# Xharlie/pointnerf

Hardware: AMD Instinct MI355X
Metric: rays/sec (render+bwd) NeRF-synth lego 800^2, K=8, 128 samp/ray (higher is better)
Workload: dtype f32 in / out / accumulate; forward GEMM operands as 2 x f16 planes (22-bit) on the f16 MFMA, 3 products per multiply-add; input-gradient GEMMs: f16 leading product + e4m3 cross terms (csrc/mixq.h), 2 product equivalents; weight-gradient GEMM operands as one f16 plane each

## Files before the change

pointnerf_amd/csrc/aggregate.hip:

```cpp
#include "mixq.h"
#include <stdlib.h>

extern "C" int pnerf_mlp_layout(int feat_dim, int64_t *offsets) {
    if (feat_dim != PN_F || !offsets) return PNERF_E_UNSUP;
    const int64_t o[PNERF_MLP_NTENSORS + 1] = {PO_W1, PO_B1, PO_W2, PO_B2, PO_W3, PO_B3, PO_W4, PO_B4, PO_W5, PO_B5,
                                               PO_WC1, PO_BC1, PO_WC2, PO_BC2, PO_WC3, PO_BC3, PO_WC4, PO_BC4, PO_TOTAL};
    for (int i = 0; i <= PNERF_MLP_NTENSORS; ++i) offsets[i] = o[i];
    return 0;
}
extern "C" size_t pnerf_mlp_packed_bytes(void) { return (size_t)PKC_END; }

namespace {
struct PackHDesc { int src, ld, trans, Mreal, Kreal, NCH, MB, dst, cm1, ck1; };
__device__ __forceinline__ float pn_pack_scale(const char *packed, int cm1, int ck1, int m, int k) {
    float f = 1.f;
    if (cm1 && m < (cm1 - 1 < PN_CS_C1 ? PN_H : PN_HC)) f = pn_col_scale(packed, cm1 - 1)[m];
    if (ck1) f *= pn_col_scale_inv(packed, ck1 - 1)[k];
    return f;
}
struct ColScaleDesc { int first, units, n_cons; struct { int src, ld, rows; } cons[2]; };
struct ColScaleTable { ColScaleDesc d[7]; };
__global__ __launch_bounds__(256) void k_pack_colscale(ColScaleTable t, const float *__restrict__ params, char *__restrict__ packed) {
    __shared__ unsigned red[256];
    const ColScaleDesc d = t.d[blockIdx.x];
    const int j = threadIdx.x;
    float mx = 0.f;
    if (j < d.units)
        for (int c = 0; c < d.n_cons; ++c)
            for (int r = 0; r < d.cons[c].rows; ++r) mx = fmaxf(mx, fabsf(params[d.cons[c].src + r * d.cons[c].ld + j]));
    const unsigned mb = __float_as_uint(mx);
    const bool ok = mb >= 0x00800000u && mb < 0x7f800000u;
    red[j] = ok ? mb : 0u;
    __syncthreads();
    for (int off = 128; off > 0; off >>= 1) {
        if (j < off) red[j] = red[j] > red[j + off] ? red[j] : red[j + off];
        __syncthreads();
    }
    if (j >= d.units) return;
    int e = ok ? (int)(red[0] >> 23) - (int)(mb >> 23) : 0;
    e = e > PN_CS_MAXE ? PN_CS_MAXE : e;
    float *cs = reinterpret_cast<float *>(packed + PKC_SCALE);
    cs[d.first + j] = __uint_as_float((unsigned)(127 + e) << 23);
    cs[PN_CS_UNITS + d.first + j] = __uint_as_float((unsigned)(127 - e) << 23);
}
struct PackHTable { PackHDesc d[15]; };
__global__ __launch_bounds__(256) void k_pack_h(PackHTable t, const float *__restrict__ params, char *__restrict__ packed) {
    const PackHDesc d = t.d[blockIdx.y];
    const int total = d.NCH * d.MB * 64;
    for (int e = blockIdx.x * 256 + threadIdx.x; e < total; e += gridDim.x * 256) {
        const int lane = e & 63, mb = (e >> 6) % d.MB, c = (e >> 6) / d.MB;
        const int m = 32 * mb + (lane & 31), k0 = 16 * c + 8 * (lane >> 5);
        unsigned h[4], lo[4];
#pragma unroll
        for (int j = 0; j < 4; ++j) {
            float v[2];
#pragma unroll
            for (int i = 0; i < 2; ++i) {
                const int k = k0 + 2 * j + i;
                v[i] = 0.f;
                if (m < d.Mreal && k < d.Kreal) v[i] = d.trans ? params[d.src + k * d.ld + m] * pn_pack_scale(packed, d.cm1, d.ck1, m, k) : params[d.src + m * d.ld + k];
            }
            pn_split2_sat(v[0], v[1], h[j], lo[j]);
        }
        uint4 *o = reinterpret_cast<uint4 *>(packed + d.dst) + ((size_t)(c * d.MB + mb) * 2) * 64 + lane;
        o[0] = make_uint4(h[0], h[1], h[2], h[3]);
        o[64] = make_uint4(lo[0], lo[1], lo[2], lo[3]);
    }
}

struct PackMDesc { int src, ld, trans, Mreal, Kreal, NT, MB, dst, cm1, ck1; };
struct PackMTable { PackMDesc d[9]; };
__global__ __launch_bounds__(256) void k_pack_mix(PackMTable t, const float *__restrict__ params, char *__restrict__ packed) {
    pn_mode_saturate();
    const PackMDesc d = t.d[blockIdx.y];
    auto W = [&](int m, int k) -> float {
        return (m < d.Mreal && k < d.Kreal) ? (d.trans ? params[d.src + k * d.ld + m] * pn_pack_scale(packed, d.cm1, d.ck1, m, k) : params[d.src + m * d.ld + k]) : 0.f;
    };
    uint4 *img = reinterpret_cast<uint4 *>(packed + d.dst);
    unsigned *sc = reinterpret_cast<unsigned *>(img + PN_MIMG_U4(d.NT, d.MB));
    const int nsup = PN_MIX_NS * d.MB * 64, ntail = d.NT * d.MB * 64;
    for (int e = blockIdx.x * 256 + threadIdx.x; e < nsup + ntail; e += gridDim.x * 256) {
        if (e < nsup) {
            const int lane = e & 63, mb = (e >> 6) % d.MB, s = (e >> 6) / d.MB, m = 32 * mb + (lane & 31), hf = lane >> 5;
            uint4 *o = img + ((size_t)(s * d.MB + mb) * 8) * 64 + lane;
#pragma unroll
            for (int r = 0; r < 4; ++r) {
                const int k0 = 64 * s + 16 * r + 8 * hf;
                unsigned h[4], lo[4];
#pragma unroll
                for (int j = 0; j < 4; ++j) pn_split2_rne(W(m, k0 + 2 * j), W(m, k0 + 2 * j + 1), h[j], lo[j]);
                o[r * 64] = make_uint4(h[0], h[1], h[2], h[3]);
            }
            unsigned scw = 0u;
#pragma unroll
            for (int j = 0; j < 2; ++j) {
                float wh[16], wm[16], mx = 0.f;
#pragma unroll
                for (int i = 0; i < 32; ++i) {
                    const float w = W(m, 64 * s + 32 * j + i);
#ifdef PN_EMU
                    const float wc = fmaxf(fminf(w, 65504.f), -65504.f);
#else
                    const float wc = w;
#endif
                    const float h = (float)(_Float16)wc;
                    mx = fmaxf(mx, fmaxf(fabsf(h), fabsf(w - h) * 2048.f));
                }
#pragma unroll
                for (int i = 0; i < 16; ++i) {
                    const float w = W(m, 8 * (8 * s + 4 * j + 2 * hf + (i >> 3)) + (i & 7));
#ifdef PN_EMU
                    const float wc = fmaxf(fminf(w, 65504.f), -65504.f);
#else
                    const float wc = w;
#endif
                    wh[i] = (float)(_Float16)wc; wm[i] = w - wh[i];
                }
                int ex = 0;
                const float fr = frexpf(mx, &ex);
                int be = mx > 0.f ? (fr > 0.875f ? ex - 8 : ex - 9) : 0;
                be = be < -100 ? -100 : (be > 100 ? 100 : be);
                const float sh = __uint_as_float((unsigned)(be + 127) << 23), sm = __uint_as_float((unsigned)(be + 127 - 11) << 23);
                scw |= (unsigned)(be + 127) << (8 * j);
#pragma unroll
                for (int tt = 0; tt < 2; ++tt) {
                    unsigned q[4];
#pragma unroll
                    for (int w4 = 0; w4 < 4; ++w4) {
                        const float *src = (w4 < 2 ? wm : wh) + 8 * tt + 4 * (w4 & 1);
                        const float scl = w4 < 2 ? sm : sh;
                        pn_s2 r = {0, 0};
                        r = __builtin_amdgcn_cvt_scalef32_pk_fp8_f32(r, src[0], src[1], scl, false);
                        r = __builtin_amdgcn_cvt_scalef32_pk_fp8_f32(r, src[2], src[3], scl, true);
                        q[w4] = __builtin_bit_cast(unsigned, r);
                    }
                    o[(4 + 2 * j + tt) * 64] = make_uint4(q[0], q[1], q[2], q[3]);
                }
            }
            sc[(size_t)(s * d.MB + mb) * 64 + lane] = scw;
        } else {
            const int e2 = e - nsup, lane = e2 & 63, mb = (e2 >> 6) % d.MB, tc = (e2 >> 6) / d.MB, m = 32 * mb + (lane & 31);
            const int k0 = 256 + 16 * tc + 8 * (lane >> 5);
            unsigned h[4], lo[4];
#pragma unroll
            for (int j = 0; j < 4; ++j) pn_split2_sat(W(m, k0 + 2 * j), W(m, k0 + 2 * j + 1), h[j], lo[j]);
            uint4 *o = img + (size_t)PN_MIX_NS * d.MB * 8 * 64 + ((size_t)(tc * d.MB + mb) * 2) * 64 + lane;
            o[0] = make_uint4(h[0], h[1], h[2], h[3]);
            o[64] = make_uint4(lo[0], lo[1], lo[2], lo[3]);
        }
    }
}
}

extern "C" int pnerf_mlp_pack(const float *d_params, void *d_packed, void *stream) {
    if (!d_params || !d_packed) return PNERF_E_INVAL;
    PackHTable th = {{
        {PO_W1, PN_IN1, 0, PN_H, PN_IN1, 18, 8, PKH_F1},
        {PO_W2, PN_H, 0, PN_H, PN_H, 16, 8, PKH_F2},
        {PO_W3, PN_IN3, 0, PN_H, PN_IN3, 17, 8, PKH_F3},
        {PO_W4, PN_H, 0, PN_H, PN_H, 16, 8, PKH_F4},
        {PO_W4, PN_H, 1, PN_H, PN_H, 16, 8, PKH_D4, PN_CS_L3 + 1, PN_CS_L4 + 1},
        {PO_W3, PN_IN3, 1, PN_IN3, PN_H, 16, 9, PKH_D3, PN_CS_L2 + 1, PN_CS_L3 + 1},
        {PO_W2, PN_H, 1, PN_H, PN_H, 16, 8, PKH_D2, PN_CS_L1 + 1, PN_CS_L2 + 1},
        {PO_W1, PN_IN1, 1, 32 * PN_MB_D1, PN_H, 16, PN_MB_D1, PKH_D1, 0, PN_CS_L1 + 1},
        {PO_WC1, PN_INC, 0, PN_HC, PN_INC, 18, 4, PKH_FC1},
        {PO_WC2, PN_HC, 0, PN_HC, PN_HC, 8, 4, PKH_FC2},
        {PO_WC3, PN_HC, 0, PN_HC, PN_HC, 8, 4, PKH_FC3},
        {PO_WC3, PN_HC, 1, PN_HC, PN_HC, 8, 4, PKH_DC3, PN_CS_C2 + 1, PN_CS_C3 + 1},
        {PO_WC2, PN_HC, 1, PN_HC, PN_HC, 8, 4, PKH_DC2, PN_CS_C1 + 1, PN_CS_C2 + 1},
        {PO_WC1, PN_INC, 1, PN_H, PN_HC, 8, 8, PKH_DC1, PN_CS_L4 + 1, PN_CS_C1 + 1},
        {PO_W1 + 32 * PN_MB_D1, PN_IN1, 1, PN_IN1 - 32 * PN_MB_D1, PN_H, 16, 2, PKH_D1T, 0, PN_CS_L1 + 1},
    }};
    const ColScaleTable tc = {{
        {PN_CS_L1, PN_H, 1, {{PO_W2, PN_H, PN_H}}},
        {PN_CS_L2, PN_H, 1, {{PO_W3, PN_IN3, PN_H}}},
        {PN_CS_L3, PN_H, 1, {{PO_W4, PN_H, PN_H}}},
        {PN_CS_L4, PN_H, 2, {{PO_W5, PN_H, 1}, {PO_WC1, PN_INC, PN_HC}}},
        {PN_CS_C1, PN_HC, 1, {{PO_WC2, PN_HC, PN_HC}}},
        {PN_CS_C2, PN_HC, 1, {{PO_WC3, PN_HC, PN_HC}}},
        {PN_CS_C3, PN_HC, 1, {{PO_WC4, PN_HC, 3}}},
    }};
    PnProfScope prof(PNK_PACK, (hipStream_t)stream);
    hipLaunchKernelGGL(k_pack_colscale, dim3(7), dim3(256), 0, (hipStream_t)stream, tc, d_params, (char *)d_packed);
    hipLaunchKernelGGL(k_pack_h, dim3(40, 15), dim3(256), 0, (hipStream_t)stream, th, d_params, (char *)d_packed);
    PackMTable tm = {{
        {PO_W1, PN_IN1, 0, PN_H, PN_IN1, 2, 8, PKM_F1},
        {PO_W2, PN_H, 0, PN_H, PN_H, 0, 8, PKM_F2},
        {PO_W3, PN_IN3, 0, PN_H, PN_IN3, 1, 8, PKM_F3},
        {PO_W4, PN_H, 0, PN_H, PN_H, 0, 8, PKM_F4},
        {PO_W4, PN_H, 1, PN_H, PN_H, 0, 8, PKM_D4, PN_CS_L3 + 1, PN_CS_L4 + 1},
        {PO_W3, PN_IN3, 1, PN_IN3, PN_H, 0, 9, PKM_D3, PN_CS_L2 + 1, PN_CS_L3 + 1},
        {PO_W2, PN_H, 1, PN_H, PN_H, 0, 8, PKM_D2, PN_CS_L1 + 1, PN_CS_L2 + 1},
        {PO_W1, PN_IN1, 1, 32 * PN_MB_D1, PN_H, 0, PN_MB_D1, PKM_D1, 0, PN_CS_L1 + 1},
        {PO_W1 + 32 * PN_MB_D1, PN_IN1, 1, PN_IN1 - 32 * PN_MB_D1, PN_H, 0, 2, PKM_D1T, 0, PN_CS_L1 + 1},
    }};
    hipLaunchKernelGGL(k_pack_mix, dim3(12, 9), dim3(256), 0, (hipStream_t)stream, tm, d_params, (char *)d_packed);
    PN_CHECK_LAUNCH();
    return 0;
}

namespace {
template <int NT>
__global__ __launch_bounds__(256) void k_debug_mix_gemm(const float *__restrict__ x, const char *__restrict__ img, float *__restrict__ out) {
    extern __shared__ __attribute__((aligned(16))) char smem_d[];
    pn_mode_saturate();
    constexpr int K = 256 + 16 * NT;
    char *X = smem_d;
    const int tid = threadIdx.x, lane = tid & 63, wave = __builtin_amdgcn_readfirstlane(tid >> 6);
    for (int e = tid; e < PN_TILE * (K / 4); e += 256) {
        const int row = e / (K / 4), col = 4 * (e % (K / 4));
        const float4 v = *reinterpret_cast<const float4 *>(x + row * K + col);
        if (col < 256) pn_xq_store4(X, row, col, v.x, v.y, v.z, v.w);
        else pn_xt_store4(X, row, col, v.x, v.y, v.z, v.w);
    }
    __syncthreads();
    f32x16 acc[2][2];
    pn_acc_zero(acc);
    pn_gemm_mix<PN_MIX_NS, NT, 8, 2>(X, img, 2 * wave, lane, acc);
#pragma unroll
    for (int fb = 0; fb < 2; ++fb)
#pragma unroll
        for (int rb = 0; rb < 2; ++rb)
#pragma unroll
            for (int g = 0; g < 4; ++g)
#pragma unroll
                for (int i = 0; i < 4; ++i) out[(32 * rb + (lane & 31)) * PN_H + pn_d_feat(2 * wave + fb, g, lane) + i] = acc[fb][rb][4 * g + i];
}
}

extern "C" int pnerf_debug_mix_gemm(const float *d_w, int K, const float *d_x, void *d_img, float *d_out, void *stream) {
    if (!d_w || !d_x || !d_img || !d_out || (K != 256 && K != 272 && K != 288)) return PNERF_E_INVAL;
    hipStream_t s = (hipStream_t)stream;
    const int NT = (K - 256) / 16;
    PackMTable tm = {{{0, K, 0, PN_H, K, NT, 8, 0}}};
    hipLaunchKernelGGL(k_pack_mix, dim3(12, 1), dim3(256), 0, s, tm, d_w, (char *)d_img);
    const void *fn = NT == 0 ? (const void *)k_debug_mix_gemm<0> : NT == 1 ? (const void *)k_debug_mix_gemm<1> : (const void *)k_debug_mix_gemm<2>;
    if (hipFuncSetAttribute(fn, hipFuncAttributeMaxDynamicSharedMemorySize, PN_XBYTES) != hipSuccess) return PNERF_E_LAUNCH;
    if (NT == 0) hipLaunchKernelGGL(k_debug_mix_gemm<0>, dim3(1), dim3(256), PN_XBYTES, s, d_x, (const char *)d_img, d_out);
    else if (NT == 1) hipLaunchKernelGGL(k_debug_mix_gemm<1>, dim3(1), dim3(256), PN_XBYTES, s, d_x, (const char *)d_img, d_out);
    else hipLaunchKernelGGL(k_debug_mix_gemm<2>, dim3(1), dim3(256), PN_XBYTES, s, d_x, (const char *)d_img, d_out);
    PN_CHECK_LAUNCH();
    return 0;
}

namespace {
__global__ __launch_bounds__(64) void k_debug_mfma_f16(const uint4 *__restrict__ a, const uint4 *__restrict__ b, float *__restrict__ d) {
    f32x16 acc;
#pragma unroll
    for (int r = 0; r < 16; ++r) acc[r] = 0.f;
    acc = __builtin_amdgcn_mfma_f32_32x32x16_f16(__builtin_bit_cast(pn_h8, a[threadIdx.x]), __builtin_bit_cast(pn_h8, b[threadIdx.x]), acc, 0, 0, 0);
#pragma unroll
    for (int r = 0; r < 16; ++r) d[threadIdx.x * 16 + r] = acc[r];
}
}
namespace {
__global__ __launch_bounds__(256) void k_debug_split(const float *__restrict__ x, long long n, unsigned *__restrict__ h, unsigned *__restrict__ m, int sat) {
    for (long long i = (long long)blockIdx.x * 256 + threadIdx.x; 2 * i < n; i += (long long)gridDim.x * 256) {
        unsigned hh, mm;
        if (sat) pn_split2_sat(x[2 * i], x[2 * i + 1], hh, mm);
        else pn_split2(x[2 * i], x[2 * i + 1], hh, mm);
        h[i] = hh; m[i] = mm;
    }
}
}
extern "C" int pnerf_debug_split(const float *d_x, int64_t n, void *d_h, void *d_m, int sat, void *stream) {
    if (!d_x || !d_h || !d_m || n < 0 || (n & 1)) return PNERF_E_INVAL;
    if (n == 0) return 0;
    hipLaunchKernelGGL(k_debug_split, dim3(64), dim3(256), 0, (hipStream_t)stream, d_x, (long long)n, (unsigned *)d_h, (unsigned *)d_m, sat);
    PN_CHECK_LAUNCH();
    return 0;
}

namespace {
template <int NF> __global__ __launch_bounds__(256) void k_debug_pe(const float *__restrict__ x, long long n, float *__restrict__ out) {
    for (long long i = (long long)blockIdx.x * 256 + threadIdx.x; i < n; i += (long long)gridDim.x * 256) {
        float s[NF], c[NF];
        pn_pe_octaves<NF>(x[i], s, c);
#pragma unroll
        for (int f = 0; f < NF; ++f) { out[(i * NF + f) * 2] = s[f]; out[(i * NF + f) * 2 + 1] = c[f]; }
    }
}
}
extern "C" int pnerf_debug_pe(const float *d_x, int64_t n, int nfreq, float *d_out, void *stream) {
    if (!d_x || !d_out || n < 0 || nfreq < 1 || nfreq > 5) return PNERF_E_INVAL;
    if (n == 0) return 0;
    hipStream_t s = (hipStream_t)stream;
    switch (nfreq) {
        case 1: hipLaunchKernelGGL(k_debug_pe<1>, dim3(64), dim3(256), 0, s, d_x, (long long)n, d_out); break;
        case 2: hipLaunchKernelGGL(k_debug_pe<2>, dim3(64), dim3(256), 0, s, d_x, (long long)n, d_out); break;
        case 3: hipLaunchKernelGGL(k_debug_pe<3>, dim3(64), dim3(256), 0, s, d_x, (long long)n, d_out); break;
        case 4: hipLaunchKernelGGL(k_debug_pe<4>, dim3(64), dim3(256), 0, s, d_x, (long long)n, d_out); break;
        default: hipLaunchKernelGGL(k_debug_pe<5>, dim3(64), dim3(256), 0, s, d_x, (long long)n, d_out); break;
    }
    PN_CHECK_LAUNCH();
    return 0;
}

extern "C" int pnerf_debug_mfma_f16(const void *d_a, const void *d_b, float *d_out, void *stream) {
    if (!d_a || !d_b || !d_out) return PNERF_E_INVAL;
    hipLaunchKernelGGL(k_debug_mfma_f16, dim3(1), dim3(64), 0, (hipStream_t)stream, (const uint4 *)d_a, (const uint4 *)d_b, d_out);
    PN_CHECK_LAUNCH();
    return 0;
}

size_t pn_saved_walk(void *base, long long n_valid, int K, PnSaved &s) {
    const int TS = pn_tile_samples(K);
    const long long tiles = (n_valid + TS - 1) / TS + 2 * PN_NCLS + 1;
    s.rows = tiles * PN_TILE;
    s.samples = ((tiles * TS + PN_CTILE - 1) / PN_CTILE + 1) * PN_CTILE;
    PnCarver cv(base);
    const size_t rg = (size_t)s.rows / 8, rgc = (size_t)s.samples / 8;
    auto planes = [&](uint4 *&x0, uint4 *&h2, uint4 *&h1, uint4 *&h3, uint4 *&dy1, uint4 *&dy2, uint4 *&dy3, uint4 *&dy4) {
        x0 = cv.take<uint4>(rg * PN_NF1); h2 = cv.take<uint4>(rg * PN_NF1);
        h1 = cv.take<uint4>(rg * PN_H); h3 = cv.take<uint4>(rg * PN_H);
        dy1 = cv.take<uint4>(rg * PN_H); dy2 = cv.take<uint4>(rg * PN_H);
        dy3 = cv.take<uint4>(rg * PN_H); dy4 = cv.take<uint4>(rg * PN_H);
    };
    auto cplanes = [&](uint4 *&xc, uint4 *&c1, uint4 *&c2, uint4 *&dc1, uint4 *&dc2, uint4 *&dc3) {
        xc = cv.take<uint4>(rgc * PN_NF1); c1 = cv.take<uint4>(rgc * PN_HC); c2 = cv.take<uint4>(rgc * PN_HC);
        dc1 = cv.take<uint4>(rgc * PN_HC); dc2 = cv.take<uint4>(rgc * PN_HC); dc3 = cv.take<uint4>(rgc * PN_HC);
    };
    planes(s.x0k, s.h2k, s.h1k, s.h3k, s.dy1k, s.dy2k, s.dy3k, s.dy4k);
    s.h4r = cv.take<uint4>((size_t)s.rows * 32 * 2);
    s.arow = cv.take<float>((size_t)s.rows); s.rmeta = cv.take<int4>((size_t)s.rows);
    s.lmask = cv.take<unsigned>((size_t)tiles * 3 * 512);
    s.gscale = cv.take<unsigned>(PN_GS_WORDS);
    s.fs = cv.take<float>((size_t)s.samples * PN_H); s.dfs = cv.take<float>((size_t)s.samples * PN_H);
    s.c3 = cv.take<float>((size_t)s.samples * PN_HC);
    cplanes(s.xck, s.c1k, s.c2k, s.dc1k, s.dc2k, s.dc3k);
    s.cmask = cv.take<unsigned>((size_t)s.samples / PN_CTILE * 2 * 256);
    s.wg2 = pn_arith().wgrad_planes == 2 ? 1 : 0;
    s.x0m = s.h1m = s.h2m = s.h3m = s.dy1m = s.dy2m = s.dy3m = s.dy4m = nullptr;
    s.xcm = s.c1m = s.c2m = s.dc1m = s.dc2m = s.dc3m = nullptr;
    if (s.wg2) {
        planes(s.x0m, s.h2m, s.h1m, s.h3m, s.dy1m, s.dy2m, s.dy3m, s.dy4m);
        cplanes(s.xcm, s.c1m, s.c2m, s.dc1m, s.dc2m, s.dc3m);
    }
    pn_cls_walk(cv, s);
    return cv.off;
}
void pn_cls_walk(PnCarver &cv, PnSaved &s) {
    s.cls_list = cv.take<int>((size_t)s.samples);
    s.cls_info = cv.take<int>(PN_CI_WORDS);
    s.cls_tmp = cv.take<int>((size_t)2 * s.samples + pn_scan_scratch_ints(s.samples) + 8);
}
size_t pn_saved_bytes(long long n_valid, int K) { PnSaved s; return pn_saved_walk(nullptr, n_valid, K, s); }
PnSaved pn_saved_carve(void *base, long long n_valid, int K) { PnSaved s; pn_saved_walk(base, n_valid, K, s); return s; }

extern "C" size_t pnerf_agg_saved_bytes(int64_t n_valid_samples, int K) {
    if (K <= 0 || K > PNERF_MAX_K || n_valid_samples < 0) return 0;
    return pn_saved_bytes(n_valid_samples, K);
}

namespace {
struct FwdArgs {
    pnerf_camera cam;
    const float *xyz, *emb, *conf, *dir, *color;
    const float *params;
    const float4 *packed;
    const float *raydir, *sample_loc;
    const float *xyz_pers, *loc_pers;
    const int *pidx, *valid_list, *counters;
    const int *cls_list, *cls_info;
    int cls, Kstride;
    int save_x0;
    int R, SR, K, TS;
    long long cap_samples;
    float *decoded, *weight;
    PnSaved sv;
};
struct FwdArgsF : FwdArgs { const float *frames; };
template <bool FRAMES> struct FwdArgsOf { using type = FwdArgs; };
template <> struct FwdArgsOf<true> { using type = FwdArgsF; };

namespace {
struct ClsArgs { const int *valid_list, *counters, *pidx; int K, n, ncls; int kc[PN_NCLS], ts[PN_NCLS]; };

__global__ void k_cls_flags(ClsArgs c, int which, int *__restrict__ flags) {
    const int vs = blockIdx.x * blockDim.x + threadIdx.x;
    if (vs >= c.n) return;
    const int Ns = c.counters[0] < c.n ? c.counters[0] : c.n;
    int f = 0;
    if (vs < Ns) {
        const long long si = c.valid_list[vs];
        int hv = 0;
        for (int k = 0; k < c.K; ++k)
            if (c.pidx[si * c.K + k] >= 0) hv = k + 1;
        int cl = 0;
        for (int j = 1; j < c.ncls; ++j)
            if (hv <= c.kc[j]) cl = j;
        f = cl == which;
    }
    flags[vs] = f;
}

__global__ void k_cls_gather(ClsArgs c, int which, const int *__restrict__ pos, const int *__restrict__ count, int *__restrict__ cls_list,
                             int *__restrict__ info) {
    const int n = *count, base = info[PN_CI_VBASE + which];
    for (int i = blockIdx.x * blockDim.x + threadIdx.x; i < n; i += gridDim.x * blockDim.x) cls_list[base + i] = c.valid_list[pos[i]];
    if (blockIdx.x == 0 && threadIdx.x == 0) {
        const int tiles = (n + c.ts[which] - 1) / c.ts[which], tb = info[PN_CI_TBASE + which];
        info[PN_CI_COUNT + which] = n;
        if (which + 1 < PN_NCLS) { info[PN_CI_VBASE + which + 1] = base + n; info[PN_CI_TBASE + which + 1] = tb + tiles + 1; }
        info[PN_CI_TILES] = tb + tiles + 1;
    }
}

__global__ void k_cls_zero_gaps(PnSaved sv, int ncls, int save_x0) {
    const int c = blockIdx.y;
    if (c >= ncls) return;
    if ((blockIdx.x == 0 && !save_x0) || (blockIdx.x == 8 && save_x0)) return;
    const long long gap = (c + 1 < PN_NCLS ? sv.cls_info[PN_CI_TBASE + c + 1] : sv.cls_info[PN_CI_TILES]) - 1;
    uint4 *arrs[9] = {sv.x0k, sv.h2k, sv.h1k, sv.h3k, sv.dy1k, sv.dy2k, sv.dy3k, sv.dy4k, sv.x0k};
    uint4 *arrm[9] = {sv.x0m, sv.h2m, sv.h1m, sv.h3m, sv.dy1m, sv.dy2m, sv.dy3m, sv.dy4m, nullptr};
    const int which = blockIdx.x;
    const int nf = which == 8 ? 64 : which < 2 ? PN_NF1 : PN_H;
    uint4 *p = arrs[which] + gap * 8 * nf;
    for (int i = threadIdx.x; i < 8 * nf; i += blockDim.x) p[i] = make_uint4(0u, 0u, 0u, 0u);
    if (sv.wg2 && arrm[which]) {
        uint4 *pm = arrm[which] + gap * 8 * nf;
        for (int i = threadIdx.x; i < 8 * nf; i += blockDim.x) pm[i] = make_uint4(0u, 0u, 0u, 0u);
    }
}
}

}

int pn_class_slots(int K, int kc[PN_NCLS]) {
    if (K % 4 == 0) { kc[0] = K; kc[1] = K / 2; kc[2] = K / 4; return 3; }
    kc[0] = K; kc[1] = kc[2] = 0;
    return 1;
}

int pn_classify(const PnSaved &sv, const int32_t *d_valid_list, const int32_t *d_counters, const int32_t *d_pidx, int K, long long n_valid,
                bool train, bool save_x0, hipStream_t s) {
    ClsArgs c;
    c.valid_list = d_valid_list; c.counters = d_counters; c.pidx = d_pidx; c.K = K; c.n = (int)n_valid;
    c.ncls = pn_class_slots(K, c.kc);
    for (int j = 0; j < PN_NCLS; ++j) c.ts[j] = c.kc[j] > 0 ? pn_tile_samples(c.kc[j]) : 1;
    if (hipMemsetAsync(sv.cls_info, 0, PN_CI_WORDS * sizeof(int), s) != hipSuccess) return PNERF_E_LAUNCH;
    if (n_valid <= 0) return 0;
    int *flags = sv.cls_tmp, *pos = flags + n_valid, *cnt = pos + n_valid, *scratch = cnt + 8;
    PnProfScope prof(PNK_COMPACT, s);
    for (int j = 0; j < c.ncls; ++j) {
        hipLaunchKernelGGL(k_cls_flags, dim3(pn_cdiv(n_valid, 256)), dim3(256), 0, s, c, j, flags);
        int rc = pn_compact_gt0_i32(flags, n_valid, pos, cnt, scratch, s);
        if (rc) return rc;
        hipLaunchKernelGGL(k_cls_gather, dim3(256), dim3(256), 0, s, c, j, pos, cnt, sv.cls_list, sv.cls_info);
    }
    if (train) hipLaunchKernelGGL(k_cls_zero_gaps, dim3(9, c.ncls), dim3(256), 0, s, sv, c.ncls, save_x0 ? 1 : 0);
    PN_CHECK_LAUNCH();
    return 0;
}


namespace {

constexpr int FL_EX = PN_XBYTES, FL_W5 = FL_EX + PN_TILE * 8 * 4, FL_ROW = FL_W5 + PN_H * 4, FL_CLAIM = FL_ROW + 4 * PN_TILE * 4 , FL_BYTES = FL_CLAIM + 16;
static_assert(2 * FL_BYTES <= 160 * 1024, "two forward workgroups must fit the 160 KB LDS");

struct FGather {
    float4 e0, e1;
    float px, py, pz, lx, ly, lz, cf;
    float ppx, ppy, ppz, lpx, lpy, lpz;
    float dxv, dyv, dzv, cx, cy, cz, rx, ry, rz;
    float fx, fy, fz, gx, gy, gz;
};

__device__ __forceinline__ int f_sample_of(const FwdArgs &a, long long tile, int row, int Ns, unsigned kinv) {
    const int ls = pn_row_div(row, kinv);
    const long long vs = tile * a.TS + ls;
    return (ls < a.TS && vs < Ns) ? a.valid_list[vs] : -1;
}

template <bool PERS, bool FRAMES = false>
__device__ __forceinline__ void f_gather(const FwdArgs &a, FGather &G, int si_, int p_, int q, const float *frames = nullptr) {
    const int p = p_ > 0 ? p_ : 0, si = si_ > 0 ? si_ : 0;
    const float *ep = a.emb + (long long)p * PN_F + PN_EPT * q;
    G.e0 = *reinterpret_cast<const float4 *>(ep); G.e1 = *reinterpret_cast<const float4 *>(ep + 4);
    G.px = a.xyz[3 * p]; G.py = a.xyz[3 * p + 1]; G.pz = a.xyz[3 * p + 2];
    G.lx = a.sample_loc[(long long)si * 3]; G.ly = a.sample_loc[(long long)si * 3 + 1]; G.lz = a.sample_loc[(long long)si * 3 + 2];
    if (PERS) {
        G.ppx = a.xyz_pers[3 * p]; G.ppy = a.xyz_pers[3 * p + 1]; G.ppz = a.xyz_pers[3 * p + 2];
        G.lpx = a.loc_pers[(long long)si * 3]; G.lpy = a.loc_pers[(long long)si * 3 + 1]; G.lpz = a.loc_pers[(long long)si * 3 + 2];
    }
    G.cf = a.conf[p];
    if (FRAMES) {
        const int r = si / a.SR, fr = q < 3 ? q : 2;
        const int ps_ = a.pidx[(long long)si * a.Kstride], ps = ps_ > 0 ? ps_ : 0;
        const float *fp = frames + (long long)p * 9 + 3 * fr, *gp = frames + (long long)ps * 9 + 3 * fr;
        G.fx = fp[0]; G.fy = fp[1]; G.fz = fp[2];
        G.gx = gp[0]; G.gy = gp[1]; G.gz = gp[2];
        G.dxv = a.dir[3 * p]; G.dyv = a.dir[3 * p + 1]; G.dzv = a.dir[3 * p + 2];
        G.rx = a.raydir[3 * r]; G.ry = a.raydir[3 * r + 1]; G.rz = a.raydir[3 * r + 2];
        if (q == 0) { G.cx = a.color[3 * p]; G.cy = a.color[3 * p + 1]; G.cz = a.color[3 * p + 2]; }
    } else if (q == 0) {
        const int r = si / a.SR;
        G.dxv = a.dir[3 * p]; G.dyv = a.dir[3 * p + 1]; G.dzv = a.dir[3 * p + 2];
        G.cx = a.color[3 * p]; G.cy = a.color[3 * p + 1]; G.cz = a.color[3 * p + 2];
        G.rx = a.raydir[3 * r]; G.ry = a.raydir[3 * r + 1]; G.rz = a.raydir[3 * r + 2];
    }
}

template <bool PERS, bool MIX = false, bool FRAMES = false>
__device__ __forceinline__ void f_build(const FwdArgs &a, const FGather &G, char *X, float *exb, float *wraw, int *sidx, int si, int p, int row, int q) {
    const float dwx = G.px - G.lx, dwy = G.py - G.ly, dwz = G.pz - G.lz;
    float ppx, ppy, pcz, spx, spy, scz;
    if (PERS) {
        ppx = G.ppx; ppy = G.ppy; pcz = G.ppz; spx = G.lpx; spy = G.lpy; scz = G.lpz;
    } else {
        float pcx, pcy, scx, scy;
        if (FRAMES) {
            const float *M = a.cam.camrot;
            const float x = G.px - a.cam.campos[0], y = G.py - a.cam.campos[1], z = G.pz - a.cam.campos[2];
            const float u = G.lx - a.cam.campos[0], v = G.ly - a.cam.campos[1], w = G.lz - a.cam.campos[2];
            pcx = __builtin_fmaf(z, M[6], __builtin_fmaf(y, M[3], x * M[0]));
            pcy = __builtin_fmaf(z, M[7], __builtin_fmaf(y, M[4], x * M[1]));
            pcz = __builtin_fmaf(z, M[8], __builtin_fmaf(y, M[5], x * M[2]));
            scx = __builtin_fmaf(w, M[6], __builtin_fmaf(u, M[0], v * M[3]));
            scy = __builtin_fmaf(w, M[7], __builtin_fmaf(u, M[1], v * M[4]));
            scz = __builtin_fmaf(w, M[8], __builtin_fmaf(u, M[2], v * M[5]));
        } else {
        rot3(a.cam.camrot, G.px - a.cam.campos[0], G.py - a.cam.campos[1], G.pz - a.cam.campos[2], false, pcx, pcy, pcz);
        rot3(a.cam.camrot, G.lx - a.cam.campos[0], G.ly - a.cam.campos[1], G.lz - a.cam.campos[2], false, scx, scy, scz);
        }
        ppx = pcx / pcz; ppy = pcy / pcz; spx = scx / scz; spy = scy / scz;
    }
    float d0, d1, d2;
    if (FRAMES) d0 = d1 = d2 = dwx * G.fx + dwy * G.fy + dwz * G.fz;
    else rot3(a.cam.rw2c, dwx, dwy, dwz, true, d0, d1, d2);
    const float d3 = ppx * pcz - spx * scz, d4 = ppy * pcz - spy * scz, d5 = pcz - scz;
    const float da = q == 0 ? d0 : q == 1 ? d1 : q == 2 ? d2 : d3;
    const float db = q == 0 ? d4 : d5;
    const float e[8] = {G.e0.x, G.e0.y, G.e0.z, G.e0.w, G.e1.x, G.e1.y, G.e1.z, G.e1.w};
    if (MIX) {
        pn_xq_store4(X, row, PN_EPT * q, e[0], e[1], e[2], e[3]);
        pn_xq_store4(X, row, PN_EPT * q + 4, e[4], e[5], e[6], e[7]);
#pragma unroll
        for (int i = 0; i < 8; i += 2) {
            const int col = PN_F + (PN_EPT * q + i) * 6;
            float s0[3], c0[3], s1[3], c1[3];
            pn_pe_octaves<3>(e[i], s0, c0);
            pn_pe_octaves<3>(e[i + 1], s1, c1);
            pn_xq_store4(X, row, col, s0[0], c0[0], s0[1], c0[1]);
            pn_xq_store4(X, row, col + 4, s0[2], c0[2], s1[0], c1[0]);
            pn_xq_store4(X, row, col + 8, s1[1], c1[1], s1[2], c1[2]);
        }
    } else {
    pn_xt_store4(X, row, PN_EPT * q, e[0], e[1], e[2], e[3]); pn_xt_store4(X, row, PN_EPT * q + 4, e[4], e[5], e[6], e[7]);
#pragma unroll
    for (int i = 0; i < 8; ++i) {
        const int dd = PN_EPT * q + i;
        float s[3], c[3];
        pn_pe_octaves<3>(e[i], s, c);
        pn_xt_store2(X, row, PN_F + dd * 6, s[0], c[0]);
        pn_xt_store2(X, row, PN_F + dd * 6 + 2, s[1], c[1]);
        pn_xt_store2(X, row, PN_F + dd * 6 + 4, s[2], c[2]);
    }
    }
#pragma unroll
    for (int j = 0; j < 2; ++j) {
        const int comp = q + 4 * j;
        if (comp < 6) {
            float s[5], c[5];
            pn_pe_octaves<5>(j == 0 ? da : db, s, c);
#pragma unroll
            for (int f = 0; f < 5; ++f) {
                if (MIX) pn_xa_store2(X, row, PN_F * 7 + (comp * 5 + f) * 2, s[f], c[f]);
                else pn_xt_store2(X, row, PN_F * 7 + (comp * 5 + f) * 2, s[f], c[f]);
            }
        }
    }
    if (q == 3) pn_xt_store4(X, row, PN_ONES1, 1.f, 0.f, 0.f, 0.f);
    float fvx = 0.f, fvy = 0.f, fvz = 0.f, fqx = 0.f, fqy = 0.f, fqz = 0.f;
    if (FRAMES) {
        fvx = G.rx * G.gx + G.ry * G.gy + G.rz * G.gz;
        fqx = G.dxv * G.fx + G.dyv * G.fy + G.dzv * G.fz;
        fvy = __shfl_down(fvx, 1, 64); fvz = __shfl_down(fvx, 2, 64);
        fqy = __shfl_down(fqx, 1, 64); fqz = __shfl_down(fqx, 2, 64);
    }
    if (q == 0) {
        float vx, vy, vz, qx, qy, qz;
        if (FRAMES) { vx = fvx; vy = fvy; vz = fvz; qx = fqx; qy = fqy; qz = fqz; }
        else {
        rot3(a.cam.rw2c, G.rx, G.ry, G.rz, true, vx, vy, vz);
        rot3(a.cam.rw2c, G.dxv, G.dyv, G.dzv, true, qx, qy, qz);
        }
        float *ex = exb + row * 8;
        *reinterpret_cast<float4 *>(ex) = make_float4(G.cx, G.cy, G.cz, qx - vx);
        if (FRAMES) {
            *reinterpret_cast<float4 *>(ex + 4) = make_float4(qy - vy, qz - vz, __builtin_fmaf(qz, vz, __builtin_fmaf(qx, vx, qy * vy)), 1.f);
            wraw[row] = p >= 0 ? 1.0f / fmaxf(sqrtf(__builtin_fmaf(dwz, dwz, __builtin_fmaf(dwx, dwx, dwy * dwy))), 1e-6f) : 0.f;
        } else {
        *reinterpret_cast<float4 *>(ex + 4) = make_float4(qy - vy, qz - vz, qx * vx + qy * vy + qz * vz, 1.f);
        wraw[row] = p >= 0 ? 1.0f / fmaxf(sqrtf(dwx * dwx + dwy * dwy + dwz * dwz), 1e-6f) : 0.f;
        }
        sidx[row] = si;
    }
}

__device__ __forceinline__ void f_acc_bias(const float *__restrict__ bias, int wave, int lane, f32x16 (&acc)[PN_NFB][2]) {
#pragma unroll
    for (int fb = 0; fb < PN_NFB; ++fb)
#pragma unroll
        for (int g = 0; g < 4; ++g) {
            const float4 b = *reinterpret_cast<const float4 *>(bias + pn_d_feat(PN_NFB * wave + fb, g, lane));
#pragma unroll
            for (int rb = 0; rb < 2; ++rb) { acc[fb][rb][4 * g] = b.x; acc[fb][rb][4 * g + 1] = b.y; acc[fb][rb][4 * g + 2] = b.z; acc[fb][rb][4 * g + 3] = b.w; }
        }
}
template <bool BITS, bool MIX = false, bool HR = false>
__device__ __forceinline__ void f_epilogue(const f32x16 (&acc)[PN_NFB][2], char *X, int wave, int lane, unsigned (&mw)[PN_NFB]) {
#pragma unroll
    for (int fb = 0; fb < PN_NFB; ++fb) mw[fb] = 0u;
#pragma unroll
    for (int fb = 0; fb < PN_NFB; ++fb)
#pragma unroll
        for (int rb = 0; rb < 2; ++rb)
#pragma unroll
            for (int g = 0; g < 4; ++g) {
                const int f0 = pn_d_feat(PN_NFB * wave + fb, g, lane);
                float v[4] = {acc[fb][rb][4 * g], acc[fb][rb][4 * g + 1], acc[fb][rb][4 * g + 2], acc[fb][rb][4 * g + 3]};
                if (BITS) {
#pragma unroll
                    for (int i = 0; i < 4; ++i) mw[fb] = __builtin_amdgcn_alignbit(mw[fb], __float_as_uint(v[i]), 31);
                }
#pragma unroll
                for (int i = 0; i < 4; ++i) v[i] = fmaxf(v[i], 0.01f * v[i]);
                if (MIX) pn_xq_store4(X, 32 * rb + (lane & 31), f0, v[0], v[1], v[2], v[3]);
                else if (HR) pn_xt_store4(X, 32 * rb + (lane & 31), f0, v[0], v[1], v[2], v[3]);
                else pn_x_store4<false>(X, 32 * rb + (lane & 31), f0, v[0], v[1], v[2], v[3]);
            }
}
__device__ __forceinline__ void f_store_masks(unsigned *__restrict__ lmask, long long gtile, int layer, int wave, int lane, const unsigned (&mw)[PN_NFB]) {
#pragma unroll
    for (int fb = 0; fb < PN_NFB; ++fb) lmask[((gtile * 3 + layer) * 8 + PN_NFB * wave + fb) * 64 + lane] = mw[fb];
}

template <int KC, bool TRAIN>
__device__ __forceinline__ void f_tail(const FwdArgs &a, const char *X, const float *w5s, const float *wrow, const int *sidx, float b5,
                                       long long tile, long long gtile, int tid, float *wraw = nullptr) {
    constexpr int NS = KC == 0 ? 1 : 8 / (KC == 0 ? 1 : KC);
    const int lane = tid & 63, cg = tid & 31, r0 = 8 * (tid >> 5);
    const float4 wa = *reinterpret_cast<const float4 *>(w5s + 8 * cg), wb = *reinterpret_cast<const float4 *>(w5s + 8 * cg + 4);
    float pa[8];
    float4 fa[NS], fb[NS];
#pragma unroll
    for (int j = 0; j < NS; ++j) fa[j] = fb[j] = make_float4(0.f, 0.f, 0.f, 0.f);
#pragma unroll
    for (int i = 0; i < 8; ++i) {
        const int r = r0 + i;
        const uint4 h = *reinterpret_cast<const uint4 *>(X + r * PN_XRS + cg * 16);
        const uint4 m = *reinterpret_cast<const uint4 *>(X + PN_XPLANE + r * PN_XRS + cg * 16);
        if (TRAIN) {
            pn_f4 th = {__uint_as_float(h.x), __uint_as_float(h.y), __uint_as_float(h.z), __uint_as_float(h.w)};
            pn_f4 tm = {__uint_as_float(m.x), __uint_as_float(m.y), __uint_as_float(m.z), __uint_as_float(m.w)};
            PN_STREAM_STORE(th, reinterpret_cast<pn_f4 *>(a.sv.h4r + (gtile * PN_TILE + r) * 32 + cg));
            PN_STREAM_STORE(tm, reinterpret_cast<pn_f4 *>(a.sv.h4r + (a.sv.rows + gtile * PN_TILE + r) * 32 + cg));
        }
        float s = 0.f;
        s = pn_fma2_lo(h.x, m.x, wa.x, s); s = pn_fma2_hi(h.x, m.x, wa.y, s); s = pn_fma2_lo(h.y, m.y, wa.z, s); s = pn_fma2_hi(h.y, m.y, wa.w, s);
        s = pn_fma2_lo(h.z, m.z, wb.x, s); s = pn_fma2_hi(h.z, m.z, wb.y, s); s = pn_fma2_lo(h.w, m.w, wb.z, s); s = pn_fma2_hi(h.w, m.w, wb.w, s);
        pa[i] = s;
        if (KC != 0) {
            const float w = wrow[r];
            float4 &f0 = fa[i / (KC == 0 ? 1 : KC)], &f1 = fb[i / (KC == 0 ? 1 : KC)];
            f0.x = pn_fma2_lo(h.x, m.x, w, f0.x); f0.y = pn_fma2_hi(h.x, m.x, w, f0.y); f0.z = pn_fma2_lo(h.y, m.y, w, f0.z); f0.w = pn_fma2_hi(h.y, m.y, w, f0.w);
            f1.x = pn_fma2_lo(h.z, m.z, w, f1.x); f1.y = pn_fma2_hi(h.z, m.z, w, f1.y); f1.z = pn_fma2_lo(h.w, m.w, w, f1.z); f1.w = pn_fma2_hi(h.w, m.w, w, f1.w);
        }
    }
#pragma unroll
    for (int j = 0; j < (KC == 0 ? 0 : NS); ++j) {
        const long long vs = tile * (PN_TILE / (KC == 0 ? 1 : KC)) + (r0 / (KC == 0 ? 1 : KC)) + j;
        if (vs < a.cap_samples) {
            *reinterpret_cast<float4 *>(a.sv.fs + vs * PN_H + 8 * cg) = fa[j];
            *reinterpret_cast<float4 *>(a.sv.fs + vs * PN_H + 8 * cg + 4) = fb[j];
        }
    }
    {
        const bool b4 = lane & 16, b3 = lane & 8, b2 = lane & 4;
#pragma unroll
        for (int j = 0; j < 4; ++j) { const float send = b4 ? pa[j] : pa[j + 4], keep = b4 ? pa[j + 4] : pa[j]; pa[j] = keep + __shfl_xor(send, 16, 64); }
#pragma unroll
        for (int j = 0; j < 2; ++j) { const float send = b3 ? pa[j] : pa[j + 2], keep = b3 ? pa[j + 2] : pa[j]; pa[j] = keep + __shfl_xor(send, 8, 64); }
        { const float send = b2 ? pa[0] : pa[1], keep = b2 ? pa[1] : pa[0]; pa[0] = keep + __shfl_xor(send, 4, 64); }
        pa[0] += __shfl_xor(pa[0], 2, 64);
        pa[0] += __shfl_xor(pa[0], 1, 64);
        const int i = ((lane >> 4) & 1) * 4 + ((lane >> 3) & 1) * 2 + ((lane >> 2) & 1), r = r0 + i;
        const float x = pa[0] + b5 - 1.0f;
        float sg = pn_softplus(x) * wrow[r];
        if (TRAIN && (lane & 3) == 0) a.sv.arow[gtile * PN_TILE + r] = x;
        if (KC == 0) {
            if ((lane & 3) == 0) wraw[r] = sg;
            return;
        }
        if (KC >= 2) sg += __shfl_xor(sg, 4, 64);
        if (KC >= 4) sg += __shfl_xor(sg, 8, 64);
        if (KC >= 8) sg += __shfl_xor(sg, 16, 64);
        if ((lane & 3) == 0 && (i % (KC == 0 ? 1 : KC)) == 0) {
            const int si = sidx[r];
            if (si >= 0) a.decoded[(long long)si * 4] = sg;
        }
    }
}

#ifdef PN_PHASE_TRACE
PN_TR_DECL(pn_trace_fwd);
PN_TR_SPAN_DECL(pn_span_fwd);
#endif
template <bool TRAIN, bool PERS, int NP, bool WG2 = false, bool FRAMES = false>
__global__ __launch_bounds__(PN_NTHR, PN_NW / 2) void k_agg_forward(typename FwdArgsOf<FRAMES>::type a) {
    constexpr bool MIX = NP == 4;
    static_assert(!FRAMES || (!TRAIN && NP == 3), "per-point frames: the default inference arithmetic only");
    constexpr bool HR = !MIX;
    constexpr bool HC = TRAIN && !WG2;
    static_assert(!(MIX && WG2), "the two-plane weight-gradient mode keeps f16x3.h's arithmetic everywhere");
    pn_mode_saturate();
    extern __shared__ __attribute__((aligned(16))) char smem_f[];
    char *X = smem_f;
    float *exb = reinterpret_cast<float *>(smem_f + FL_EX), *w5s = reinterpret_cast<float *>(smem_f + FL_W5);
    float *wraw = reinterpret_cast<float *>(smem_f + FL_ROW), *wrow = wraw + PN_TILE, *wnrm = wrow + PN_TILE;
    int *sidx = reinterpret_cast<int *>(wnrm + PN_TILE);
    const float *frames = nullptr;
    if constexpr (FRAMES) frames = a.frames;
    const int tid0 = threadIdx.x;
    const int K = a.K, TS = a.TS;
    const unsigned kinv = pn_kinv(K);
    const int Ns = a.cls_info[PN_CI_COUNT + a.cls];
    const long long vb = a.cls_info[PN_CI_VBASE + a.cls], tb = a.cls_info[PN_CI_TBASE + a.cls];
    a.valid_list = a.cls_list + vb; a.cap_samples = Ns;
    a.sv.fs += vb * PN_H;
    const long long ntiles = ((long long)Ns + TS - 1) / TS;
    const float *P = a.params;
    const char *img = reinterpret_cast<const char *>(a.packed);
    if (tid0 < PN_H) w5s[tid0] = P[PO_W5 + tid0];
    const float b5 = P[PO_B5];
    const int tile_last = (int)ntiles, grid = gridDim.x;
    int t0 = blockIdx.x, t1 = t0 + grid, t2 = t1 + grid;
    if (t0 >= tile_last) return;
    int *claim_ctr = a.sv.cls_info + PN_CI_CLAIM + a.cls, *claim_w = reinterpret_cast<int *>(smem_f + FL_CLAIM);
    int nclaim = 0;

    long long tile = t0;
    int si0, si1, si2, p0, p1;
    FGather G;
    {
        const int row = tid0 / PN_TPR, q = tid0 % PN_TPR, k = row - pn_row_div(row, kinv) * K;
        si0 = f_sample_of(a, tile, row, Ns, kinv); si1 = t1 < tile_last ? f_sample_of(a, t1, row, Ns, kinv) : -1;
        si2 = t2 < tile_last ? f_sample_of(a, t2, row, Ns, kinv) : -1;
        p0 = si0 >= 0 ? a.pidx[(long long)si0 * a.Kstride + k] : -1;
        p1 = si1 >= 0 ? a.pidx[(long long)si1 * a.Kstride + k] : -1;
        f_gather<PERS, FRAMES>(a, G, si0, p0, q, frames);
    }

    f32x16 acc[PN_NFB][2];
    PN_TR_ITER_DECL;
    for (bool first = true; t0 < tile_last; first = false) {
        PN_TR_ITER_NEXT;
        tile = t0;
        int tid = threadIdx.x;
        asm volatile("" : "+v"(tid));
        const int lane = tid & 63, wave = __builtin_amdgcn_readfirstlane(tid >> 6);
        const int row = tid / PN_TPR, q = tid % PN_TPR, k = row - pn_row_div(row, kinv) * K;
        const long long gtile = tb + tile;
        PN_LDS_BARRIER();
        PN_TR(pn_trace_fwd, 0); PN_TR_HWID(pn_trace_fwd); PN_TR_SPAN(pn_span_fwd, a.cls, 0);
        f_build<PERS, MIX, FRAMES>(a, G, X, exb, wraw, sidx, si0, p0, row, q);
        f_acc_bias(P + PO_B1, wave, lane, acc);
        PnTileW<MIX, 2, 8, NP> W1;
        W1.prefetch(img, PKH_F1, PKM_F1, PN_NFB * wave, lane);
        PN_LDS_BARRIER();
        if (q == 0) {
            const int ls = pn_row_div(row, kinv);
            float wn = 0.f, w = 0.f;
            if (si0 >= 0) {
                float sum = 0.f;
                for (int kk = 0; kk < K; ++kk) sum += wraw[ls * K + kk];
                wn = wraw[row] / fmaxf(sum, 1e-8f);
                w = wn * fminf(fmaxf(G.cf, 1e-4f), 1.0f);
                a.weight[(long long)si0 * a.Kstride + k] = wn;
            }
            wnrm[row] = wn; wrow[row] = w;
            if (TRAIN) a.sv.rmeta[gtile * PN_TILE + row] = make_int4(si0, si0 >= 0 ? p0 : -1, __float_as_int(wn), __float_as_int(w));
        }
        unsigned mask[PN_NFB];
        PN_TR(pn_trace_fwd, 1);
        PN_TR(pn_trace_fwd, 2);
        W1.run(X, lane, acc);
        if (TRAIN) {
            if (HC) {
                if (a.save_x0) pn_copy_out_kmajor_h<PN_NF1>(X, a.sv.x0k, gtile * 8, tid);
                else pn_copy_out_kmajor_cols64_h<224>(X, a.sv.x0k, gtile * 8, tid);
            } else if (WG2) pn_copy_out_kmajor<PN_NF1, true>(X, a.sv.x0k, gtile * 8, tid, a.sv.x0m);
            else if (a.save_x0) pn_copy_out_kmajor<PN_NF1, false>(X, a.sv.x0k, gtile * 8, tid);
            else pn_copy_out_kmajor_cols64<224>(X, a.sv.x0k, gtile * 8, tid);
        }
        PN_LDS_BARRIER();
        PN_TR(pn_trace_fwd, 3);
        f_epilogue<TRAIN, MIX, HR>(acc, X, wave, lane, mask);
        if (TRAIN) f_store_masks(a.sv.lmask, gtile, 0, wave, lane, mask);
        f_acc_bias(P + PO_B2, wave, lane, acc);
        PnTileW<MIX, 0, 8, NP> W2;
        W2.prefetch(img, PKH_F2, PKM_F2, PN_NFB * wave, lane);
        PN_LDS_BARRIER();
        PN_TR(pn_trace_fwd, 4);
        PN_TR(pn_trace_fwd, 5);
        W2.run(X, lane, acc);
        if (TRAIN) {
            if (HC) pn_copy_out_kmajor_h<PN_H>(X, a.sv.h1k, gtile * 8, tid);
            else pn_copy_out_kmajor<PN_H, WG2>(X, a.sv.h1k, gtile * 8, tid, a.sv.h1m);
        }
        PN_LDS_BARRIER();
        PN_TR(pn_trace_fwd, 6);
        f_epilogue<TRAIN, MIX, HR>(acc, X, wave, lane, mask);
        if (TRAIN) f_store_masks(a.sv.lmask, gtile, 1, wave, lane, mask);
        if (tid < PN_TILE) {
            const float4 u = *reinterpret_cast<const float4 *>(exb + tid * 8), v = *reinterpret_cast<const float4 *>(exb + tid * 8 + 4);
            pn_xt_store4(X, tid, PN_H, u.x, u.y, u.z, u.w);
            pn_xt_store4(X, tid, PN_H + 4, v.x, v.y, v.z, v.w);
            pn_xt_store4(X, tid, PN_H + 8, 0.f, 0.f, 0.f, 0.f);
            pn_xt_store4(X, tid, PN_H + 12, 0.f, 0.f, 0.f, 0.f);
        }
        f_acc_bias(P + PO_B3, wave, lane, acc);
        PnTileW<MIX, 1, 8, NP> W3;
        W3.prefetch(img, PKH_F3, PKM_F3, PN_NFB * wave, lane);
        PN_LDS_BARRIER();
        PN_TR(pn_trace_fwd, 7);
        PN_TR(pn_trace_fwd, 8);
        W3.run(X, lane, acc);
        if (TRAIN) {
            if (HC) pn_copy_out_kmajor_h<PN_NF1>(X, a.sv.h2k, gtile * 8, tid);
            else pn_copy_out_kmajor<PN_NF1, WG2>(X, a.sv.h2k, gtile * 8, tid, a.sv.h2m);
        }
        PN_LDS_BARRIER();
        PN_TR(pn_trace_fwd, 9);
        f_epilogue<TRAIN, MIX, HR>(acc, X, wave, lane, mask);
        if (TRAIN) f_store_masks(a.sv.lmask, gtile, 2, wave, lane, mask);
        f_acc_bias(P + PO_B4, wave, lane, acc);
        PnTileW<MIX, 0, 8, NP> W4;
        W4.prefetch(img, PKH_F4, PKM_F4, PN_NFB * wave, lane);
        PN_LDS_BARRIER();
        PN_TR(pn_trace_fwd, 10);
        PN_TR(pn_trace_fwd, 11);
        W4.run(X, lane, acc);
        if (TRAIN) {
            if (HC) pn_copy_out_kmajor_h<PN_H>(X, a.sv.h3k, gtile * 8, tid);
            else pn_copy_out_kmajor<PN_H, WG2>(X, a.sv.h3k, gtile * 8, tid, a.sv.h3m);
        }
        PN_TR(pn_trace_fwd, 12);
        const int t3 = first ? t2 + grid : pn_claim_tile(PN_CLAIM_STATIC_FWD, grid, __builtin_amdgcn_readfirstlane(*claim_w), nclaim - 1);
        const bool claims = nclaim % PN_CLAIM_TILES == 0;
        int claimed = 0;
        if (tid == 0 && claims) claimed = atomicAdd(claim_ctr, 1);
        const int si_next = si1, p_next = p1;
        if (t1 < tile_last) f_gather<PERS, FRAMES>(a, G, si1, p1, q, frames);
        const int p2 = si2 >= 0 ? a.pidx[(long long)si2 * a.Kstride + k] : -1;
        const int si3 = t3 < tile_last ? f_sample_of(a, t3, row, Ns, kinv) : -1;
        PN_LDS_BARRIER();
        PN_TR(pn_trace_fwd, 13);
        f_epilogue<false>(acc, X, wave, lane, mask);
        PN_LDS_BARRIER();
        PN_TR(pn_trace_fwd, 14);
        if (K == 8 || K == 4 || K == 2 || K == 1) {
            if (K == 8) f_tail<8, TRAIN>(a, X, w5s, wrow, sidx, b5, tile, gtile, tid);
            else if (K == 4) f_tail<4, TRAIN>(a, X, w5s, wrow, sidx, b5, tile, gtile, tid);
            else if (K == 2) f_tail<2, TRAIN>(a, X, w5s, wrow, sidx, b5, tile, gtile, tid);
            else f_tail<1, TRAIN>(a, X, w5s, wrow, sidx, b5, tile, gtile, tid);
            PN_TR(pn_trace_fwd, 15);
        } else {
        f_tail<0, TRAIN>(a, X, w5s, wrow, sidx, b5, tile, gtile, tid, wraw);
        PN_LDS_BARRIER();
        PN_TR(pn_trace_fwd, 15);
        for (int e = tid; e < TS * 32; e += PN_NTHR) {
            const int ls = e >> 5, cg = e & 31;
            float4 f0 = make_float4(0.f, 0.f, 0.f, 0.f), f1 = f0;
            for (int kk = 0; kk < K; ++kk) {
                const int r = ls * K + kk;
                const uint4 h = *reinterpret_cast<const uint4 *>(X + r * PN_XRS + cg * 16);
                const uint4 m = *reinterpret_cast<const uint4 *>(X + PN_XPLANE + r * PN_XRS + cg * 16);
                const float w = wrow[r];
                f0.x = pn_fma2_lo(h.x, m.x, w, f0.x); f0.y = pn_fma2_hi(h.x, m.x, w, f0.y); f0.z = pn_fma2_lo(h.y, m.y, w, f0.z); f0.w = pn_fma2_hi(h.y, m.y, w, f0.w);
                f1.x = pn_fma2_lo(h.z, m.z, w, f1.x); f1.y = pn_fma2_hi(h.z, m.z, w, f1.y); f1.z = pn_fma2_lo(h.w, m.w, w, f1.z); f1.w = pn_fma2_hi(h.w, m.w, w, f1.w);
            }
            const long long vs = tile * TS + ls;
            if (vs < a.cap_samples) {
                *reinterpret_cast<float4 *>(a.sv.fs + vs * PN_H + 8 * cg) = f0;
                *reinterpret_cast<float4 *>(a.sv.fs + vs * PN_H + 8 * cg + 4) = f1;
            }
        }
        if (tid < TS) {
            const int si = sidx[tid * K];
            if (si >= 0) {
                float sg = 0.f;
                for (int kk = 0; kk < K; ++kk) sg += wraw[tid * K + kk];
                a.decoded[(long long)si * 4] = sg;
            }
        }
        }
        si0 = si_next; p0 = p_next; si1 = si2; p1 = p2; si2 = si3;
        if (tid == 0 && claims) *claim_w = claimed;
        t0 = t1; t1 = t2; t2 = t3; ++nclaim;
        PN_TR(pn_trace_fwd, 16); PN_TR_SPAN(pn_span_fwd, a.cls, 1);
    }
}

constexpr int CL_W4 = PN_XBYTES, CL_BYTES = CL_W4 + 3 * PN_HC * 4;
static_assert(2 * CL_BYTES <= 160 * 1024, "two colour workgroups must fit the 160 KB LDS");

__device__ __forceinline__ void c_load_bias(const float *__restrict__ bias, int wave, int lane, float4 (&b)[4]) {
#pragma unroll
    for (int g = 0; g < 4; ++g) {
        const float *p = bias + pn_d_feat(wave, g, lane);
        b[g] = make_float4(p[0], p[1], p[2], p[3]);
    }
}
template <bool TRAIN, bool SAVE32>
__device__ __forceinline__ unsigned c_epilogue(const f32x16 (&acc)[2][2], const float4 (&bias)[4], char *X, int wave, int lane, float *__restrict__ save, long long grow0) {
    unsigned mw = 0u;
#pragma unroll
    for (int rb = 0; rb < 2; ++rb)
#pragma unroll
        for (int g = 0; g < 4; ++g) {
            const int f0 = pn_d_feat(wave, g, lane), row = 32 * rb + (lane & 31);
            const float4 b = bias[g];
            float v[4] = {acc[0][rb][4 * g] + b.x, acc[0][rb][4 * g + 1] + b.y, acc[0][rb][4 * g + 2] + b.z, acc[0][rb][4 * g + 3] + b.w};
            if (TRAIN && !SAVE32) {
#pragma unroll
                for (int i = 0; i < 4; ++i) mw = __builtin_amdgcn_alignbit(mw, __float_as_uint(v[i]), 31);
            }
#pragma unroll
            for (int i = 0; i < 4; ++i) v[i] = fmaxf(v[i], 0.01f * v[i]);
            if (TRAIN && SAVE32) {
                pn_f4 t = {v[0], v[1], v[2], v[3]};
                PN_REG_STORE(t, reinterpret_cast<pn_f4 *>(save + (grow0 + row) * PN_HC + f0));
            }
            pn_x_store4<false>(X, row, f0, v[0], v[1], v[2], v[3]);
        }
    return mw;
}

template <bool TRAIN, int NP, bool WG2 = false, bool FRAMES = false>
__global__ __launch_bounds__(256, 2) void k_color_forward(typename FwdArgsOf<FRAMES>::type a) {
    extern __shared__ __attribute__((aligned(16))) char smem_c[];
    char *X = smem_c;
    float *w4s = reinterpret_cast<float *>(smem_c + CL_W4);
    const int Ns = a.counters[0] < a.cap_samples ? a.counters[0] : (int)a.cap_samples;
    const float *P = a.params;
    const char *img = reinterpret_cast<const char *>(a.packed);
    for (int i = threadIdx.x; i < 3 * PN_HC; i += 256) w4s[i] = P[PO_WC4 + i];
    const float b40 = P[PO_BC4], b41 = P[PO_BC4 + 1], b42 = P[PO_BC4 + 2];

    f32x16 acc[2][2];
    for (long long tile = blockIdx.x; tile * PN_CTILE < Ns; tile += gridDim.x) {
        int tid = threadIdx.x;
        asm volatile("" : "+v"(tid));
        const int lane = tid & 63, wave = __builtin_amdgcn_readfirstlane(tid >> 6), row = tid >> 2, q = tid & 3;
        const long long grow0 = tile * PN_CTILE, vs = grow0 + row;
        const int si = vs < Ns ? a.valid_list[vs] : -1;
        PnGemmW<18, 4, 1, 7, NP> WC1;
        WC1.prefetch(reinterpret_cast<const uint4 *>(img + PKH_FC1), wave, lane);
        PN_LDS_BARRIER();
        if (si >= 0) {
            const float4 *f = reinterpret_cast<const float4 *>(a.sv.fs + vs * PN_H);
            float4 fv[16];
#pragma unroll
            for (int c = 0; c < 16; ++c) fv[c] = f[4 * c + q];
#pragma unroll
            for (int c = 0; c < 16; ++c) pn_x_store4<false>(X, row, 16 * c + 4 * q, fv[c].x, fv[c].y, fv[c].z, fv[c].w);
            {
                const int r = si / a.SR;
                float v[3], sn[4], cs[4];
                if constexpr (FRAMES) {
                    const int ps_ = a.pidx[(long long)si * a.Kstride], ps = ps_ > 0 ? ps_ : 0;
                    const float *fp = a.frames + (long long)ps * 9;
                    const float fm[9] = {fp[0], fp[1], fp[2], fp[3], fp[4], fp[5], fp[6], fp[7], fp[8]};
                    rot3(fm, a.raydir[3 * r], a.raydir[3 * r + 1], a.raydir[3 * r + 2], true, v[0], v[1], v[2]);
                } else
                rot3(a.cam.rw2c, a.raydir[3 * r], a.raydir[3 * r + 1], a.raydir[3 * r + 2], true, v[0], v[1], v[2]);
                const float vq = q == 0 ? v[0] : (q == 1 ? v[1] : v[2]);
                pn_pe_octaves<4>(vq, sn, cs);
                if (q < 3) {
                    pn_x_store4<false>(X, row, PN_H + 4 * q, sn[0], sn[1], sn[2], sn[3]);
                    pn_x_store4<false>(X, row, PN_H + 12 + 4 * q, cs[0], cs[1], cs[2], cs[3]);
                } else {
                    pn_x_store4<false>(X, row, PN_H + 24, 0.f, 0.f, 0.f, 0.f);
                    pn_x_store4<false>(X, row, PN_H + 28, 0.f, 0.f, 0.f, 0.f);
                }
            }
        } else {
#pragma unroll
            for (int c = 0; c < 18; ++c) pn_x_store4<false>(X, row, 16 * c + 4 * q, 0.f, 0.f, 0.f, 0.f);
        }
        PN_LDS_BARRIER();
        float4 bias[4];
        if (TRAIN) pn_copy_out_kmajor<PN_NF1, WG2>(X, a.sv.xck, tile * 8, tid, a.sv.xcm);
        pn_acc_zero(acc);
        pn_gemm_f16x3_run<18, 4, 1, 7, NP>(X, WC1, lane, acc);
        c_load_bias(P + PO_BC1, wave, lane, bias);
        PN_LDS_BARRIER();
        unsigned mw = c_epilogue<TRAIN, false>(acc, bias, X, wave, lane, nullptr, grow0);
        if (TRAIN) a.sv.cmask[(tile * 2 + 0) * 256 + tid] = mw;
        PnGemmW<8, 4, 1, 7, NP> WC2;
        WC2.prefetch(reinterpret_cast<const uint4 *>(img + PKH_FC2), wave, lane);
        PN_LDS_BARRIER();
        if (TRAIN) pn_copy_out_kmajor<PN_HC, WG2>(X, a.sv.c1k, tile * 8, tid, a.sv.c1m);
        pn_acc_zero(acc);
        pn_gemm_f16x3_run<8, 4, 1, 7, NP>(X, WC2, lane, acc);
        c_load_bias(P + PO_BC2, wave, lane, bias);
        PN_LDS_BARRIER();
        mw = c_epilogue<TRAIN, false>(acc, bias, X, wave, lane, nullptr, grow0);
        if (TRAIN) a.sv.cmask[(tile * 2 + 1) * 256 + tid] = mw;
        PnGemmW<8, 4, 1, 7, NP> WC3;
        WC3.prefetch(reinterpret_cast<const uint4 *>(img + PKH_FC3), wave, lane);
        PN_LDS_BARRIER();
        if (TRAIN) pn_copy_out_kmajor<PN_HC, WG2>(X, a.sv.c2k, tile * 8, tid, a.sv.c2m);
        pn_acc_zero(acc);
        pn_gemm_f16x3_run<8, 4, 1, 7, NP>(X, WC3, lane, acc);
        c_load_bias(P + PO_BC3, wave, lane, bias);
        PN_LDS_BARRIER();
        c_epilogue<TRAIN, true>(acc, bias, X, wave, lane, a.sv.c3, grow0);
        PN_LDS_BARRIER();
        {
            float o0 = 0.f, o1 = 0.f, o2 = 0.f;
#pragma unroll
            for (int j = 0; j < 4; ++j) {
                const int c0 = q * 32 + 8 * j;
                o0 = pn_x_dot8(X, row, c0, *reinterpret_cast<const float4 *>(w4s + c0), *reinterpret_cast<const float4 *>(w4s + c0 + 4), o0);
                o1 = pn_x_dot8(X, row, c0, *reinterpret_cast<const float4 *>(w4s + PN_HC + c0), *reinterpret_cast<const float4 *>(w4s + PN_HC + c0 + 4), o1);
                o2 = pn_x_dot8(X, row, c0, *reinterpret_cast<const float4 *>(w4s + 2 * PN_HC + c0), *reinterpret_cast<const float4 *>(w4s + 2 * PN_HC + c0 + 4), o2);
            }
            o0 = group_sum<4>(o0); o1 = group_sum<4>(o1); o2 = group_sum<4>(o2);
            if (q == 0 && si >= 0) {
                float *o = a.decoded + (long long)si * 4;
                o[1] = 1.0f / (1.0f + expf(-(o0 + b40))) * 1.002f - 0.001f;
                o[2] = 1.0f / (1.0f + expf(-(o1 + b41))) * 1.002f - 0.001f;
                o[3] = 1.0f / (1.0f + expf(-(o2 + b42))) * 1.002f - 0.001f;
            }
        }
    }
}
}

#ifndef PN_MIX_DEFAULT_MASK
#define PN_MIX_DEFAULT_MASK 4
#endif
static PnArith &pn_arith_record() {
    static PnArith a = [] {
        const char *e = getenv("PNERF_MIX_MASK");
        return PnArith{3, 1, 8, e ? atoi(e) & 7 : PN_MIX_DEFAULT_MASK};
    }();
    return a;
}
PnArith pn_arith() { return pn_arith_record(); }
static int pn_arith_set(int PnArith::*field, int v, bool valid) {
    if (!valid) return PNERF_E_INVAL;
    const int old = pn_arith_record().*field;
    pn_arith_record().*field = v;
    return old;
}
extern "C" int pnerf_set_inference_products(int n) { return pn_arith_set(&PnArith::products, n, n == 2 || n == 3); }
extern "C" int pnerf_set_wgrad_planes(int n) { return pn_arith_set(&PnArith::wgrad_planes, n, n == 1 || n == 2); }
extern "C" int pnerf_set_cross_terms(int bits) { return pn_arith_set(&PnArith::cross_terms, bits, bits == 8 || bits == 16); }
extern "C" int pnerf_set_cross_terms_where(int mask) { return pn_arith_set(&PnArith::mix_where, mask, mask >= 0 && mask <= 7); }
static int pn_tile_grid_cap = 0;
int pn_tile_grid(long long tiles, long long dflt) { return pn_capped_grid(tiles, pn_tile_grid_cap > 0 && pn_tile_grid_cap < dflt ? pn_tile_grid_cap : dflt); }
extern "C" int pnerf_debug_set_tile_grid(int max_workgroups) {
    if (max_workgroups < 0) return PNERF_E_INVAL;
    const int old = pn_tile_grid_cap;
    pn_tile_grid_cap = max_workgroups;
    return old;
}
extern "C" int pnerf_get_arithmetic(int32_t out[4]) {
    if (!out) return PNERF_E_INVAL;
    const PnArith a = pn_arith();
    out[0] = a.products; out[1] = a.wgrad_planes; out[2] = a.cross_terms; out[3] = a.mix_where;
    return 0;
}

int pn_agg_forward_launch(const pnerf_camera *cam, const pnerf_points *pts, const pnerf_step &st, float *d_decoded, float *d_weight,
                          const PnSaved &sv, bool train, bool save_x0, hipStream_t s) {
    const int K = st.K;
    const long long cap_samples = st.n_valid_max;
    const PnArith ar = pn_arith();
    FwdArgs a;
    const bool wg2 = train && sv.wg2;
    if (wg2) save_x0 = true;
    a.save_x0 = save_x0 ? 1 : 0;
    a.cam = *cam;
    a.xyz = pts->xyz; a.emb = pts->embedding; a.conf = pts->conf; a.dir = pts->dir; a.color = pts->color;
    a.params = st.params; a.packed = (const float4 *)st.packed_mlp;
    a.raydir = st.raydir; a.sample_loc = st.sample_loc; a.xyz_pers = st.xyz_pers; a.loc_pers = st.loc_pers; a.pidx = st.sample_pidx; a.valid_list = st.valid_list; a.counters = st.counters;
    a.R = st.R; a.SR = st.SR; a.K = K; a.TS = pn_tile_samples(K);
    a.cap_samples = cap_samples;
    a.decoded = d_decoded; a.weight = d_weight; a.sv = sv;
    const bool frames = pts->frames != nullptr;
    if (frames && train) return PNERF_E_INVAL;
    const int ncu = pn_cu_count();
    if (!ncu) return PNERF_E_LAUNCH;
    const int grid_c = pn_tile_grid((cap_samples + PN_CTILE - 1) / PN_CTILE, 2LL * ncu);
    const size_t lds_a = FL_BYTES, lds_c = CL_BYTES;
    const bool pers = st.xyz_pers != nullptr;
    const bool np2 = !train && ar.products == 2;
    const bool mix = !wg2 && !np2 && (ar.mix_mask() & (train ? 2 : 1));
    if (frames && (np2 || mix)) return PNERF_E_UNSUP;
    using FwdKernel = void (*)(FwdArgs);
    using FwdKernelF = void (*)(FwdArgsF);
    const FwdKernelF kfnf = pers ? k_agg_forward<false, true, 3, false, true> : k_agg_forward<false, false, 3, false, true>;
    const FwdKernelF cfnf = k_color_forward<false, 3, false, true>;
    const FwdKernel kfn = wg2   ? (pers ? k_agg_forward<true, true, 3, true> : k_agg_forward<true, false, 3, true>)
                        : mix   ? (train ? (pers ? k_agg_forward<true, true, 4> : k_agg_forward<true, false, 4>)
                                         : (pers ? k_agg_forward<false, true, 4> : k_agg_forward<false, false, 4>))
                        : train ? (pers ? k_agg_forward<true, true, 3> : k_agg_forward<true, false, 3>)
                        : np2   ? (pers ? k_agg_forward<false, true, 2> : k_agg_forward<false, false, 2>)
                                : (pers ? k_agg_forward<false, true, 3> : k_agg_forward<false, false, 3>);
    const FwdKernel cfn = wg2 ? k_color_forward<true, 3, true> : train ? k_color_forward<true, 3> : np2 ? k_color_forward<false, 2> : k_color_forward<false, 3>;
    if (hipFuncSetAttribute(frames ? reinterpret_cast<const void *>(kfnf) : reinterpret_cast<const void *>(kfn), hipFuncAttributeMaxDynamicSharedMemorySize, (int)lds_a) != hipSuccess) return PNERF_E_LAUNCH;
    if (hipFuncSetAttribute(frames ? reinterpret_cast<const void *>(cfnf) : reinterpret_cast<const void *>(cfn), hipFuncAttributeMaxDynamicSharedMemorySize, (int)lds_c) != hipSuccess) return PNERF_E_LAUNCH;
    int rc = pn_classify(sv, st.valid_list, st.counters, st.sample_pidx, K, cap_samples, train, save_x0, s);
    if (rc) return rc;
    a.cls_list = sv.cls_list; a.cls_info = sv.cls_info; a.Kstride = K;
    int kc[PN_NCLS];
    const int ncls = pn_class_slots(K, kc);
    {
        PnProfScope prof(PNK_AGG_FWD, s);
        for (int j = 0; j < ncls; ++j) {
            a.cls = j; a.K = kc[j]; a.TS = pn_tile_samples(kc[j]);
            const int grid_a = pn_tile_grid((cap_samples + a.TS - 1) / a.TS, 2LL * ncu);
            if (frames) { FwdArgsF af; static_cast<FwdArgs &>(af) = a; af.frames = pts->frames; hipLaunchKernelGGL(kfnf, dim3(grid_a), dim3(PN_NTHR), lds_a, s, af); }
            else hipLaunchKernelGGL(kfn, dim3(grid_a), dim3(PN_NTHR), lds_a, s, a);
        }
    }
    a.K = K; a.TS = pn_tile_samples(K); a.valid_list = sv.cls_list;
    {
        PnProfScope prof(PNK_COLOR_FWD, s);
        if (frames) { FwdArgsF af; static_cast<FwdArgs &>(af) = a; af.frames = pts->frames; hipLaunchKernelGGL(cfnf, dim3(grid_c), dim3(256), lds_c, s, af); }
        else hipLaunchKernelGGL(cfn, dim3(grid_c), dim3(256), lds_c, s, a);
    }
    PN_CHECK_LAUNCH();
    return 0;
}

#ifdef PN_PHASE_TRACE
extern "C" int pnerf_debug_trace_fwd(void *host, size_t bytes) {
    return hipMemcpyFromSymbol(host, HIP_SYMBOL(pn_trace_fwd), bytes < sizeof(pn_trace_fwd) ? bytes : sizeof(pn_trace_fwd)) == hipSuccess ? 0 : -1;
}
extern "C" int pnerf_debug_span_fwd(void *host, size_t bytes) {
    return hipMemcpyFromSymbol(host, HIP_SYMBOL(pn_span_fwd), bytes < sizeof(pn_span_fwd) ? bytes : sizeof(pn_span_fwd)) == hipSuccess ? 0 : -1;
}
#endif
```

pointnerf_amd/csrc/backward.hip:

```cpp
#include "mixq.h"

namespace {
constexpr int WG_CHUNKS = 256;
constexpr size_t PARTIAL_FLOATS = (size_t)WG_CHUNKS * PN_H * PN_IN1P;

struct BwdArgs {
    pnerf_camera cam;
    const float *params;
    const float4 *packed;
    const float *raydir;
    const int *pidx, *valid_list, *counters;
    const int *cls_list, *cls_info;
    int cls;
    int SR, K, TS;
    long long cap_samples;
    const float *decoded, *weight, *grad_decoded;
    PnSaved sv;
    const float *emb;
    float *gparams;
    float *g_emb, *g_conf, *g_dir, *g_color;
    const float *conf, *zo_gs;
    float zo_eps;
};
struct BwdXArgs : BwdArgs {
    const float *xyz, *sample_loc;
    float *g_xyz;
};
template <bool XYZG> struct BwdArgsOf { using T = BwdArgs; };
template <> struct BwdArgsOf<true> { using T = BwdXArgs; };

__global__ __launch_bounds__(256) void k_grad_max(const int *__restrict__ list, const int *__restrict__ counters, long long cap, const float *__restrict__ gd,
                                                  unsigned *__restrict__ gscale) {
    __shared__ unsigned red[4];
    const long long Ns = counters[0] < cap ? counters[0] : cap;
    float m = 0.f;
    for (long long vs = (long long)blockIdx.x * 256 + threadIdx.x; vs < Ns; vs += (long long)gridDim.x * 256) {
        const float4 g = *reinterpret_cast<const float4 *>(gd + (long long)list[vs] * 4);
        m = fmaxf(m, fmaxf(fmaxf(fabsf(g.x), fabsf(g.y)), fmaxf(fabsf(g.z), fabsf(g.w))));
    }
#pragma unroll
    for (int off = 32; off > 0; off >>= 1) m = fmaxf(m, __shfl_xor(m, off, 64));
    if ((threadIdx.x & 63) == 0) red[threadIdx.x >> 6] = __float_as_uint(m);
    __syncthreads();
    if (threadIdx.x == 0) {
        unsigned r = red[0];
        for (int i = 1; i < 4; ++i) r = red[i] > r ? red[i] : r;
        if (r != 0u && r < 0x7f800000u) atomicMax(gscale, r);
    }
}
__device__ __forceinline__ void pn_scale_from_bits(unsigned mb, float &S, float &invS) {
    const int e = (int)((mb >> 23) & 0xffu);
    int se = (e == 0 || e == 255) ? 127 : 127 + 4 - (e - 127);
    se = se < 2 ? 2 : (se > 252 ? 252 : se);
    S = __uint_as_float((unsigned)se << 23);
    invS = __uint_as_float((unsigned)(254 - se) << 23);
}
static_assert(PN_CTILE == PN_TILE, "one row-scale record layout for both tile kernels");
constexpr int PN_RSC_BYTES = PN_TILE * 16 + PN_TILE * 2;
__device__ __forceinline__ void pn_sample_scale(const float4 g, float S, float invS, float &Si, float &invSi) {
    const unsigned mb = __float_as_uint(fmaxf(fmaxf(fabsf(g.x), fabsf(g.y)), fmaxf(fabsf(g.z), fabsf(g.w))));
    Si = S; invSi = invS;
    if (mb >= 0x00800000u && mb < 0x7f800000u) {
        pn_scale_from_bits(mb, Si, invSi);
        if (Si < S) { Si = S; invSi = invS; }
    }
}
struct PnRowScale {
    float *p;
    __device__ __forceinline__ void set(int r, float Si, float invSi, float S, float w = 0.f) const {
        const float f = S * invSi;
        *reinterpret_cast<float4 *>(p + 4 * r) = make_float4(Si, invSi, f, w * Si);
        reinterpret_cast<_Float16 *>(p + 4 * PN_TILE)[r] = (_Float16)f;
    }
    __device__ __forceinline__ float S(int r) const { return p[4 * r]; }
    __device__ __forceinline__ float inv(int r) const { return p[4 * r + 1]; }
    __device__ __forceinline__ float to_call(int r) const { return p[4 * r + 2]; }
    __device__ __forceinline__ float wS(int r) const { return p[4 * r + 3]; }
    __device__ __forceinline__ const char *h8(int rg) const { return reinterpret_cast<const char *>(p + 4 * PN_TILE) + rg * 16; }
};
template <int NF, int XRS = PN_XRS>
__device__ __forceinline__ void pn_copy_out_kmajor_hs(const char *X, const PnRowScale &rs, uint4 *__restrict__ dst, long long rg0, int tid) {
    const int lane = tid & 63, wave = tid >> 6;
    const int blk = ((lane >> 2) & 3) * XRS + ((lane >> 4) * 16 + (lane & 3) * 4) * 2;
#pragma unroll
    for (int i = 0; i < 2; ++i) {
        const int rg = wave * 2 + i;
        const char *src = X + rg * 8 * XRS + blk;
        uint4 *d = dst + (rg0 + rg) * NF;
        const uint4 fq = *reinterpret_cast<const uint4 *>(rs.h8(rg));
        const pn_h4 flo = __builtin_bit_cast(pn_h4, make_uint2(fq.x, fq.y)), fhi = __builtin_bit_cast(pn_h4, make_uint2(fq.z, fq.w));
        uint2 lo[(NF + 63) / 64], hi[(NF + 63) / 64];
#pragma unroll
        for (int j = 0; j < (NF + 63) / 64; ++j) { lo[j] = pn_lds_read_tr16(src + j * 128); hi[j] = pn_lds_read_tr16(src + 4 * XRS + j * 128); }
#pragma unroll
        for (int j = 0; j < (NF + 63) / 64; ++j) {
            const int f = lane + 64 * j;
            if (f < NF) {
                const uint2 a = __builtin_bit_cast(uint2, __builtin_bit_cast(pn_h4, lo[j]) * flo), b = __builtin_bit_cast(uint2, __builtin_bit_cast(pn_h4, hi[j]) * fhi);
                pn_f4 t = {__uint_as_float(a.x), __uint_as_float(a.y), __uint_as_float(b.x), __uint_as_float(b.y)};
                PN_STREAM_STORE(t, reinterpret_cast<pn_f4 *>(d + f));
            }
        }
    }
}

constexpr int CB_XRS = 2 * PN_HC + 16, CB_XPL = PN_CTILE * CB_XRS, CB_XBYTES = 2 * CB_XPL;
constexpr int CB_GSUMS = 6 * PN_HC;
constexpr int CB_DRAW = CB_XBYTES, CB_GACC = CB_DRAW + PN_CTILE * 4 * 4, CB_W4 = CB_GACC + 4 * CB_GSUMS * 4, CB_RSC = CB_W4 + 3 * PN_HC * 4, CB_BYTES = CB_RSC + PN_RSC_BYTES;
static_assert(3 * CB_BYTES <= 160 * 1024, "three colour workgroups must fit the 160 KB LDS");

__device__ __forceinline__ void cb_epilogue(const f32x16 (&acc)[2][2], unsigned mw, char *X, int wave, int lane) {
#pragma unroll
    for (int rb = 0; rb < 2; ++rb)
#pragma unroll
        for (int g = 0; g < 4; ++g) {
            const int f0 = pn_d_feat(wave, g, lane), row = 32 * rb + (lane & 31), e = rb * 16 + g * 4;
            float v[4];
#pragma unroll
            for (int i = 0; i < 4; ++i) v[i] = acc[0][rb][4 * g + i] * ((int)(mw << (e + i)) < 0 ? 0.01f : 1.f);
            pn_x_store4<true, CB_XRS, CB_XPL>(X, row, f0, v[0], v[1], v[2], v[3]);
        }
}
__device__ __forceinline__ void cb_bias_sums(const char *X, const PnRowScale &rs, int tid, float *__restrict__ gsum) {
    const int cp = tid & 63, r0 = 16 * (tid >> 6);
    float g0 = 0.f, g1 = 0.f;
#pragma unroll
    for (int rr = 0; rr < 16; ++rr) {
        const unsigned h = *reinterpret_cast<const unsigned *>(X + (r0 + rr) * CB_XRS + cp * 4);
        const unsigned m = *reinterpret_cast<const unsigned *>(X + CB_XPL + (r0 + rr) * CB_XRS + cp * 4);
        const float f = rs.to_call(r0 + rr);
        g0 = pn_fma2_lo(h, m, f, g0); g1 = pn_fma2_hi(h, m, f, g1);
    }
    float2 *d = reinterpret_cast<float2 *>(gsum) + cp;
    const float2 t = *d;
    *d = make_float2(t.x + g0, t.y + g1);
}

__device__ __forceinline__ void cb_add4(float *__restrict__ d, const float (&v)[4]) {
    float4 *p = reinterpret_cast<float4 *>(d);
    const float4 t = *p;
    *p = make_float4(t.x + v[0], t.y + v[1], t.z + v[2], t.w + v[3]);
}

template <bool WG2>
__global__ __launch_bounds__(256, 3) void k_color_backward(BwdArgs a) {
    extern __shared__ __attribute__((aligned(16))) char smem_cb[];
    char *X = smem_cb;
    float *draw = reinterpret_cast<float *>(smem_cb + CB_DRAW);
    const PnRowScale rs{reinterpret_cast<float *>(smem_cb + CB_RSC)};
    const int Ns = a.counters[0] < a.cap_samples ? a.counters[0] : (int)a.cap_samples;
    const float *P = a.params;
    const char *img = reinterpret_cast<const char *>(a.packed);
    float S, invS;
    pn_scale_from_bits(a.sv.gscale[0], S, invS);
    if (blockIdx.x == 0 && threadIdx.x == 0) a.sv.cls_info[PN_CI_CTILES] = (Ns + PN_CTILE - 1) / PN_CTILE;
    float *gacc = reinterpret_cast<float *>(smem_cb + CB_GACC);
    for (int i = threadIdx.x; i < 4 * CB_GSUMS; i += 256) gacc[i] = 0.f;
    float *gaccw = gacc + (threadIdx.x >> 6) * CB_GSUMS;
    float gb4x = 0.f, gb4y = 0.f, gb4z = 0.f;
    auto row_sample = [&](long long t) -> long long {
        const long long vs = t * PN_CTILE + threadIdx.x;
        return (threadIdx.x < PN_CTILE && vs < Ns) ? (long long)a.valid_list[vs] : -1;
    };
    float po[3] = {0.f, 0.f, 0.f}, pg[3] = {0.f, 0.f, 0.f}, pgs = 0.f;
    auto row_values = [&](long long si) {
        if (si >= 0) {
            const float *o = a.decoded + si * 4, *g = a.grad_decoded + si * 4;
            po[0] = o[1]; po[1] = o[2]; po[2] = o[3]; pgs = g[0]; pg[0] = g[1]; pg[1] = g[2]; pg[2] = g[3];
        }
    };
    long long si_cur = row_sample(blockIdx.x);
    row_values(si_cur);
    float *w4s = reinterpret_cast<float *>(smem_cb + CB_W4);
    for (int i = threadIdx.x; i < 3 * PN_HC; i += 256) w4s[i] = P[PO_WC4 + i] * pn_col_scale(a.packed, PN_CS_C3)[i & (PN_HC - 1)];

    f32x16 acc[2][2];
    for (long long tile = blockIdx.x; tile * PN_CTILE < Ns; tile += gridDim.x) {
        int tid = threadIdx.x;
        asm volatile("" : "+v"(tid));
        const int lane = tid & 63, wave = __builtin_amdgcn_readfirstlane(tid >> 6);
        const long long grow0 = tile * PN_CTILE;
        float4 c3v[8];
#pragma unroll
        for (int rr = 0; rr < 8; ++rr) c3v[rr] = *reinterpret_cast<const float4 *>(a.sv.c3 + (grow0 + 8 * (tid >> 5) + rr) * PN_HC + 4 * (tid & 31));
        const unsigned mw2 = a.sv.cmask[(tile * 2 + 1) * 256 + tid], mw1 = a.sv.cmask[(tile * 2 + 0) * 256 + tid];
        PN_LDS_BARRIER();
        if (tid < PN_CTILE) {
            float d0 = 0.f, d1 = 0.f, d2 = 0.f, Si = S, invSi = invS;
            if (si_cur >= 0) {
                pn_sample_scale(make_float4(pgs, pg[0], pg[1], pg[2]), S, invS, Si, invSi);
                const float s0 = (po[0] + 0.001f) / 1.002f, s1 = (po[1] + 0.001f) / 1.002f, s2 = (po[2] + 0.001f) / 1.002f;
                d0 = pg[0] * 1.002f * s0 * (1.f - s0); d1 = pg[1] * 1.002f * s1 * (1.f - s1); d2 = pg[2] * 1.002f * s2 * (1.f - s2);
            }
            *reinterpret_cast<float4 *>(draw + tid * 4) = make_float4(d0, d1, d2, Si);
            rs.set(tid, Si, invSi, S);
            gb4x += d0; gb4y += d1; gb4z += d2;
        }
        const long long si_next = row_sample(tile + gridDim.x);
        PN_LDS_BARRIER();
        {
            const int c4 = tid & 31, rg = tid >> 5;
            float w4[3][4], gw4[3][4], gb3[4] = {0.f, 0.f, 0.f, 0.f};
#pragma unroll
            for (int k = 0; k < 3; ++k) {
                const float4 w = *reinterpret_cast<const float4 *>(w4s + k * PN_HC + 4 * c4);
                w4[k][0] = w.x; w4[k][1] = w.y; w4[k][2] = w.z; w4[k][3] = w.w;
#pragma unroll
                for (int i = 0; i < 4; ++i) gw4[k][i] = 0.f;
            }
#pragma unroll
            for (int rr = 0; rr < 8; ++rr) {
                const int row = 8 * rg + rr;
                const float4 d = *reinterpret_cast<const float4 *>(draw + row * 4);
                const float c[4] = {c3v[rr].x, c3v[rr].y, c3v[rr].z, c3v[rr].w};
                float u[4];
#pragma unroll
                for (int i = 0; i < 4; ++i) {
                    u[i] = (d.x * w4[0][i] + d.y * w4[1][i] + d.z * w4[2][i]) * pn_lrelu_grad(c[i]);
                    gw4[0][i] += d.x * c[i]; gw4[1][i] += d.y * c[i]; gw4[2][i] += d.z * c[i];
                    gb3[i] += u[i];
                }
                pn_x_store4<true, CB_XRS, CB_XPL>(X, row, 4 * c4, u[0] * d.w, u[1] * d.w, u[2] * d.w, u[3] * d.w);
            }
#pragma unroll
            for (int i = 0; i < 4; ++i) {
#pragma unroll
                for (int k = 0; k < 3; ++k) gw4[k][i] += __shfl_xor(gw4[k][i], 32, 64);
                gb3[i] += __shfl_xor(gb3[i], 32, 64);
            }
            if (lane < 32) {
#pragma unroll
                for (int k = 0; k < 3; ++k) cb_add4(gaccw + k * PN_HC + 4 * c4, gw4[k]);
                cb_add4(gaccw + 3 * PN_HC + 4 * c4, gb3);
            }
        }
        PnGemmW<8, 4, 1, 4, 3> WD3;
        WD3.prefetch(reinterpret_cast<const uint4 *>(img + PKH_DC3), wave, lane);
        PN_LDS_BARRIER();
        pn_copy_out_kmajor_hs<PN_HC, CB_XRS>(X, rs, a.sv.dc3k, tile * 8, tid);
        if (WG2) pn_copy_out_kmajor_hs<PN_HC, CB_XRS>(X + CB_XPL, rs, a.sv.dc3m, tile * 8, tid);
        pn_acc_zero(acc);
        pn_gemm_f16x3_run<8, 4, 1, 4, 3, CB_XRS, CB_XPL>(X, WD3, lane, acc);
        row_values(si_next);
        si_cur = si_next;
        PN_LDS_BARRIER();
        cb_epilogue(acc, mw2, X, wave, lane);
        PnGemmW<8, 4, 1, 4, 3> WD2;
        WD2.prefetch(reinterpret_cast<const uint4 *>(img + PKH_DC2), wave, lane);
        PN_LDS_BARRIER();
        cb_bias_sums(X, rs, tid, gaccw + 4 * PN_HC);
        pn_copy_out_kmajor_hs<PN_HC, CB_XRS>(X, rs, a.sv.dc2k, tile * 8, tid);
        if (WG2) pn_copy_out_kmajor_hs<PN_HC, CB_XRS>(X + CB_XPL, rs, a.sv.dc2m, tile * 8, tid);
        pn_acc_zero(acc);
        pn_gemm_f16x3_run<8, 4, 1, 4, 3, CB_XRS, CB_XPL>(X, WD2, lane, acc);
        PN_LDS_BARRIER();
        cb_epilogue(acc, mw1, X, wave, lane);
        PnGemmW<8, 8, 2, 1, 3> WD1;
        WD1.prefetch(reinterpret_cast<const uint4 *>(img + PKH_DC1), 2 * wave, lane);
        PN_LDS_BARRIER();
        cb_bias_sums(X, rs, tid, gaccw + 5 * PN_HC);
        pn_copy_out_kmajor_hs<PN_HC, CB_XRS>(X, rs, a.sv.dc1k, tile * 8, tid);
        if (WG2) pn_copy_out_kmajor_hs<PN_HC, CB_XRS>(X + CB_XPL, rs, a.sv.dc1m, tile * 8, tid);
        pn_acc_zero(acc);
        pn_gemm_f16x3_run<8, 8, 2, 1, 3, CB_XRS, CB_XPL>(X, WD1, lane, acc);
#pragma unroll
        for (int fb = 0; fb < 2; ++fb)
#pragma unroll
            for (int rb = 0; rb < 2; ++rb) {
                const float ri = rs.inv(32 * rb + (lane & 31));
#pragma unroll
                for (int g = 0; g < 4; ++g) {
                    pn_f4 t = {acc[fb][rb][4 * g] * ri, acc[fb][rb][4 * g + 1] * ri, acc[fb][rb][4 * g + 2] * ri, acc[fb][rb][4 * g + 3] * ri};
                    PN_REG_STORE(t, reinterpret_cast<pn_f4 *>(a.sv.dfs + (grow0 + 32 * rb + (lane & 31)) * PN_H + pn_d_feat(2 * wave + fb, g, lane)));
                }
            }
    }
    PN_LDS_BARRIER();
    {
        const int tid = threadIdx.x;
        auto total = [&](int i) { return (gacc[i] + gacc[CB_GSUMS + i]) + (gacc[2 * CB_GSUMS + i] + gacc[3 * CB_GSUMS + i]); };
        for (int i = tid; i < 3 * PN_HC; i += 256) atomicAdd(&a.gparams[PO_WC4 + i], total(i));
        if (tid < PN_HC) {
            atomicAdd(&a.gparams[PO_BC3 + tid], total(3 * PN_HC + tid) * pn_col_scale_inv(a.packed, PN_CS_C3)[tid]);
            atomicAdd(&a.gparams[PO_BC2 + tid], total(4 * PN_HC + tid) * invS * pn_col_scale_inv(a.packed, PN_CS_C2)[tid]);
            atomicAdd(&a.gparams[PO_BC1 + tid], total(5 * PN_HC + tid) * invS * pn_col_scale_inv(a.packed, PN_CS_C1)[tid]);
        }
        if (tid < PN_CTILE) {
#pragma unroll
            for (int off = 32; off > 0; off >>= 1) { gb4x += __shfl_xor(gb4x, off, 64); gb4y += __shfl_xor(gb4y, off, 64); gb4z += __shfl_xor(gb4z, off, 64); }
            if (tid == 0) { atomicAdd(&a.gparams[PO_BC4], gb4x); atomicAdd(&a.gparams[PO_BC4 + 1], gb4y); atomicAdd(&a.gparams[PO_BC4 + 2], gb4z); }
        }
    }
}

constexpr int BL_ROW = PN_XBYTES, BL_RSC = BL_ROW + 10 * PN_TILE * 4, BL_W5 = BL_RSC + PN_RSC_BYTES, BL_CLAIM = BL_W5 + PN_H * 4 ,
              BL_C4 = BL_CLAIM + 16 , BL_BYTES = BL_C4 + PN_H * 4;
constexpr int LDDX = 228;
static_assert(2 * BL_BYTES <= 160 * 1024, "two backward workgroups must fit the 160 KB LDS");
static_assert(PN_TILE * LDDX * 4 <= PN_XBYTES, "d X0 tile");
constexpr int LDDX_X = 292, BL_GW = BL_BYTES, BL_BYTES_X = BL_GW + PN_TILE * 4;
static_assert(2 * BL_BYTES_X <= 160 * 1024, "two xyz_grad backward workgroups must fit the 160 KB LDS");
static_assert(PN_TILE * LDDX_X * 4 <= PN_XBYTES, "d X0 tile (xyz_grad)");

template <bool MIX = false>
__device__ __forceinline__ void b_epilogue(const f32x16 (&acc)[PN_NFB][2], const unsigned (&mask)[PN_NFB], char *X, int wave, int lane) {
#pragma unroll
    for (int fb = 0; fb < PN_NFB; ++fb) {
        const unsigned mw = mask[fb];
#pragma unroll
        for (int rb = 0; rb < 2; ++rb)
#pragma unroll
            for (int g = 0; g < 4; ++g) {
                float v[4];
#pragma unroll
                for (int i = 0; i < 4; ++i) {
                    const int e = (rb * 4 + g) * 4 + i;
                    v[i] = acc[fb][rb][4 * g + i] * ((int)(mw << e) < 0 ? 0.01f : 1.f);
                }
                if (MIX) pn_xq_store4(X, 32 * rb + (lane & 31), pn_d_feat(PN_NFB * wave + fb, g, lane), v[0], v[1], v[2], v[3]);
                else pn_x_store4<true>(X, 32 * rb + (lane & 31), pn_d_feat(PN_NFB * wave + fb, g, lane), v[0], v[1], v[2], v[3]);
            }
    }
}

#ifdef PN_EMU
#define PN_WAVE_LDS_SYNC() __syncthreads()
#else
#define PN_WAVE_LDS_SYNC() asm volatile("s_waitcnt lgkmcnt(0)" ::: "memory")
#endif

template <int KC, bool MIX = false, bool XG = false>
__device__ __forceinline__ void b_front(const BwdArgs &a, char *X, const float *w5s, const float *c4is, const float *wrow, const float *wnrm, const float *dsg, const float *xrow,
                                        float *draw, const int *sidx, const int *prow, const float4 (&dfr)[4], const float *dfb0, const PnRowScale &rs, int tid,
                                        float (&gw5)[8], float &gb5t, unsigned kinv = 0u, float *gwf = nullptr) {
    const int lane = tid & 63, cg = tid & 31, r0 = 8 * (tid >> 5);
    const int j0 = KC == 0 ? pn_row_div(r0, kinv) : 0;
    float zo_conf = 0.f;
    if (a.zo_gs && (lane & 3) == 0) {
        const int rz = prow[r0 + ((lane >> 4) & 1) * 4 + ((lane >> 3) & 1) * 2 + ((lane >> 2) & 1)];
        if (rz >= 0) zo_conf = a.conf[rz];
    }
    auto df_of = [&](int j, float4 &ga, float4 &gb) {
        if (KC >= 4) { ga = dfr[2 * j]; gb = dfr[2 * j + 1]; }
        else { ga = *reinterpret_cast<const float4 *>(dfb0 + j * PN_H); gb = *reinterpret_cast<const float4 *>(dfb0 + j * PN_H + 4); }
    };
    const float4 cia = *reinterpret_cast<const float4 *>(c4is + 8 * cg), cib = *reinterpret_cast<const float4 *>(c4is + 8 * cg + 4);
    float pd[8];
#pragma unroll
    for (int i = 0; i < 8; ++i) {
        const int r = r0 + i, j = KC == 0 ? pn_row_div(r, kinv) - j0 : i / (KC == 0 ? 1 : KC);
        const uint4 h = *reinterpret_cast<const uint4 *>(X + r * PN_XRS + cg * 16);
        const uint4 m = *reinterpret_cast<const uint4 *>(X + PN_XPLANE + r * PN_XRS + cg * 16);
        float4 ga, gb;
        df_of(j, ga, gb);
        ga.x *= cia.x; ga.y *= cia.y; ga.z *= cia.z; ga.w *= cia.w; gb.x *= cib.x; gb.y *= cib.y; gb.z *= cib.z; gb.w *= cib.w;
        float s = 0.f;
        s = pn_fma2_lo(h.x, m.x, ga.x, s); s = pn_fma2_hi(h.x, m.x, ga.y, s); s = pn_fma2_lo(h.y, m.y, ga.z, s); s = pn_fma2_hi(h.y, m.y, ga.w, s);
        s = pn_fma2_lo(h.z, m.z, gb.x, s); s = pn_fma2_hi(h.z, m.z, gb.y, s); s = pn_fma2_lo(h.w, m.w, gb.z, s); s = pn_fma2_hi(h.w, m.w, gb.w, s);
        pd[i] = s;
    }
    {
        const bool b4 = lane & 16, b3 = lane & 8, b2 = lane & 4;
#pragma unroll
        for (int j = 0; j < 4; ++j) { const float send = b4 ? pd[j] : pd[j + 4], keep = b4 ? pd[j + 4] : pd[j]; pd[j] = keep + __shfl_xor(send, 16, 64); }
#pragma unroll
        for (int j = 0; j < 2; ++j) { const float send = b3 ? pd[j] : pd[j + 2], keep = b3 ? pd[j + 2] : pd[j]; pd[j] = keep + __shfl_xor(send, 8, 64); }
        { const float send = b2 ? pd[0] : pd[1], keep = b2 ? pd[1] : pd[0]; pd[0] = keep + __shfl_xor(send, 4, 64); }
        pd[0] += __shfl_xor(pd[0], 2, 64);
        pd[0] += __shfl_xor(pd[0], 1, 64);
        const int r = r0 + ((lane >> 4) & 1) * 4 + ((lane >> 3) & 1) * 2 + ((lane >> 2) & 1);
        if ((lane & 3) == 0) {
            float dr = 0.f, gw = 0.f;
            if (sidx[r] >= 0) {
                const float x = xrow[r], dotf = pd[0] * rs.S(r);
                const float alpha = pn_softplus(x), sg = pn_sigmoid(x);
                const int rp = prow[r];
                float zo_eps = a.zo_eps;
                asm volatile("" : "+s"(zo_eps));
                if (rp >= 0) atomicAdd(&a.g_conf[rp], (dsg[r] * alpha + dotf) * wnrm[r] * rs.inv(r) + (a.zo_gs ? PnZeroOne(zo_conf, zo_eps).grad(a.zo_gs[0]) : 0.f));
                if (XG && rp >= 0) gw = dsg[r] * alpha + dotf;
                dr = dsg[r] * wrow[r] * sg;
            }
            draw[r] = dr;
            if (XG) gwf[r] = gw;
        }
    }
    PN_WAVE_LDS_SYNC();
    const float4 wa = *reinterpret_cast<const float4 *>(w5s + 8 * cg), wb = *reinterpret_cast<const float4 *>(w5s + 8 * cg + 4);
    const float w5[8] = {wa.x, wa.y, wa.z, wa.w, wb.x, wb.y, wb.z, wb.w};
    float drsum = 0.f;
#pragma unroll
    for (int i = 0; i < 8; ++i) {
        const int r = r0 + i, j = KC == 0 ? pn_row_div(r, kinv) - j0 : i / (KC == 0 ? 1 : KC);
        const uint4 h = *reinterpret_cast<const uint4 *>(X + r * PN_XRS + cg * 16);
        const uint4 m = *reinterpret_cast<const uint4 *>(X + PN_XPLANE + r * PN_XRS + cg * 16);
        const bool live = sidx[r] >= 0;
        const float dr = draw[r], w = rs.wS(r), drc = dr * rs.to_call(r);
        drsum += drc;
        const float hv[8] = {pn_h_lo(h.x) + pn_h_lo(m.x), pn_h_hi(h.x) + pn_h_hi(m.x), pn_h_lo(h.y) + pn_h_lo(m.y), pn_h_hi(h.y) + pn_h_hi(m.y),
                             pn_h_lo(h.z) + pn_h_lo(m.z), pn_h_hi(h.z) + pn_h_hi(m.z), pn_h_lo(h.w) + pn_h_lo(m.w), pn_h_hi(h.w) + pn_h_hi(m.w)};
        float4 ga, gb;
        df_of(j, ga, gb);
        const float g[8] = {ga.x, ga.y, ga.z, ga.w, gb.x, gb.y, gb.z, gb.w};
        float o[8];
#pragma unroll
        for (int c = 0; c < 8; ++c) {
            o[c] = live ? (w * g[c] + dr * w5[c]) * pn_lrelu_grad(hv[c]) : 0.f;
            gw5[c] += drc * hv[c];
        }
        unsigned oh[4], om[4];
#pragma unroll
        for (int c = 0; c < 4; ++c) pn_split2_sat(o[2 * c], o[2 * c + 1], oh[c], om[c]);
        *reinterpret_cast<uint4 *>(X + r * PN_XRS + cg * 16) = make_uint4(oh[0], oh[1], oh[2], oh[3]);
        if (MIX) *reinterpret_cast<uint4 *>(X + PN_XPLANE + r * PN_XRS + cg * 16) =
                     make_uint4(pn_q8x4(oh[0], oh[1], 1.0f), pn_q8x4(oh[2], oh[3], 1.0f), pn_q8x4(om[0], om[1], PN_MIX_MSC), pn_q8x4(om[2], om[3], PN_MIX_MSC));
        else *reinterpret_cast<uint4 *>(X + PN_XPLANE + r * PN_XRS + cg * 16) = make_uint4(om[0], om[1], om[2], om[3]);
    }
    if (cg == 0) gb5t += drsum;
}

__device__ __forceinline__ void b_xyz_row(const BwdXArgs &a, const float *dxr, const float *gwf, const float *wrow, const float *wnrm, const int *sidx,
                                          int rp, int row, int q, int K, unsigned kinv, float invS) {
    float u[6] = {0.f, 0.f, 0.f, 0.f, 0.f, 0.f}, t = 0.f;
    float dwx = 0.f, dwy = 0.f, dwz = 0.f;
    if (rp >= 0) {
        const long long si = sidx[row];
        const float px = a.xyz[3 * rp], py = a.xyz[3 * rp + 1], pz = a.xyz[3 * rp + 2];
        const float lx = a.sample_loc[si * 3], ly = a.sample_loc[si * 3 + 1], lz = a.sample_loc[si * 3 + 2];
        dwx = px - lx; dwy = py - ly; dwz = pz - lz;
        float pcx, pcy, pcz, scx, scy, scz, d0, d1, d2;
        rot3(a.cam.camrot, px - a.cam.campos[0], py - a.cam.campos[1], pz - a.cam.campos[2], false, pcx, pcy, pcz);
        rot3(a.cam.camrot, lx - a.cam.campos[0], ly - a.cam.campos[1], lz - a.cam.campos[2], false, scx, scy, scz);
        rot3(a.cam.rw2c, dwx, dwy, dwz, true, d0, d1, d2);
        const float d3 = (pcx / pcz) * pcz - (scx / scz) * scz, d4 = (pcy / pcz) * pcz - (scy / scz) * scz, d5 = pcz - scz;
#pragma unroll
        for (int j = 0; j < 2; ++j) {
            const int c = q + 4 * j;
            if (c < 6) {
                float sn[5], cs[5];
                pn_pe_octaves<5>(j == 0 ? (q == 0 ? d0 : q == 1 ? d1 : q == 2 ? d2 : d3) : (q == 0 ? d4 : d5), sn, cs);
                float g = 0.f, fr = 1.f;
#pragma unroll
                for (int f = 0; f < 5; ++f) {
                    const float2 x = *reinterpret_cast<const float2 *>(dxr + PN_F * 7 + (c * 5 + f) * 2);
                    g += fr * (x.x * cs[f] - x.y * sn[f]);
                    fr *= 2.f;
                }
#pragma unroll
                for (int i = 0; i < 6; ++i) u[i] = c == i ? g : u[i];
            }
        }
        const int k0 = pn_row_div(row, kinv) * K;
        for (int k = q; k < K; k += 4) t += gwf[k0 + k] * wrow[k0 + k];
    }
#pragma unroll
    for (int i = 0; i < 6; ++i) u[i] = group_sum<4>(u[i]);
    t = group_sum<4>(t);
    if (rp >= 0 && q < 3) {
        float gx, gy, gz, hx, hy, hz;
        rot3(a.cam.rw2c, u[0], u[1], u[2], false, gx, gy, gz);
        rot3(a.cam.camrot, u[3], u[4], u[5], true, hx, hy, hz);
        const float len = sqrtf(dwx * dwx + dwy * dwy + dwz * dwz);
        const float cw = len >= 1e-6f ? -(gwf[row] * wrow[row] - t * wnrm[row]) / (len * len) : 0.f;
        const float v = q == 0 ? gx + hx + cw * dwx : q == 1 ? gy + hy + cw * dwy : gz + hz + cw * dwz;
        atomicAdd(&a.g_xyz[3 * rp + q], v * invS);
    }
}

#ifdef PN_PHASE_TRACE
PN_TR_DECL(pn_trace_bwd);
PN_TR_SPAN_DECL(pn_span_bwd);
#endif
template <bool WG2, bool MIX = false, bool XYZG = false>
__global__ __launch_bounds__(PN_NTHR, PN_NW / 2) void k_agg_backward(typename BwdArgsOf<XYZG>::T a) {
    static_assert(!(MIX && WG2), "the two-plane weight-gradient mode keeps f16x3.h's arithmetic everywhere");
    constexpr int LDX = XYZG ? LDDX_X : LDDX;
    pn_mode_saturate();
    extern __shared__ __attribute__((aligned(16))) char smem_b[];
    char *X = smem_b;
    float *wrow = reinterpret_cast<float *>(smem_b + BL_ROW), *wnrm = wrow + PN_TILE, *draw = wnrm + PN_TILE, *dsg = draw + PN_TILE, *xrow = dsg + PN_TILE;
    const PnRowScale rs{reinterpret_cast<float *>(smem_b + BL_RSC)};
    int *sidx = reinterpret_cast<int *>(xrow + PN_TILE), *prow = sidx + PN_TILE;
    float *rdir = reinterpret_cast<float *>(prow + PN_TILE);
    float *w5s = reinterpret_cast<float *>(smem_b + BL_W5), *c4is = reinterpret_cast<float *>(smem_b + BL_C4);
    float *dx = reinterpret_cast<float *>(smem_b);
    float *gwf = XYZG ? reinterpret_cast<float *>(smem_b + BL_GW) : nullptr;
    const int tid0 = threadIdx.x;
    const int K = a.K, TS = a.TS;
    const unsigned kinv = pn_kinv(K);
    const int Ns = a.cls_info[PN_CI_COUNT + a.cls];
    const long long vb = a.cls_info[PN_CI_VBASE + a.cls], tb = a.cls_info[PN_CI_TBASE + a.cls];
    a.sv.dfs += vb * PN_H;
    const long long ntiles = ((long long)Ns + TS - 1) / TS;
    const float *P = a.params;
    const char *img = reinterpret_cast<const char *>(a.packed);
    float S, invS;
    pn_scale_from_bits(a.sv.gscale[0], S, invS);
    if (tid0 < PN_H) { w5s[tid0] = P[PO_W5 + tid0] * pn_col_scale(a.packed, PN_CS_L4)[tid0]; c4is[tid0] = pn_col_scale_inv(a.packed, PN_CS_L4)[tid0]; }
    float gw5[8] = {0.f, 0.f, 0.f, 0.f, 0.f, 0.f, 0.f, 0.f};
    float gb5t = 0.f;
    f32x16 acc[PN_NFB][2];
    constexpr bool CLAIM = !(XYZG && !MIX);
    using tile_t = std::conditional_t<CLAIM, int, long long>;
    const tile_t tile_first = blockIdx.x, tile_last = (tile_t)ntiles, grid = gridDim.x;
    tile_t t_cur = tile_first;
    [[maybe_unused]] tile_t t_nxt = t_cur + grid;
    int nclaim = 0;
    int *claim_ctr = reinterpret_cast<int *>(a.sv.gscale) + PN_GS_CLAIM + a.cls, *claim_w = reinterpret_cast<int *>(smem_b + BL_CLAIM);
    int4 rm_cur = make_int4(-1, -1, 0, 0);
    float ar_cur = 0.f;
    if (tid0 < PN_TILE && tile_first < tile_last) {
        rm_cur = a.sv.rmeta[(tb + tile_first) * PN_TILE + tid0];
        ar_cur = a.sv.arow[(tb + tile_first) * PN_TILE + tid0];
    }
    PN_TR_ITER_DECL;
    for (; t_cur < tile_last; ++nclaim) {
        PN_TR_ITER_NEXT;
        const long long tile = t_cur;
        int tid = threadIdx.x;
        asm volatile("" : "+v"(tid));
        const int lane = tid & 63, wave = __builtin_amdgcn_readfirstlane(tid >> 6);
        const int row = tid / PN_TPR, q = tid % PN_TPR;
        const long long gtile = tb + tile;
        PN_LDS_BARRIER();
        PN_TR(pn_trace_bwd, 0); PN_TR_HWID(pn_trace_bwd); PN_TR_SPAN(pn_span_bwd, a.cls, 0);
        unsigned m1[PN_NFB], m2[PN_NFB], m3[PN_NFB];
#pragma unroll
        for (int fb = 0; fb < PN_NFB; ++fb) {
            const long long o = (long long)(PN_NFB * wave + fb) * 64 + lane;
            m1[fb] = a.sv.lmask[(gtile * 3 + 0) * 512 + o]; m2[fb] = a.sv.lmask[(gtile * 3 + 1) * 512 + o]; m3[fb] = a.sv.lmask[(gtile * 3 + 2) * 512 + o];
        }
        float4 gd_v = make_float4(0.f, 0.f, 0.f, 0.f);
        float rdx = 0.f, rdy = 0.f, rdz = 0.f;
        if (tid < PN_TILE && rm_cur.x >= 0) {
            gd_v = *reinterpret_cast<const float4 *>(a.grad_decoded + (long long)rm_cur.x * 4);
            const int r = rm_cur.x / a.SR;
            rdx = a.raydir[3 * r]; rdy = a.raydir[3 * r + 1]; rdz = a.raydir[3 * r + 2];
        }
        pn_f4 h4v[2 * PN_TILE * 32 / PN_NTHR];
#pragma unroll
        for (int i = 0; i < 2 * PN_TILE * 32 / PN_NTHR; ++i) {
            const int e = tid + PN_NTHR * i, plane = e >> 11, r = (e >> 5) & 63, u = e & 31;
            h4v[i] = *reinterpret_cast<const pn_f4 *>(a.sv.h4r + ((long long)plane * a.sv.rows + gtile * PN_TILE + r) * 32 + u);
        }
        int4 rm_nxt = make_int4(-1, -1, 0, 0);
        float ar_nxt = 0.f;
        if constexpr (CLAIM) {
            if (tid < PN_TILE && t_nxt < tile_last) {
                rm_nxt = a.sv.rmeta[(tb + t_nxt) * PN_TILE + tid];
                ar_nxt = a.sv.arow[(tb + t_nxt) * PN_TILE + tid];
            }
        } else {
            if (tid < PN_TILE && tile + grid < tile_last) {
                rm_nxt = a.sv.rmeta[(gtile + grid) * PN_TILE + tid];
                ar_nxt = a.sv.arow[(gtile + grid) * PN_TILE + tid];
            }
        }
        __builtin_amdgcn_sched_barrier(0);
        if (tid < PN_TILE) {
            sidx[tid] = rm_cur.x; prow[tid] = rm_cur.y;
            wnrm[tid] = __int_as_float(rm_cur.z); wrow[tid] = __int_as_float(rm_cur.w);
            xrow[tid] = ar_cur;
            float Si, invSi;
            pn_sample_scale(gd_v, S, invS, Si, invSi);
            rs.set(tid, Si, invSi, S, __int_as_float(rm_cur.w));
            dsg[tid] = gd_v.x * Si;
            rdir[tid] = rdx; rdir[PN_TILE + tid] = rdy; rdir[2 * PN_TILE + tid] = rdz;
        }
#pragma unroll
        for (int i = 0; i < 2 * PN_TILE * 32 / PN_NTHR; ++i) {
            const int e = tid + PN_NTHR * i, plane = e >> 11, r = (e >> 5) & 63, u = e & 31;
            *reinterpret_cast<pn_f4 *>(X + plane * PN_XPLANE + r * PN_XRS + u * 16) = h4v[i];
        }
        __builtin_amdgcn_sched_barrier(0);
        float4 dfr[4];
        const float *dfb0 = a.sv.dfs + (tile * TS + pn_row_div(8 * ((tid >> 5) & 7), kinv)) * PN_H + 8 * (tid & 31);
        if (K == 8 || K == 4) {
            dfr[0] = *reinterpret_cast<const float4 *>(dfb0); dfr[1] = *reinterpret_cast<const float4 *>(dfb0 + 4);
            if (K == 4) { dfr[2] = *reinterpret_cast<const float4 *>(dfb0 + PN_H); dfr[3] = *reinterpret_cast<const float4 *>(dfb0 + PN_H + 4); }
        }
        __builtin_amdgcn_sched_barrier(0);
        rm_cur = rm_nxt; ar_cur = ar_nxt;
        PN_LDS_BARRIER();
        PN_TR(pn_trace_bwd, 1);
        [[maybe_unused]] const bool claims = nclaim % PN_CLAIM_TILES == 0;
        [[maybe_unused]] int claimed = 0;
        if constexpr (CLAIM) { if (tid == 0 && claims) claimed = atomicAdd(claim_ctr, 1); }
        const int rp = prow[row];
        float4 e0 = make_float4(0.f, 0.f, 0.f, 0.f), e1 = e0;
        if (rp >= 0) {
            const float *ep = a.emb + (long long)rp * PN_F + PN_EPT * q;
            e0 = *reinterpret_cast<const float4 *>(ep); e1 = *reinterpret_cast<const float4 *>(ep + 4);
        }
        {
            if (K == 8) b_front<8, MIX, XYZG>(a, X, w5s, c4is, wrow, wnrm, dsg, xrow, draw, sidx, prow, dfr, dfb0, rs, tid, gw5, gb5t, 0u, gwf);
            else if (K == 4) b_front<4, MIX, XYZG>(a, X, w5s, c4is, wrow, wnrm, dsg, xrow, draw, sidx, prow, dfr, dfb0, rs, tid, gw5, gb5t, 0u, gwf);
            else if (K == 2) b_front<2, MIX, XYZG>(a, X, w5s, c4is, wrow, wnrm, dsg, xrow, draw, sidx, prow, dfr, dfb0, rs, tid, gw5, gb5t, 0u, gwf);
            else if (K == 1) b_front<1, MIX, XYZG>(a, X, w5s, c4is, wrow, wnrm, dsg, xrow, draw, sidx, prow, dfr, dfb0, rs, tid, gw5, gb5t, 0u, gwf);
            else b_front<0, MIX, XYZG>(a, X, w5s, c4is, wrow, wnrm, dsg, xrow, draw, sidx, prow, dfr, dfb0, rs, tid, gw5, gb5t, kinv, gwf);
            PN_TR(pn_trace_bwd, 2);
        }
        PnTileW<MIX, 0, 8> W4;
        W4.prefetch(img, PKH_D4, PKM_D4, PN_NFB * wave, lane);
        if constexpr (CLAIM) { if (tid == 0 && claims) *claim_w = claimed; }
        PN_LDS_BARRIER();
        PN_TR(pn_trace_bwd, 3);
        if constexpr (CLAIM) {
            t_cur = t_nxt;
            t_nxt = pn_claim_tile(PN_CLAIM_STATIC_BWD, grid, __builtin_amdgcn_readfirstlane(*claim_w), nclaim);
        }
        pn_acc_zero(acc);
        PN_TR(pn_trace_bwd, 4);
        W4.run(X, lane, acc);
        pn_copy_out_kmajor_hs<PN_H>(X, rs, a.sv.dy4k, gtile * 8, tid);
        if (WG2) pn_copy_out_kmajor_hs<PN_H>(X + PN_XPLANE, rs, a.sv.dy4m, gtile * 8, tid);
        PN_LDS_BARRIER();
        PN_TR(pn_trace_bwd, 5);
        b_epilogue<MIX>(acc, m3, X, wave, lane);
        PnTileW<MIX, 0, 9> W3;
        W3.prefetch(img, PKH_D3, PKM_D3, PN_NFB * wave, lane);
        PN_LDS_BARRIER();
        PN_TR(pn_trace_bwd, 6);
        pn_acc_zero(acc);
        PN_TR(pn_trace_bwd, 7);
        if (wave < PN_NW) {
            f32x16 acce[1][2];
            pn_acc_zero(acce);
            if constexpr (MIX) pn_gemm_mix<1, 0, 9, 1>(X, img + PKM_D3, 8, lane, acce, wave);
            else pn_gemm_f16x3<4, 9, 1>(X, reinterpret_cast<const uint4 *>(img + PKH_D3), 8, lane, acce, 4 * wave);
#pragma unroll
            for (int rb = 0; rb < 2; ++rb)
                *reinterpret_cast<float4 *>(X + (wave >> 1) * PN_XPLANE + (32 * rb + (lane & 31)) * PN_XRS + 512 + (wave & 1) * 32 + (lane >> 5) * 16) =
                    make_float4(acce[0][rb][0], acce[0][rb][1], acce[0][rb][2], acce[0][rb][3]);
        }
        W3.run(X, lane, acc);
        pn_copy_out_kmajor_hs<PN_H>(X, rs, a.sv.dy3k, gtile * 8, tid);
        if (WG2) pn_copy_out_kmajor_hs<PN_H>(X + PN_XPLANE, rs, a.sv.dy3m, gtile * 8, tid);
        PN_LDS_BARRIER();
        PN_TR(pn_trace_bwd, 8);
        b_epilogue<MIX>(acc, m2, X, wave, lane);
        PN_LDS_BARRIER();
        if (tid < PN_TILE) {
            const int p = prow[tid];
            float4 u = make_float4(0.f, 0.f, 0.f, 0.f), v = u;
#pragma unroll
            for (int w = 0; w < 4; ++w) {
                const float4 a0 = *reinterpret_cast<const float4 *>(X + (w >> 1) * PN_XPLANE + tid * PN_XRS + 512 + (w & 1) * 32);
                const float4 a1 = *reinterpret_cast<const float4 *>(X + (w >> 1) * PN_XPLANE + tid * PN_XRS + 512 + (w & 1) * 32 + 16);
                u.x += a0.x; u.y += a0.y; u.z += a0.z; u.w += a0.w; v.x += a1.x; v.y += a1.y; v.z += a1.z; v.w += a1.w;
            }
            float vx, vy, vz, gx = 0.f, gy = 0.f, gz = 0.f;
            if (p >= 0) {
                rot3(a.cam.rw2c, rdir[tid], rdir[PN_TILE + tid], rdir[2 * PN_TILE + tid], true, vx, vy, vz);
                rot3(a.cam.rw2c, u.w + v.z * vx, v.x + v.z * vy, v.y + v.z * vz, false, gx, gy, gz);
            }
            float *slot = reinterpret_cast<float *>(X + tid * PN_XRS + 512);
            const float ri = rs.inv(tid);
            *reinterpret_cast<float4 *>(slot) = make_float4(u.x * ri, u.y * ri, u.z * ri, gx * ri);
            *reinterpret_cast<float2 *>(slot + 4) = make_float2(gy * ri, gz * ri);
        }
        PN_WAVE_LDS_SYNC();
        if (tid < PN_TILE) {
#pragma unroll
            for (int j = 0; j < 3; ++j) {
                const int e = 64 * j + tid, r = (e * 21846) >> 16, c = e - 3 * r;
                const int p = prow[r];
                if (p >= 0) {
                    const float *slot = reinterpret_cast<const float *>(X + r * PN_XRS + 512);
                    atomicAdd(&a.g_color[3 * p + c], slot[c]);
                    atomicAdd(&a.g_dir[3 * p + c], slot[3 + c]);
                }
            }
        }
        PnTileW<MIX, 0, 8> W2;
        W2.prefetch(img, PKH_D2, PKM_D2, PN_NFB * wave, lane);
        PN_LDS_BARRIER();
        PN_TR(pn_trace_bwd, 9);
        pn_acc_zero(acc);
        PN_TR(pn_trace_bwd, 10);
        W2.run(X, lane, acc);
        pn_copy_out_kmajor_hs<PN_H>(X, rs, a.sv.dy2k, gtile * 8, tid);
        if (WG2) pn_copy_out_kmajor_hs<PN_H>(X + PN_XPLANE, rs, a.sv.dy2m, gtile * 8, tid);
        PN_LDS_BARRIER();
        PN_TR(pn_trace_bwd, 11);
        b_epilogue<MIX>(acc, m1, X, wave, lane);
        PN_LDS_BARRIER();
        PN_TR(pn_trace_bwd, 12);
        pn_acc_zero(acc);
        PN_TR(pn_trace_bwd, 13);
        [[maybe_unused]] f32x16 acx[1][2];
        [[maybe_unused]] f32x16 (&acc1)[1][2] = *reinterpret_cast<f32x16 (*)[1][2]>(&acc[PN_NFB - 1]);
        if constexpr (MIX) {
            if (wave < 3) pn_gemm_mix<PN_MIX_NS, 0, PN_MB_D1, PN_NFB>(X, img + PKM_D1, 2 * wave, lane, acc);
            else {
                pn_gemm_mix<PN_MIX_NS, 0, PN_MB_D1, 1>(X, img + PKM_D1, 6, lane, acc);
                if constexpr (XYZG) {
                    pn_gemm_mix<PN_MIX_NS, 0, 2, 1>(X, img + PKM_D1T, 0, lane, acc1);
                    pn_acc_zero(acx);
                    pn_gemm_mix<PN_MIX_NS, 0, 2, 1>(X, img + PKM_D1T, 1, lane, acx);
                }
            }
        } else {
            if (wave < 3) pn_gemm_f16x3<16, PN_MB_D1, PN_NFB>(X, reinterpret_cast<const uint4 *>(img + PKH_D1), 2 * wave, lane, acc);
            else {
                pn_gemm_f16x3<16, PN_MB_D1, 1>(X, reinterpret_cast<const uint4 *>(img + PKH_D1), 6, lane, acc);
                if constexpr (XYZG) {
                    pn_gemm_f16x3<16, 2, 1>(X, reinterpret_cast<const uint4 *>(img + PKH_D1T), 0, lane, acc1);
                    pn_acc_zero(acx);
                    pn_gemm_f16x3<16, 2, 1>(X, reinterpret_cast<const uint4 *>(img + PKH_D1T), 1, lane, acx);
                }
            }
        }
        pn_copy_out_kmajor_hs<PN_H>(X, rs, a.sv.dy1k, gtile * 8, tid);
        if (WG2) pn_copy_out_kmajor_hs<PN_H>(X + PN_XPLANE, rs, a.sv.dy1m, gtile * 8, tid);
        PN_LDS_BARRIER();
        PN_TR(pn_trace_bwd, 14);
#pragma unroll
        for (int fb = 0; fb < PN_NFB; ++fb)
            if (PN_NFB * wave + fb < PN_MB_D1) {
#pragma unroll
                for (int rb = 0; rb < 2; ++rb)
#pragma unroll
                    for (int g = 0; g < 4; ++g)
                        *reinterpret_cast<float4 *>(dx + (32 * rb + (lane & 31)) * LDX + pn_d_feat(PN_NFB * wave + fb, g, lane)) =
                            make_float4(acc[fb][rb][4 * g], acc[fb][rb][4 * g + 1], acc[fb][rb][4 * g + 2], acc[fb][rb][4 * g + 3]);
            }
        if constexpr (XYZG) {
            if (wave == 3) {
#pragma unroll
                for (int fb = 0; fb < 2; ++fb)
#pragma unroll
                    for (int rb = 0; rb < 2; ++rb)
#pragma unroll
                        for (int g = 0; g < 4; ++g) {
                            const f32x16 &v = fb == 0 ? acc1[0][rb] : acx[0][rb];
                            *reinterpret_cast<float4 *>(dx + (32 * rb + (lane & 31)) * LDX + pn_d_feat(PN_MB_D1 + fb, g, lane)) =
                                make_float4(v[4 * g], v[4 * g + 1], v[4 * g + 2], v[4 * g + 3]);
                        }
            }
        }
        PN_LDS_BARRIER();
        PN_TR(pn_trace_bwd, 15);
        if (rp >= 0) {
            float *dr_ = dx + row * LDX;
            const float e[8] = {e0.x, e0.y, e0.z, e0.w, e1.x, e1.y, e1.z, e1.w};
            float go[PN_EPT];
            const float ri = rs.inv(row);
#pragma unroll
            for (int i = 0; i < PN_EPT; ++i) {
                const int dd = PN_EPT * q + i;
                float s[3], c[3];
                pn_pe_octaves<3>(e[i], s, c);
                float g = dr_[dd], fr = 1.f;
#pragma unroll
                for (int f = 0; f < 3; ++f) {
                    const float2 t = *reinterpret_cast<const float2 *>(dr_ + PN_F + dd * 6 + 2 * f);
                    g += fr * (t.x * c[f] - t.y * s[f]);
                    fr *= 2.f;
                }
                go[i] = g * ri;
            }
#pragma unroll
            for (int i = 0; i < PN_EPT; i += 4) *reinterpret_cast<float4 *>(dr_ + PN_EPT * q + i) = make_float4(go[i], go[i + 1], go[i + 2], go[i + 3]);
        }
        PN_WAVE_LDS_SYNC();
        const int r0w = (row & ~15) + (lane >> 5), col = lane & 31;
#pragma unroll
        for (int j = 0; j < 8; ++j) {
            const int r = r0w + 2 * j, p = prow[r];
            if (p >= 0) atomicAdd(&a.g_emb[(long long)p * PN_F + col], dx[r * LDX + col]);
        }
        if constexpr (XYZG) b_xyz_row(a, dx + row * LDX, gwf, wrow, wnrm, sidx, rp, row, q, K, kinv, rs.inv(row));
        if constexpr (!CLAIM) t_cur += grid;
        PN_TR(pn_trace_bwd, 16); PN_TR_SPAN(pn_span_bwd, a.cls, 1);
    }
    if (tile_first >= tile_last) return;
    {
        const int cg = tid0 & 31, rs = tid0 >> 5;
        float *red = reinterpret_cast<float *>(smem_b);
        PN_LDS_BARRIER();
        if (tid0 < PN_NTHR) {
#pragma unroll
            for (int c = 0; c < 8; ++c) red[rs * PN_H + 8 * cg + c] = gw5[c];
            if (cg == 0) red[8 * PN_H + rs] = gb5t;
        }
        PN_LDS_BARRIER();
        if (tid0 >= PN_H) return;
        float t = 0.f;
#pragma unroll
        for (int r = 0; r < 8; ++r) t += red[r * PN_H + tid0];
        atomicAdd(&a.gparams[PO_W5 + tid0], t * invS);
        if (tid0 == 0) {
            float b = 0.f;
            for (int r = 0; r < 8; ++r) b += red[8 * PN_H + r];
            atomicAdd(&a.gparams[PO_B5], b * invS);
        }
    }
}

#ifdef PN_EMU
#define PN_WAIT_VMCNT(n) ((void)0)
#else
#define PN_WAIT_VMCNT(n) asm volatile("s_waitcnt vmcnt(%0)" ::"n"(n) : "memory")
#endif
#ifndef PN_WG_AUX
#define PN_WG_AUX 2
#endif
#ifndef PN_WX_AUX
#define PN_WX_AUX 2
#endif
#ifndef PN_WG_RS
#define PN_WG_RS 32
#endif
#ifndef PN_WG_NST
#define PN_WG_NST 4
#endif
#ifndef PN_WGC_RS
#define PN_WGC_RS 32
#endif
template <int N> __device__ __forceinline__ void pn_wait_vm_stages(int stages) {
    if (stages >= 3) PN_WAIT_VMCNT(3 * N);
    else if (stages == 2) PN_WAIT_VMCNT(2 * N);
    else if (stages == 1) PN_WAIT_VMCNT(N);
    else PN_WAIT_VMCNT(0);
}
template <int NFB, int MF, int RS, int NST, bool TWO = false>
__global__ __launch_bounds__(512) void k_wgrad_f16(const uint4 *__restrict__ A, const uint4 *__restrict__ B,
                                                   const int *__restrict__ d_tiles, float *__restrict__ partial,
                                                   const uint4 *__restrict__ Am = nullptr, const uint4 *__restrict__ Bm = nullptr) {
    constexpr int RG = RS / 8;
    constexpr int AU = RG * MF, BU = RG * NFB;
    constexpr int HALF = AU + BU;
    constexpr int STAGE = TWO ? 2 * HALF : HALF;
    constexpr int NI = STAGE / 64, NIW = (NI + 7) / 8;
    static_assert((NST - 2) * NIW <= 63 && NST >= 3 && NST <= 5, "vmcnt is a 6-bit count");
    constexpr int MTW = MF / 64, NTW = NFB >= 256 ? 2 : 1;
    constexpr int NMAIN = 4 * NTW * 32;
    constexpr bool TAIL_B = NFB > NMAIN, TAIL_ONES = !TAIL_B && MF == 256;
    static_assert(STAGE % 64 == 0, "a stage is a whole number of 1 KB wave copies");
    extern __shared__ __attribute__((aligned(16))) uint4 smem_w[];
    const int tid = threadIdx.x, lane = tid & 63, wave = __builtin_amdgcn_readfirstlane(tid >> 6);
    const int wm = wave >> 2, wn = wave & 3;
    const long long stages = (long long)(*d_tiles) * (PN_TILE / RS);
    const int nst = stages > (long long)blockIdx.x ? (int)((stages - blockIdx.x + gridDim.x - 1) / gridDim.x) : 0;
    f32x16 acc[MTW][NTW], acct;
#pragma unroll
    for (int r = 0; r < 16; ++r) {
        acct[r] = 0.f;
#pragma unroll
        for (int i = 0; i < MTW; ++i)
#pragma unroll
            for (int j = 0; j < NTW; ++j) acc[i][j][r] = 0.f;
    }
    auto issue = [&](int s, int buf) {
        const long long rg = (long long)RG * ((long long)blockIdx.x + (long long)gridDim.x * s);
#pragma unroll
        for (int i = 0; i < NIW; ++i) {
            const bool pad = wave + 8 * i >= NI;
            const int j = pad ? 0 : wave + 8 * i, u0 = 64 * j;
            const uint4 *dst = smem_w + (pad ? NST * STAGE : buf * STAGE + u0);
            const uint4 *src;
            if (u0 < AU) src = A + rg * MF + u0;
            else if (u0 < HALF) src = B + rg * NFB + (u0 - AU);
            else if (u0 < HALF + AU) src = Am + rg * MF + (u0 - HALF);
            else src = Bm + rg * NFB + (u0 - HALF - AU);
            __builtin_amdgcn_global_load_lds(src + lane, (__attribute__((address_space(3))) void *)dst, 16, 0, PN_WG_AUX);
        }
    };
    pn_h8 ones = {0, 0, 0, 0, 0, 0, 0, 0};
    if ((lane & 31) == 0) ones = pn_h8{1, 1, 1, 1, 1, 1, 1, 1};
    const bool has_tail = (TAIL_B || TAIL_ONES) && (MF == 256 || wn < 2);
    if (nst > 0) {
#pragma unroll
        for (int i = 0; i < NST - 1; ++i) if (nst > i) issue(i, i);
        for (int s = 0; s < nst; ++s) {
            pn_wait_vm_stages<NIW>(nst - 1 - s < NST - 2 ? nst - 1 - s : NST - 2);
            __builtin_amdgcn_s_barrier();
            if (s + NST - 1 < nst) issue(s + NST - 1, (s + NST - 1) % NST);
            const uint4 *st = smem_w + (s % NST) * STAGE;
#pragma unroll
            for (int kk = 0; kk < RS / 16; ++kk) {
                const uint4 *fa = st + (2 * kk + (lane >> 5)) * MF + (lane & 31);
                const uint4 *fb = st + AU + (2 * kk + (lane >> 5)) * NFB + (lane & 31);
                pn_h8 ah[MTW], bh[NTW], am[TWO ? MTW : 1], bm[TWO ? NTW : 1];
#pragma unroll
                for (int i = 0; i < MTW; ++i) ah[i] = __builtin_bit_cast(pn_h8, fa[(MTW * wm + i) * 32]);
#pragma unroll
                for (int i = 0; i < NTW; ++i) bh[i] = __builtin_bit_cast(pn_h8, fb[(NTW * wn + i) * 32]);
                if (TWO) {
#pragma unroll
                    for (int i = 0; i < MTW; ++i) am[i] = __builtin_bit_cast(pn_h8, fa[HALF + (MTW * wm + i) * 32]);
#pragma unroll
                    for (int i = 0; i < NTW; ++i) bm[i] = __builtin_bit_cast(pn_h8, fb[HALF + (NTW * wn + i) * 32]);
                }
#pragma unroll
                for (int i = 0; i < MTW; ++i)
#pragma unroll
                    for (int j = 0; j < NTW; ++j)
                        acc[i][j] = __builtin_amdgcn_mfma_f32_32x32x16_f16(ah[i], bh[j], acc[i][j], 0, 0, 0);
                if (TWO) {
#pragma unroll
                    for (int i = 0; i < MTW; ++i)
#pragma unroll
                        for (int j = 0; j < NTW; ++j)
                            acc[i][j] = __builtin_amdgcn_mfma_f32_32x32x16_f16(ah[i], bm[j], acc[i][j], 0, 0, 0);
#pragma unroll
                    for (int i = 0; i < MTW; ++i)
#pragma unroll
                        for (int j = 0; j < NTW; ++j)
                            acc[i][j] = __builtin_amdgcn_mfma_f32_32x32x16_f16(am[i], bh[j], acc[i][j], 0, 0, 0);
                }
                if (has_tail) {
                    pn_h8 tah, tam = ah[0];
                    if (MF == 256) tah = wn == 0 ? ah[0] : wn == 1 ? ah[1] : wn == 2 ? ah[MTW > 2 ? 2 : 0] : ah[MTW > 3 ? 3 : 0];
                    else tah = wn == 0 ? ah[0] : ah[MTW > 1 ? 1 : 0];
                    if (TWO) {
                        if (MF == 256) tam = wn == 0 ? am[0] : wn == 1 ? am[TWO && MTW > 1 ? 1 : 0] : wn == 2 ? am[TWO && MTW > 2 ? 2 : 0] : am[TWO && MTW > 3 ? 3 : 0];
                        else tam = wn == 0 ? am[0] : am[TWO && MTW > 1 ? 1 : 0];
                    }
                    if (TAIL_B) {
                        acct = __builtin_amdgcn_mfma_f32_32x32x16_f16(tah, __builtin_bit_cast(pn_h8, fb[NMAIN]), acct, 0, 0, 0);
                        if (TWO) {
                            acct = __builtin_amdgcn_mfma_f32_32x32x16_f16(tah, __builtin_bit_cast(pn_h8, fb[HALF + NMAIN]), acct, 0, 0, 0);
                            acct = __builtin_amdgcn_mfma_f32_32x32x16_f16(tam, __builtin_bit_cast(pn_h8, fb[NMAIN]), acct, 0, 0, 0);
                        }
                    } else {
                        acct = __builtin_amdgcn_mfma_f32_32x32x16_f16(tah, ones, acct, 0, 0, 0);
                        if (TWO) acct = __builtin_amdgcn_mfma_f32_32x32x16_f16(tam, ones, acct, 0, 0, 0);
                    }
                }
            }
        }
    }
    float *out = partial + (size_t)blockIdx.x * 256 * 288;
#pragma unroll
    for (int i = 0; i < MTW; ++i)
#pragma unroll
        for (int j = 0; j < NTW; ++j)
#pragma unroll
            for (int r = 0; r < 16; ++r) {
                const int m = (MTW * wm + i) * 32 + (r & 3) + 8 * (r >> 2) + 4 * (lane >> 5);
                out[(size_t)m * 288 + (NTW * wn + j) * 32 + (lane & 31)] = acc[i][j][r];
            }
    if (has_tail) {
#pragma unroll
        for (int r = 0; r < 16; ++r) {
            const int m = (MTW * wm + wn) * 32 + (r & 3) + 8 * (r >> 2) + 4 * (lane >> 5);
            out[(size_t)m * 288 + 256 + (lane & 31)] = acct[r];
        }
    }
}

__global__ __launch_bounds__(256) void k_wgrad_reduce_f16(const float *__restrict__ partial, int chunks, int Mreal, int Nreal, int bias_col, const unsigned *__restrict__ gscale,
                                                          const float *__restrict__ cinv, float *__restrict__ grad, int dst_w, int ldc, int dst_b) {
    __shared__ float part[4][64];
    const int lane = threadIdx.x & 63, w = threadIdx.x >> 6;
    const int e = blockIdx.x * 64 + lane;
    const size_t stride = (size_t)256 * 288;
    float s = 0.f;
    if (e < Mreal * 288) {
#pragma unroll 8
        for (int c = w; c < chunks; c += 4) s += partial[c * stride + e];
    }
    part[w][lane] = s;
    __syncthreads();
    if (w == 0 && e < Mreal * 288) {
        float S, invS;
        pn_scale_from_bits(gscale[0], S, invS);
        const int m = e / 288, n = e - m * 288;
        const float v = ((part[0][lane] + part[1][lane]) + (part[2][lane] + part[3][lane])) * invS * cinv[m];
        if (n < Nreal) grad[dst_w + m * ldc + n] += v;
        else if (n == bias_col) grad[dst_b + m] += v;
    }
}

enum WgShape { WG_288x256, WG_256x256, WG_288x128, WG_128x128 };
struct WgLayer {
    WgShape shape;
    const uint4 *dy, *x, *dym, *xm;
    const int *d_tiles;
    long long rows_max;
    int dst_w, ldc, nreal, bias_col, dst_b;
    const float *cinv;
};
template <int NFB, int MF, int RS, int NST, bool TWO>
int launch_wgrad_f16(const WgLayer &L, float *partial, const unsigned *gscale, float *grad, hipStream_t s) {
    int chunks = WG_CHUNKS;
    const long long most = MF == PN_HC ? L.rows_max / ((long long)RS * NST) : L.rows_max / PN_TILE;
    if (most < chunks) chunks = (int)(most > 0 ? most : 1);
    if ((size_t)chunks * 256 * 288 > PARTIAL_FLOATS) return PNERF_E_WS;
    if (TWO && (!L.dym || !L.xm)) return PNERF_E_INVAL;
    constexpr size_t lds = ((size_t)NST * (TWO ? 2 : 1) * (RS / 8) * (MF + NFB) + 64) * 16;
    static_assert(lds <= 160 * 1024, "wgrad ring");
    if (hipFuncSetAttribute((const void *)k_wgrad_f16<NFB, MF, RS, NST, TWO>, hipFuncAttributeMaxDynamicSharedMemorySize, (int)lds) != hipSuccess) return PNERF_E_LAUNCH;
    { PnProfScope prof(PNK_WGRAD, s);
    hipLaunchKernelGGL((k_wgrad_f16<NFB, MF, RS, NST, TWO>), dim3(chunks), dim3(512), lds, s, L.dy, L.x, L.d_tiles, partial, L.dym, L.xm); }
    PnProfScope prof(PNK_WGRAD_REDUCE, s);
    hipLaunchKernelGGL(k_wgrad_reduce_f16, dim3(pn_cdiv((long long)MF * 288, 64)), dim3(256), 0, s, partial, chunks, MF, L.nreal, L.bias_col, gscale, L.cinv, grad, L.dst_w, L.ldc, L.dst_b);
    PN_CHECK_LAUNCH();
    return 0;
}
template <bool TWO>
int launch_wgrad_layer(const WgLayer &L, float *partial, const unsigned *gscale, float *grad, hipStream_t s) {
    constexpr int RS = TWO ? 16 : PN_WG_RS, NST = TWO ? 4 : PN_WG_NST, RSC = TWO ? 16 : PN_WGC_RS;
    switch (L.shape) {
        case WG_288x256: return launch_wgrad_f16<PN_NF1, PN_H, RS, NST, TWO>(L, partial, gscale, grad, s);
        case WG_256x256: return launch_wgrad_f16<PN_H, PN_H, RS, NST, TWO>(L, partial, gscale, grad, s);
        case WG_288x128: return launch_wgrad_f16<PN_NF1, PN_HC, RSC, 4, TWO>(L, partial, gscale, grad, s);
        default: return launch_wgrad_f16<PN_HC, PN_HC, RSC, 4, TWO>(L, partial, gscale, grad, s);
    }
}


struct WgX0Args {
    const int4 *rmeta;
    const float *emb;
    const uint4 *x0t;
    int n_points;
};
#ifndef PN_WX_RS
#define PN_WX_RS 32
#endif
#ifndef PN_WX_D
#define PN_WX_D (PN_WX_RS == 32 ? 3 : 7)
#endif
constexpr int WX_RS = PN_WX_RS, WX_RG = WX_RS / 8;
constexpr int WX_AU = WX_RG * PN_H;
constexpr int WX_NB = 224;
constexpr int WX_BU = WX_RG * WX_NB;
constexpr int WX_TU = WX_RG * 64;
constexpr int WX_GU = WX_RS * 8;
constexpr int WX_NA = WX_AU / 512;
constexpr int WX_L = WX_NA + 2;
constexpr int WX_D = PN_WX_D;
constexpr int WX_NST = WX_D + 1, WX_RMD = 2 * WX_D + 2, WX_GD = WX_D + 1;
constexpr int WX_RM_SLOTS = WX_D + 2, WX_G_SLOTS = WX_D + 1;
static_assert(WX_L * (WX_D - 1) <= 63 && WX_D >= 2, "vmcnt is a 6-bit count");
static_assert(WX_RS == 16 || WX_RS == 32, "rows per stage");
constexpr int WX_OFF_T = WX_NST * WX_AU, WX_OFF_B = WX_OFF_T + WX_NST * WX_TU, WX_OFF_RM = WX_OFF_B + 2 * WX_BU,
              WX_OFF_G = WX_OFF_RM + WX_RM_SLOTS * WX_RS, WX_OFF_PAD = WX_OFF_G + WX_G_SLOTS * WX_GU, WX_UNITS = WX_OFF_PAD + 64;
static_assert(WX_UNITS * 16 <= 160 * 1024, "k_wgrad_x0 LDS");

__device__ __forceinline__ void wx_store_h16(char *buf, int rg, int f, int rlow, _Float16 v) {
    *reinterpret_cast<_Float16 *>(buf + ((rg * WX_NB + f) * 16) + rlow * 2) = v;
}

__global__ __launch_bounds__(512) void k_wgrad_x0(const uint4 *__restrict__ A, WgX0Args g, const int *__restrict__ d_tiles, float *__restrict__ partial) {
    constexpr int MF = PN_H, MTW = 4;
    extern __shared__ __attribute__((aligned(16))) uint4 smem_x[];
    const int tid = threadIdx.x, lane = tid & 63, wave = __builtin_amdgcn_readfirstlane(tid >> 6);
    const int wm = wave >> 2, wn = wave & 3;
    const long long stages = (long long)(*d_tiles) * (PN_TILE / WX_RS);
    const int nst = stages > (long long)blockIdx.x ? (int)((stages - blockIdx.x + gridDim.x - 1) / gridDim.x) : 0;
    auto stage_rg = [&](int s) { return (long long)WX_RG * ((long long)blockIdx.x + (long long)gridDim.x * s); };
    f32x16 acc[MTW][2], acct;
#pragma unroll
    for (int r = 0; r < 16; ++r) {
        acct[r] = 0.f;
#pragma unroll
        for (int i = 0; i < MTW; ++i) { acc[i][0][r] = 0.f; acc[i][1][r] = 0.f; }
    }
    char *lds = reinterpret_cast<char *>(smem_x);
    int p_gather = 0;
    auto issue_a = [&](int s) {
        const bool ok = s < nst;
#pragma unroll
        for (int i = 0; i < WX_NA; ++i) {
            const int piece = wave + 8 * i;
            const uint4 *src = A + (ok ? stage_rg(s) * MF + 64 * piece : 0) + lane;
            const uint4 *dst = smem_x + (ok ? (s % WX_NST) * WX_AU + 64 * piece : WX_OFF_PAD);
            __builtin_amdgcn_global_load_lds(src, (__attribute__((address_space(3))) void *)dst, 16, 0, PN_WX_AUX);
        }
        const bool okt = ok && wave < WX_RG;
        const uint4 *src = g.x0t + (okt ? (stage_rg(s) + wave) * 64 : 0) + lane;
        const uint4 *dst = smem_x + (okt ? WX_OFF_T + (s % WX_NST) * WX_TU + wave * 64 : WX_OFF_PAD);
        __builtin_amdgcn_global_load_lds(src, (__attribute__((address_space(3))) void *)dst, 16, 0, PN_WX_AUX);
    };
    auto issue_second = [&](int s_rm, int s_g) {
        if (wave == 0) {
            const bool ok = s_rm < nst;
            const int4 *src = g.rmeta + (ok ? stage_rg(s_rm) * 8 : 0) + (lane & (WX_RS - 1));
            const uint4 *dst = smem_x + (ok ? WX_OFF_RM + (s_rm % WX_RM_SLOTS) * WX_RS : WX_OFF_PAD);
            if (lane < WX_RS) __builtin_amdgcn_global_load_lds(src, (__attribute__((address_space(3))) void *)dst, 16, 0, 0);
        } else if (wave <= WX_RG) {
            const bool ok = s_g < nst;
            const int p = ok ? p_gather : 0;
            const float *src = g.emb + (long long)p * PN_F + (lane >> 3) * 4;
            const uint4 *dst = smem_x + (ok ? WX_OFF_G + (s_g % WX_G_SLOTS) * WX_GU + (wave - 1) * 64 : WX_OFF_PAD);
            __builtin_amdgcn_global_load_lds(src, (__attribute__((address_space(3))) void *)dst, 16, 0, 0);
        } else {
            __builtin_amdgcn_global_load_lds(A + lane, (__attribute__((address_space(3))) void *)(smem_x + WX_OFF_PAD), 16, 0, 0);
        }
    };
    auto next_point = [&](int s_g) {
        if (wave >= 1 && wave <= WX_RG && s_g < nst) {
            const int p = reinterpret_cast<const int4 *>(smem_x + WX_OFF_RM + (s_g % WX_RM_SLOTS) * WX_RS)[8 * (wave - 1) + (lane & 7)].y;
            p_gather = p < 0 ? 0 : (p >= g.n_points ? g.n_points - 1 : p);
        }
    };
    auto build_into = [&](char *buf, const char *slot) {
#pragma unroll
        for (int it = 0; it < WX_RS / 16; ++it) {
            const int item = tid + 512 * it, rg = item >> 8, d = (item >> 3) & 31, rlow = item & 7;
            const float e = __builtin_amdgcn_fmed3f(*reinterpret_cast<const float *>(slot + rg * 1024 + ((d >> 2) * 8 + rlow) * 16 + (d & 3) * 4), -65504.f, 65504.f);
            float sn[3], cs[3];
            pn_pe_octaves<3>(e, sn, cs);
            const int f = PN_F + d * 6;
            wx_store_h16(buf, rg, d, rlow, (_Float16)e);
#pragma unroll
            for (int o = 0; o < 3; ++o) { wx_store_h16(buf, rg, f + 2 * o, rlow, (_Float16)sn[o]); wx_store_h16(buf, rg, f + 2 * o + 1, rlow, (_Float16)cs[o]); }
        }
    };
    auto build = [&](int s) {
        build_into(lds + (size_t)(WX_OFF_B + (s & 1) * WX_BU) * 16, lds + (size_t)(WX_OFF_G + (s % WX_G_SLOTS) * WX_GU) * 16);
    };
    if (nst > 0) {
        if (wave == 0)
            for (int s = 0; s < WX_RM_SLOTS; ++s) issue_second(s, 0);
        PN_WAIT_VMCNT(0);
        __syncthreads();
        for (int s = 0; s < WX_D; ++s) issue_a(s);
        if (wave >= 1 && wave <= WX_RG)
            for (int s = 0; s < WX_GD; ++s) { next_point(s); issue_second(0, s); }
        PN_WAIT_VMCNT(0);
        __syncthreads();
        if (wave == 0)
            for (int s = WX_RM_SLOTS; s < WX_RMD; ++s) issue_second(s, 0);
        PN_WAIT_VMCNT(0);
        __syncthreads();
        build(0);
        next_point(WX_GD);
        const long long stride_a = (long long)WX_RG * gridDim.x * MF, stride_t = (long long)WX_RG * gridDim.x * 64, stride_rm = (long long)WX_RG * gridDim.x * 8;
        const uint4 *pa = A + stage_rg(WX_D) * MF + 64 * wave + lane;
        const uint4 *pt = g.x0t + (stage_rg(WX_D) + wave) * 64 + lane;
        const int4 *prm = g.rmeta + stage_rg(WX_RMD) * 8 + (lane & (WX_RS - 1));
        int ia = WX_D % WX_NST, ig = WX_GD % WX_G_SLOTS, irm = WX_RMD % WX_RM_SLOTS;
        int ra = 0, rgs = 1 % WX_G_SLOTS, rrm = (1 + WX_GD) % WX_RM_SLOTS;
        const int n_main = nst - WX_RMD > 0 ? nst - WX_RMD : 0;
        auto bump = [](int &c, int n) { c = c + 1 == n ? 0 : c + 1; };
        for (int s = 0; s < nst; ++s) {
            PN_WAIT_VMCNT(WX_L * (WX_D - 1));
            PN_LDS_BARRIER();
            if (s < n_main) {
#pragma unroll
                for (int i = 0; i < WX_NA; ++i)
                    __builtin_amdgcn_global_load_lds(pa + 512 * i, (__attribute__((address_space(3))) void *)(smem_x + ia * WX_AU + 64 * (wave + 8 * i)), 16, 0, PN_WX_AUX);
                if (wave < WX_RG) __builtin_amdgcn_global_load_lds(pt, (__attribute__((address_space(3))) void *)(smem_x + WX_OFF_T + ia * WX_TU + wave * 64), 16, 0, PN_WX_AUX);
                else __builtin_amdgcn_global_load_lds(A + lane, (__attribute__((address_space(3))) void *)(smem_x + WX_OFF_PAD), 16, 0, 0);
                if (wave == 0) {
                    if (lane < WX_RS) __builtin_amdgcn_global_load_lds(prm, (__attribute__((address_space(3))) void *)(smem_x + WX_OFF_RM + irm * WX_RS), 16, 0, 0);
                } else if (wave <= WX_RG) {
                    __builtin_amdgcn_global_load_lds(g.emb + (long long)p_gather * PN_F + (lane >> 3) * 4,
                                                     (__attribute__((address_space(3))) void *)(smem_x + WX_OFF_G + ig * WX_GU + (wave - 1) * 64), 16, 0, 0);
                } else {
                    __builtin_amdgcn_global_load_lds(A + lane, (__attribute__((address_space(3))) void *)(smem_x + WX_OFF_PAD), 16, 0, 0);
                }
            } else {
                issue_a(s + WX_D);
                issue_second(s + WX_RMD, s + WX_GD);
            }
            pa += stride_a; pt += stride_t; prm += stride_rm;
#pragma unroll
            for (int kk = 0; kk < WX_RS / 16; ++kk) {
                const uint4 *fa = smem_x + ra * WX_AU + (2 * kk + (lane >> 5)) * MF + (lane & 31);
                const uint4 *fb = smem_x + WX_OFF_B + (s & 1) * WX_BU + (2 * kk + (lane >> 5)) * WX_NB + (lane & 31);
                const uint4 *ft = smem_x + WX_OFF_T + ra * WX_TU + (2 * kk + (lane >> 5)) * 64 + (lane & 31);
                pn_h8 ah[MTW], bh[2];
#pragma unroll
                for (int i = 0; i < MTW; ++i) ah[i] = __builtin_bit_cast(pn_h8, fa[(MTW * wm + i) * 32]);
                const pn_h8 tah = __builtin_bit_cast(pn_h8, fa[(MTW * wm + wn) * 32]);
                bh[0] = __builtin_bit_cast(pn_h8, fb[(2 * wn) * 32]);
                bh[1] = __builtin_bit_cast(pn_h8, wn < 3 ? fb[(2 * wn + 1) * 32] : ft[0]);
#pragma unroll
                for (int i = 0; i < MTW; ++i)
#pragma unroll
                    for (int j = 0; j < 2; ++j)
                        acc[i][j] = __builtin_amdgcn_mfma_f32_32x32x16_f16(ah[i], bh[j], acc[i][j], 0, 0, 0);
                acct = __builtin_amdgcn_mfma_f32_32x32x16_f16(tah, __builtin_bit_cast(pn_h8, ft[32]), acct, 0, 0, 0);
            }
            build_into(lds + (size_t)(WX_OFF_B + ((s + 1) & 1) * WX_BU) * 16, lds + (size_t)(WX_OFF_G + rgs * WX_GU) * 16);
            if (wave >= 1 && wave <= WX_RG && s + 1 + WX_GD < nst) {
                const int p = reinterpret_cast<const int4 *>(smem_x + WX_OFF_RM + rrm * WX_RS)[8 * (wave - 1) + (lane & 7)].y;
                p_gather = p < 0 ? 0 : (p >= g.n_points ? g.n_points - 1 : p);
            }
            bump(ia, WX_NST); bump(ig, WX_G_SLOTS); bump(irm, WX_RM_SLOTS); bump(ra, WX_NST); bump(rgs, WX_G_SLOTS); bump(rrm, WX_RM_SLOTS);
        }
    }
    float *out = partial + (size_t)blockIdx.x * 256 * 288;
#pragma unroll
    for (int i = 0; i < MTW; ++i)
#pragma unroll
        for (int j = 0; j < 2; ++j)
#pragma unroll
            for (int r = 0; r < 16; ++r) {
                const int m = (MTW * wm + i) * 32 + (r & 3) + 8 * (r >> 2) + 4 * (lane >> 5);
                out[(size_t)m * 288 + (2 * wn + j) * 32 + (lane & 31)] = acc[i][j][r];
            }
#pragma unroll
    for (int r = 0; r < 16; ++r) {
        const int m = (MTW * wm + wn) * 32 + (r & 3) + 8 * (r >> 2) + 4 * (lane >> 5);
        out[(size_t)m * 288 + 256 + (lane & 31)] = acct[r];
    }
}

int launch_wgrad_x0(const uint4 *A, const WgX0Args &g, const int *d_tiles, long long rows_max, float *partial, const unsigned *gscale, const float *cinv,
                    float *grad, hipStream_t s) {
    int chunks = WG_CHUNKS;
    const long long tiles = rows_max / PN_TILE;
    if (tiles < chunks) chunks = (int)(tiles > 0 ? tiles : 1);
    if ((size_t)chunks * 256 * 288 > PARTIAL_FLOATS) return PNERF_E_WS;
    constexpr size_t lds = (size_t)WX_UNITS * 16;
    if (hipFuncSetAttribute((const void *)k_wgrad_x0, hipFuncAttributeMaxDynamicSharedMemorySize, (int)lds) != hipSuccess) return PNERF_E_LAUNCH;
    { PnProfScope prof(PNK_WGRAD, s);
    hipLaunchKernelGGL(k_wgrad_x0, dim3(chunks), dim3(512), lds, s, A, g, d_tiles, partial); }
    PnProfScope prof(PNK_WGRAD_REDUCE, s);
    hipLaunchKernelGGL(k_wgrad_reduce_f16, dim3(pn_cdiv((long long)PN_H * 288, 64)), dim3(256), 0, s, partial, chunks, PN_H, PN_IN1, PN_ONES1, gscale, cinv, grad, (int)PO_W1, (int)PN_IN1, (int)PO_B1);
    PN_CHECK_LAUNCH();
    return 0;
}
}

size_t pn_wgrad_partials_bytes() { return pn_align(PARTIAL_FLOATS * sizeof(float)); }

namespace {
__global__ void k_zero_one_empty(const float *__restrict__ conf, const int *__restrict__ counters, long long slots_per_ray, const float *__restrict__ gs, float eps,
                                 float *__restrict__ g_conf) {
    const long long n_empty = (long long)counters[1] * slots_per_ray - (long long)counters[3];
    if (n_empty <= 0) return;
    const float g = PnZeroOne(conf[0], eps).grad(gs[0]);
    if (g != 0.f) atomicAdd(&g_conf[0], g * (float)n_empty);
}
}

int pn_agg_backward_launch(const pnerf_camera *cam, const pnerf_points *pts, const pnerf_step &st, const float *d_decoded, const float *d_weight,
                           const float *d_grad_decoded, const PnSaved &sv, float *d_grad_params, const pnerf_point_grads *pg,
                           float *d_partials, bool x0_saved, hipStream_t s) {
    const int K = st.K;
    const long long n_valid = st.n_valid_max;
    const PnArith ar = pn_arith();
    BwdArgs a;
    a.cam = *cam; a.params = st.params; a.packed = (const float4 *)st.packed_mlp; a.raydir = st.raydir;
    a.pidx = st.sample_pidx; a.valid_list = st.valid_list; a.counters = st.counters;
    a.SR = st.SR; a.K = K; a.TS = pn_tile_samples(K); a.cap_samples = n_valid;
    a.decoded = d_decoded; a.weight = d_weight; a.grad_decoded = d_grad_decoded; a.sv = sv;
    a.emb = pts->embedding;
    a.gparams = d_grad_params; a.g_emb = pg->embedding; a.g_conf = pg->conf; a.g_dir = pg->dir; a.g_color = pg->color;
    a.conf = pts->conf; a.zo_gs = x0_saved ? nullptr : pg->zero_one_gscale; a.zo_eps = pg->zero_one_eps;
    if (a.zo_gs && !a.conf) return PNERF_E_INVAL;
    if (!a.g_emb || !a.g_conf || !a.g_dir || !a.g_color) return PNERF_E_INVAL;
    BwdXArgs ax;
    ax.xyz = pts->xyz; ax.sample_loc = st.sample_loc; ax.g_xyz = pg->xyz;
    const bool xg = ax.g_xyz != nullptr;
    if (xg && x0_saved) return PNERF_E_UNSUP;
    if (xg && (!ax.xyz || !ax.sample_loc)) return PNERF_E_INVAL;
    const int ncu = pn_cu_count();
    if (!ncu) return PNERF_E_LAUNCH;
    const int grid_c = pn_tile_grid((n_valid + PN_CTILE - 1) / PN_CTILE, 3LL * ncu);
    const size_t lds_c = CB_BYTES, lds_a = xg ? BL_BYTES_X : BL_BYTES;
    const bool wg2 = sv.wg2 != 0;
    if (wg2) x0_saved = true;
    const bool mix = !wg2 && (ar.mix_mask() & 4);
    void (*const kcb)(BwdArgs) = wg2 ? k_color_backward<true> : k_color_backward<false>;
    void (*const kab)(BwdArgs) = wg2 ? k_agg_backward<true> : mix ? k_agg_backward<false, true> : k_agg_backward<false>;
    void (*const kax)(BwdXArgs) = wg2 ? k_agg_backward<true, false, true> : mix ? k_agg_backward<false, true, true> : k_agg_backward<false, false, true>;
    if (hipFuncSetAttribute(reinterpret_cast<const void *>(kcb), hipFuncAttributeMaxDynamicSharedMemorySize, (int)lds_c) != hipSuccess) return PNERF_E_LAUNCH;
    if (hipFuncSetAttribute(xg ? reinterpret_cast<const void *>(kax) : reinterpret_cast<const void *>(kab), hipFuncAttributeMaxDynamicSharedMemorySize, (int)lds_a) != hipSuccess) return PNERF_E_LAUNCH;
    a.cls_list = sv.cls_list; a.cls_info = sv.cls_info; a.valid_list = sv.cls_list;
    if (hipMemsetAsync(sv.gscale, 0, PN_GS_WORDS * sizeof(unsigned), s) != hipSuccess) return PNERF_E_LAUNCH;
    hipLaunchKernelGGL(k_grad_max, dim3(pn_capped_grid((n_valid + 255) / 256, 1024)), dim3(256), 0, s, sv.cls_list, st.counters, n_valid, d_grad_decoded, sv.gscale);
    if (a.zo_gs) hipLaunchKernelGGL(k_zero_one_empty, dim3(1), dim3(1), 0, s, a.conf, st.counters, (long long)st.SR * K, a.zo_gs, a.zo_eps, a.g_conf);
    { PnProfScope prof(PNK_COLOR_BWD, s);
      hipLaunchKernelGGL(kcb, dim3(grid_c), dim3(256), lds_c, s, a); }
    int kc[PN_NCLS];
    const int ncls = pn_class_slots(K, kc);
    { PnProfScope prof(PNK_AGG_BWD, s);
      for (int j = 0; j < ncls; ++j) {
          a.cls = j; a.K = kc[j]; a.TS = pn_tile_samples(kc[j]);
          const int grid_a = pn_tile_grid((n_valid + a.TS - 1) / a.TS, 2LL * ncu);
          if (xg) { static_cast<BwdArgs &>(ax) = a; hipLaunchKernelGGL(kax, dim3(grid_a), dim3(PN_NTHR), lds_a, s, ax); }
          else hipLaunchKernelGGL(kab, dim3(grid_a), dim3(PN_NTHR), lds_a, s, a);
      } }
    PN_CHECK_LAUNCH();
    if (pg->ready_event && hipEventRecord((hipEvent_t)pg->ready_event, s) != hipSuccess) return PNERF_E_LAUNCH;
    const long long rows = sv.rows, smps = sv.samples;
    const int *dt = sv.cls_info + PN_CI_TILES, *ct = sv.cls_info + PN_CI_CTILES;
    const float *ci = reinterpret_cast<const float *>(reinterpret_cast<const char *>(st.packed_mlp) + PKC_SCALE) + PN_CS_UNITS;
    const WgLayer layers[7] = {
        {WG_288x256, sv.dy1k, sv.x0k, sv.dy1m, sv.x0m, dt, rows, PO_W1, PN_IN1, PN_IN1, PN_ONES1, PO_B1, ci + PN_CS_L1},
        {WG_256x256, sv.dy2k, sv.h1k, sv.dy2m, sv.h1m, dt, rows, PO_W2, PN_H, PN_H, PN_H, PO_B2, ci + PN_CS_L2},
        {WG_288x256, sv.dy3k, sv.h2k, sv.dy3m, sv.h2m, dt, rows, PO_W3, PN_IN3, PN_IN3, PN_ONES3, PO_B3, ci + PN_CS_L3},
        {WG_256x256, sv.dy4k, sv.h3k, sv.dy4m, sv.h3m, dt, rows, PO_W4, PN_H, PN_H, PN_H, PO_B4, ci + PN_CS_L4},
        {WG_288x128, sv.dc1k, sv.xck, sv.dc1m, sv.xcm, ct, smps, PO_WC1, PN_INC, PN_INC, -1, 0, ci + PN_CS_C1},
        {WG_128x128, sv.dc2k, sv.c1k, sv.dc2m, sv.c1m, ct, smps, PO_WC2, PN_HC, PN_HC, -1, 0, ci + PN_CS_C2},
        {WG_128x128, sv.dc3k, sv.c2k, sv.dc3m, sv.c2m, ct, smps, PO_WC3, PN_HC, PN_HC, -1, 0, ci + PN_CS_C3},
    };
    for (const WgLayer &L : layers) {
        int rc;
        if (&L == layers && !x0_saved) {
            WgX0Args wa;
            wa.rmeta = sv.rmeta; wa.emb = pts->embedding; wa.x0t = sv.x0k; wa.n_points = pts->n;
            rc = launch_wgrad_x0(L.dy, wa, dt, rows, d_partials, sv.gscale, L.cinv, d_grad_params, s);
        } else {
            rc = wg2 ? launch_wgrad_layer<true>(L, d_partials, sv.gscale, d_grad_params, s) : launch_wgrad_layer<false>(L, d_partials, sv.gscale, d_grad_params, s);
        }
        if (rc) return rc;
    }
    return 0;
}

#ifdef PN_PHASE_TRACE
extern "C" int pnerf_debug_trace_bwd(void *host, size_t bytes) {
    return hipMemcpyFromSymbol(host, HIP_SYMBOL(pn_trace_bwd), bytes < sizeof(pn_trace_bwd) ? bytes : sizeof(pn_trace_bwd)) == hipSuccess ? 0 : -1;
}
extern "C" int pnerf_debug_span_bwd(void *host, size_t bytes) {
    return hipMemcpyFromSymbol(host, HIP_SYMBOL(pn_span_bwd), bytes < sizeof(pn_span_bwd) ? bytes : sizeof(pn_span_bwd)) == hipSuccess ? 0 : -1;
}
#endif
```

pointnerf_amd/csrc/mlp_common.h:

```cpp
#pragma once
#include "pn_common.h"
#include <type_traits>
#include <utility>

#define PN_F      32
#define PN_IN1    284
#define PN_IN1P   288
#define PN_H      256
#define PN_IN3    263
#define PN_INC    280
#define PN_HC     128
#define PN_TILE   64
#define PN_MT     (PN_TILE / 32)
#define PN_NTHR   256
#define PN_NW     4
#define PN_NFB    2
static_assert(PN_NTHR == 64 * PN_NW && PN_NW == 4 && PN_NW * PN_NFB == 8, "the tile kernels are written for 4 waves x 2 of the 8 feature blocks each");
#define PN_TPR    (PN_NTHR / PN_TILE)
#define PN_EPT    (PN_F / PN_TPR)
#define PN_CTILE  64

enum : int {
    PO_W1 = 0, PO_B1 = PO_W1 + PN_H * PN_IN1, PO_W2 = PO_B1 + PN_H, PO_B2 = PO_W2 + PN_H * PN_H,
    PO_W3 = PO_B2 + PN_H, PO_B3 = PO_W3 + PN_H * PN_IN3, PO_W4 = PO_B3 + PN_H, PO_B4 = PO_W4 + PN_H * PN_H,
    PO_W5 = PO_B4 + PN_H, PO_B5 = PO_W5 + PN_H, PO_WC1 = PO_B5 + 1, PO_BC1 = PO_WC1 + PN_HC * PN_INC,
    PO_WC2 = PO_BC1 + PN_HC, PO_BC2 = PO_WC2 + PN_HC * PN_HC, PO_WC3 = PO_BC2 + PN_HC, PO_BC3 = PO_WC3 + PN_HC * PN_HC,
    PO_WC4 = PO_BC3 + PN_HC, PO_BC4 = PO_WC4 + 3 * PN_HC, PO_TOTAL = PO_BC4 + 3
};
static_assert(PO_TOTAL == 341764, "parameter count of the lego-script aggregator");

typedef float f32x16 __attribute__((ext_vector_type(16)));

typedef float pn_f4 __attribute__((ext_vector_type(4)));
typedef float pn_f2 __attribute__((ext_vector_type(2)));

__device__ __forceinline__ float pn_lrelu_grad(float post) { return post > 0.f ? 1.f : 0.01f; }

template <int... I, class F> __device__ __forceinline__ void pn_static_for_impl(std::integer_sequence<int, I...>, F &&f) { (f(std::integral_constant<int, I>{}), ...); }
template <int N, class F> __device__ __forceinline__ void pn_static_for(F &&f) { pn_static_for_impl(std::make_integer_sequence<int, N>{}, f); }

__device__ __forceinline__ void rot3(const float *M, float x, float y, float z, bool transpose, float &ox, float &oy, float &oz) {
    if (!transpose) { ox = x * M[0] + y * M[3] + z * M[6]; oy = x * M[1] + y * M[4] + z * M[7]; oz = x * M[2] + y * M[5] + z * M[8]; }
    else { ox = x * M[0] + y * M[1] + z * M[2]; oy = x * M[3] + y * M[4] + z * M[5]; oz = x * M[6] + y * M[7] + z * M[8]; }
}
template <int N> __device__ __forceinline__ float group_sum(float v) {
#pragma unroll
    for (int off = 1; off < N; off <<= 1) v += __shfl_xor(v, off, 64);
    return v;
}
template <int AF> __device__ __forceinline__ void pn_acc_zero(f32x16 (&acc)[AF][2]) {
#pragma unroll
    for (int i = 0; i < AF; ++i)
#pragma unroll
        for (int j = 0; j < 2; ++j)
#pragma unroll
            for (int r = 0; r < 16; ++r) acc[i][j][r] = 0.f;
}
__device__ __forceinline__ float pn_softplus(float x) {
#ifdef PN_EMU
    return x > 20.f ? x : log1pf(expf(x));
#else
    return x > 20.f ? x : __logf(1.0f + __expf(x));
#endif
}
__device__ __forceinline__ float pn_sigmoid(float x) {
#ifdef PN_EMU
    return x > 20.f ? 1.f : 1.0f / (1.0f + expf(-x));
#else
    return x > 20.f ? 1.f : __builtin_amdgcn_rcpf(1.0f + __expf(-x));
#endif
}

struct PnSaved {
    uint4 *x0k, *h1k, *h2k, *h3k;
    uint4 *dy1k, *dy2k, *dy3k, *dy4k;
    uint4 *h4r;
    float *arow;
    int4 *rmeta;
    unsigned *lmask;
    unsigned *gscale;
    float *fs, *dfs, *c3;
    uint4 *xck, *c1k, *c2k;
    uint4 *dc1k, *dc2k, *dc3k;
    unsigned *cmask;
    uint4 *x0m, *h1m, *h2m, *h3m, *dy1m, *dy2m, *dy3m, *dy4m;
    uint4 *xcm, *c1m, *c2m, *dc1m, *dc2m, *dc3m;
    int wg2;
    int *cls_list;
    int *cls_info;
    int *cls_tmp;
    long long rows, samples;
};
enum : int { PN_NCLS = 3, PN_CI_COUNT = 0, PN_CI_VBASE = 4, PN_CI_TBASE = 8, PN_CI_TILES = 12, PN_CI_CTILES = 13 ,
              PN_CI_CLAIM = 16 , PN_CI_WORDS = 20 };
#ifndef PN_CLAIM_TILES
#define PN_CLAIM_TILES 1
#endif
enum : int { PN_CLAIM_STATIC_FWD = 4, PN_CLAIM_STATIC_BWD = 2, PN_GS_CLAIM = 4, PN_GS_WORDS = 8 };
__device__ __forceinline__ int pn_claim_tile(int nstatic, int grid, int v, int m) { return nstatic * grid + v * PN_CLAIM_TILES + m % PN_CLAIM_TILES; }
int pn_tile_grid(long long tiles, long long dflt);
int pn_class_slots(int K, int kc[3]);
int pn_classify(const PnSaved &sv, const int32_t *d_valid_list, const int32_t *d_counters, const int32_t *d_pidx, int K, long long n_valid, bool train, bool save_x0, hipStream_t s);
size_t pn_saved_walk(void *base, long long n_valid, int K, PnSaved &s);
void pn_cls_walk(PnCarver &cv, PnSaved &s);
size_t pn_saved_bytes(long long n_valid, int K);
PnSaved pn_saved_carve(void *base, long long n_valid, int K);
int pn_agg_forward_launch(const pnerf_camera *cam, const pnerf_points *pts, const pnerf_step &st, float *d_decoded, float *d_weight,
                          const PnSaved &sv, bool train, bool save_x0, hipStream_t s);
int pn_agg_backward_launch(const pnerf_camera *cam, const pnerf_points *pts, const pnerf_step &st, const float *d_decoded, const float *d_weight,
                           const float *d_grad_decoded, const PnSaved &sv, float *d_grad_params, const pnerf_point_grads *pg,
                           float *d_partials, bool x0_saved, hipStream_t s);
size_t pn_wgrad_partials_bytes();
struct PnArith {
    int products;
    int wgrad_planes;
    int cross_terms;
    int mix_where;
    int mix_mask() const { return cross_terms == 8 ? mix_where : 0; }
};
PnArith pn_arith();

__host__ __device__ inline int pn_tile_samples(int K) { return PN_TILE / K; }
__device__ __forceinline__ unsigned pn_kinv(int K) { return (65536u + (unsigned)K - 1u) / (unsigned)K; }
__device__ __forceinline__ int pn_row_div(int row, unsigned kinv) { return (int)(((unsigned)row * kinv) >> 16); }


#ifdef PN_PHASE_TRACE
#define PN_TR_WGS   512
#define PN_TR_IT0   20
#define PN_TR_ITERS 6
#define PN_TR_SLOTS 24
#define PN_TR_DECL(name) __device__ unsigned long long name[PN_TR_WGS * PN_TR_ITERS * PN_TR_SLOTS]
#define PN_TR(buf, ph)                                                                                              \
    do {                                                                                                            \
        if (tid == 0 && blockIdx.x < PN_TR_WGS && titer >= PN_TR_IT0 && titer < PN_TR_IT0 + PN_TR_ITERS)           \
            buf[((size_t)blockIdx.x * PN_TR_ITERS + (titer - PN_TR_IT0)) * PN_TR_SLOTS + (ph)] = wall_clock64();    \
    } while (0)
#define PN_TR_HWID(buf)                                                                                             \
    do {                                                                                                            \
        if (tid == 0 && blockIdx.x < PN_TR_WGS && titer >= PN_TR_IT0 && titer < PN_TR_IT0 + PN_TR_ITERS)           \
            buf[((size_t)blockIdx.x * PN_TR_ITERS + (titer - PN_TR_IT0)) * PN_TR_SLOTS + PN_TR_SLOTS - 1] =         \
                (unsigned long long)__builtin_amdgcn_s_getreg((31 << 11) | 4) |                                    \
                ((unsigned long long)__builtin_amdgcn_s_getreg((31 << 11) | 20) << 32);                             \
    } while (0)
#define PN_TR_ITER_DECL int titer = -1
#define PN_TR_ITER_NEXT ++titer
#define PN_TR_SPAN_DECL(name) __device__ unsigned long long name[PN_TR_WGS * 4]
#define PN_TR_SPAN(buf, cls, end)                                                                                   \
    do {                                                                                                            \
        if (tid == 0 && (cls) == 0 && blockIdx.x < PN_TR_WGS && ((end) || titer == 0)) {                            \
            buf[(size_t)blockIdx.x * 4 + (end)] = wall_clock64();                                                   \
            if (end) buf[(size_t)blockIdx.x * 4 + 2] = (unsigned long long)(titer + 1);                             \
        }                                                                                                           \
    } while (0)
#else
#define PN_TR(buf, ph)
#define PN_TR_HWID(buf)
#define PN_TR_ITER_DECL
#define PN_TR_ITER_NEXT
#define PN_TR_SPAN(buf, cls, end)
#endif
```

Before: 2.144 million.

## Merge per-K-class aggregation launches into one persistent launch with tile-to-class mapping

Forward and claim-based backward aggregation kernels used to launch once per neighbour-count class. They now launch once, with a flat tile index that each tile maps to its class (K, tile size, base offsets) through a small on-device table. The table is built in reverse class order so the heaviest class is scheduled first. This removes per-class launch overhead and the tail drain between class launches so work from different classes can share CUs, at the cost of a little per-tile selection arithmetic and more kernel arguments. The camera-rotation code is also unified into explicit FMA forms.

```diff
diff --git a/pointnerf_amd/csrc/aggregate.hip b/pointnerf_amd/csrc/aggregate.hip
--- a/pointnerf_amd/csrc/aggregate.hip
+++ b/pointnerf_amd/csrc/aggregate.hip
@@ -362,7 +362,8 @@
     const float *xyz_pers, *loc_pers;
     const int *pidx, *valid_list, *counters;
     const int *cls_list, *cls_info;
-    int cls, Kstride;
+    PnClsRec cr[PN_NCLS];
+    int Kstride;
     int save_x0;
     int R, SR, K, TS;
     long long cap_samples;
@@ -467,11 +468,12 @@
     float fx, fy, fz, gx, gy, gz;
 };
 
-__device__ __forceinline__ int f_sample_of(const FwdArgs &a, long long tile, int row, int Ns, unsigned kinv) {
-    const int ls = pn_row_div(row, kinv);
-    const long long vs = tile * a.TS + ls;
-    return (ls < a.TS && vs < Ns) ? a.valid_list[vs] : -1;
-}
+__device__ __forceinline__ int f_sample_of(const FwdArgs &a, const PnTileCls &c, int row) {
+    const int ls = pn_row_div(row, c.kinv);
+    const long long vs = (long long)c.tile * c.TS + ls;
+    return (ls < c.TS && vs < c.Ns) ? a.cls_list[c.vb + vs] : -1;
+}
+__device__ __forceinline__ int f_slot_of(const PnTileCls &c, int row) { return row - pn_row_div(row, c.kinv) * c.K; }
 
 template <bool PERS, bool FRAMES = false>
 __device__ __forceinline__ void f_gather(const FwdArgs &a, FGather &G, int si_, int p_, int q, const float *frames = nullptr) {
@@ -502,6 +504,11 @@
     }
 }
 
+__device__ __forceinline__ void f_rot3t(const float *M, float x, float y, float z, float &ox, float &oy, float &oz) {
+    ox = __builtin_fmaf(z, M[2], __builtin_fmaf(x, M[0], y * M[1]));
+    oy = __builtin_fmaf(z, M[5], __builtin_fmaf(x, M[3], y * M[4]));
+    oz = __builtin_fmaf(z, M[8], __builtin_fmaf(x, M[6], y * M[7]));
+}
 template <bool PERS, bool MIX = false, bool FRAMES = false>
 __device__ __forceinline__ void f_build(const FwdArgs &a, const FGather &G, char *X, float *exb, float *wraw, int *sidx, int si, int p, int row, int q) {
     const float dwx = G.px - G.lx, dwy = G.py - G.ly, dwz = G.pz - G.lz;
@@ -509,27 +516,21 @@
     if (PERS) {
         ppx = G.ppx; ppy = G.ppy; pcz = G.ppz; spx = G.lpx; spy = G.lpy; scz = G.lpz;
     } else {
-        float pcx, pcy, scx, scy;
-        if (FRAMES) {
-            const float *M = a.cam.camrot;
-            const float x = G.px - a.cam.campos[0], y = G.py - a.cam.campos[1], z = G.pz - a.cam.campos[2];
-            const float u = G.lx - a.cam.campos[0], v = G.ly - a.cam.campos[1], w = G.lz - a.cam.campos[2];
-            pcx = __builtin_fmaf(z, M[6], __builtin_fmaf(y, M[3], x * M[0]));
-            pcy = __builtin_fmaf(z, M[7], __builtin_fmaf(y, M[4], x * M[1]));
-            pcz = __builtin_fmaf(z, M[8], __builtin_fmaf(y, M[5], x * M[2]));
-            scx = __builtin_fmaf(w, M[6], __builtin_fmaf(u, M[0], v * M[3]));
-            scy = __builtin_fmaf(w, M[7], __builtin_fmaf(u, M[1], v * M[4]));
-            scz = __builtin_fmaf(w, M[8], __builtin_fmaf(u, M[2], v * M[5]));
-        } else {
-        rot3(a.cam.camrot, G.px - a.cam.campos[0], G.py - a.cam.campos[1], G.pz - a.cam.campos[2], false, pcx, pcy, pcz);
-        rot3(a.cam.camrot, G.lx - a.cam.campos[0], G.ly - a.cam.campos[1], G.lz - a.cam.campos[2], false, scx, scy, scz);
-        }
+        const float *M = a.cam.camrot;
+        const float x = G.px - a.cam.campos[0], y = G.py - a.cam.campos[1], z = G.pz - a.cam.campos[2];
+        const float u = G.lx - a.cam.campos[0], v = G.ly - a.cam.campos[1], w = G.lz - a.cam.campos[2];
+        const float pcx = __builtin_fmaf(z, M[6], __builtin_fmaf(y, M[3], x * M[0]));
+        const float pcy = __builtin_fmaf(z, M[7], __builtin_fmaf(y, M[4], x * M[1]));
+        pcz = __builtin_fmaf(z, M[8], __builtin_fmaf(y, M[5], x * M[2]));
+        const float scx = __builtin_fmaf(w, M[6], __builtin_fmaf(u, M[0], v * M[3]));
+        const float scy = __builtin_fmaf(w, M[7], __builtin_fmaf(u, M[1], v * M[4]));
+        scz = __builtin_fmaf(w, M[8], __builtin_fmaf(u, M[2], v * M[5]));
         ppx = pcx / pcz; ppy = pcy / pcz; spx = scx / scz; spy = scy / scz;
     }
     float d0, d1, d2;
-    if (FRAMES) d0 = d1 = d2 = dwx * G.fx + dwy * G.fy + dwz * G.fz;
-    else rot3(a.cam.rw2c, dwx, dwy, dwz, true, d0, d1, d2);
-    const float d3 = ppx * pcz - spx * scz, d4 = ppy * pcz - spy * scz, d5 = pcz - scz;
+    if (FRAMES) d0 = d1 = d2 = __builtin_fmaf(dwz, G.fz, __builtin_fmaf(dwx, G.fx, dwy * G.fy));
+    else f_rot3t(a.cam.rw2c, dwx, dwy, dwz, d0, d1, d2);
+    const float d3 = __builtin_fmaf(ppx, pcz, -(spx * scz)), d4 = __builtin_fmaf(ppy, pcz, -(spy * scz)), d5 = pcz - scz;
     const float da = q == 0 ? d0 : q == 1 ? d1 : q == 2 ? d2 : d3;
     const float db = q == 0 ? d4 : d5;
     const float e[8] = {G.e0.x, G.e0.y, G.e0.z, G.e0.w, G.e1.x, G.e1.y, G.e1.z, G.e1.w};
@@ -574,8 +575,8 @@
     if (q == 3) pn_xt_store4(X, row, PN_ONES1, 1.f, 0.f, 0.f, 0.f);
     float fvx = 0.f, fvy = 0.f, fvz = 0.f, fqx = 0.f, fqy = 0.f, fqz = 0.f;
     if (FRAMES) {
-        fvx = G.rx * G.gx + G.ry * G.gy + G.rz * G.gz;
-        fqx = G.dxv * G.fx + G.dyv * G.fy + G.dzv * G.fz;
+        fvx = __builtin_fmaf(G.rz, G.gz, __builtin_fmaf(G.rx, G.gx, G.ry * G.gy));
+        fqx = __builtin_fmaf(G.dzv, G.fz, __builtin_fmaf(G.dxv, G.fx, G.dyv * G.fy));
         fvy = __shfl_down(fvx, 1, 64); fvz = __shfl_down(fvx, 2, 64);
         fqy = __shfl_down(fqx, 1, 64); fqz = __shfl_down(fqx, 2, 64);
     }
@@ -583,18 +584,13 @@
         float vx, vy, vz, qx, qy, qz;
         if (FRAMES) { vx = fvx; vy = fvy; vz = fvz; qx = fqx; qy = fqy; qz = fqz; }
         else {
-        rot3(a.cam.rw2c, G.rx, G.ry, G.rz, true, vx, vy, vz);
-        rot3(a.cam.rw2c, G.dxv, G.dyv, G.dzv, true, qx, qy, qz);
+        f_rot3t(a.cam.rw2c, G.rx, G.ry, G.rz, vx, vy, vz);
+        f_rot3t(a.cam.rw2c, G.dxv, G.dyv, G.dzv, qx, qy, qz);
         }
         float *ex = exb + row * 8;
         *reinterpret_cast<float4 *>(ex) = make_float4(G.cx, G.cy, G.cz, qx - vx);
-        if (FRAMES) {
-            *reinterpret_cast<float4 *>(ex + 4) = make_float4(qy - vy, qz - vz, __builtin_fmaf(qz, vz, __builtin_fmaf(qx, vx, qy * vy)), 1.f);
-            wraw[row] = p >= 0 ? 1.0f / fmaxf(sqrtf(__builtin_fmaf(dwz, dwz, __builtin_fmaf(dwx, dwx, dwy * dwy))), 1e-6f) : 0.f;
-        } else {
-        *reinterpret_cast<float4 *>(ex + 4) = make_float4(qy - vy, qz - vz, qx * vx + qy * vy + qz * vz, 1.f);
-        wraw[row] = p >= 0 ? 1.0f / fmaxf(sqrtf(dwx * dwx + dwy * dwy + dwz * dwz), 1e-6f) : 0.f;
-        }
+        *reinterpret_cast<float4 *>(ex + 4) = make_float4(qy - vy, qz - vz, __builtin_fmaf(qz, vz, __builtin_fmaf(qx, vx, qy * vy)), 1.f);
+        wraw[row] = p >= 0 ? 1.0f / fmaxf(sqrtf(__builtin_fmaf(dwz, dwz, __builtin_fmaf(dwx, dwx, dwy * dwy))), 1e-6f) : 0.f;
         sidx[row] = si;
     }
 }
@@ -638,7 +634,7 @@
 }
 
 template <int KC, bool TRAIN>
-__device__ __forceinline__ void f_tail(const FwdArgs &a, const char *X, const float *w5s, const float *wrow, const int *sidx, float b5,
+__device__ __forceinline__ void f_tail(const FwdArgs &a, float *fs, int Ns, const char *X, const float *w5s, const float *wrow, const int *sidx, float b5,
                                        long long tile, long long gtile, int tid, float *wraw = nullptr) {
     constexpr int NS = KC == 0 ? 1 : 8 / (KC == 0 ? 1 : KC);
     const int lane = tid & 63, cg = tid & 31, r0 = 8 * (tid >> 5);
@@ -672,9 +668,9 @@
 #pragma unroll
     for (int j = 0; j < (KC == 0 ? 0 : NS); ++j) {
         const long long vs = tile * (PN_TILE / (KC == 0 ? 1 : KC)) + (r0 / (KC == 0 ? 1 : KC)) + j;
-        if (vs < a.cap_samples) {
-            *reinterpret_cast<float4 *>(a.sv.fs + vs * PN_H + 8 * cg) = fa[j];
-            *reinterpret_cast<float4 *>(a.sv.fs + vs * PN_H + 8 * cg + 4) = fb[j];
+        if (vs < Ns) {
+            *reinterpret_cast<float4 *>(fs + vs * PN_H + 8 * cg) = fa[j];
+            *reinterpret_cast<float4 *>(fs + vs * PN_H + 8 * cg + 4) = fb[j];
         }
     }
     {
@@ -724,32 +720,26 @@
     const float *frames = nullptr;
     if constexpr (FRAMES) frames = a.frames;
     const int tid0 = threadIdx.x;
-    const int K = a.K, TS = a.TS;
-    const unsigned kinv = pn_kinv(K);
-    const int Ns = a.cls_info[PN_CI_COUNT + a.cls];
-    const long long vb = a.cls_info[PN_CI_VBASE + a.cls], tb = a.cls_info[PN_CI_TBASE + a.cls];
-    a.valid_list = a.cls_list + vb; a.cap_samples = Ns;
-    a.sv.fs += vb * PN_H;
-    const long long ntiles = ((long long)Ns + TS - 1) / TS;
+    const PnClsTab ctab = pn_tile_cls_init(a.cls_info, a.cr);
+    const int tile_last = ctab.total, grid = gridDim.x;
     const float *P = a.params;
     const char *img = reinterpret_cast<const char *>(a.packed);
     if (tid0 < PN_H) w5s[tid0] = P[PO_W5 + tid0];
     const float b5 = P[PO_B5];
-    const int tile_last = (int)ntiles, grid = gridDim.x;
     int t0 = blockIdx.x, t1 = t0 + grid, t2 = t1 + grid;
     if (t0 >= tile_last) return;
-    int *claim_ctr = a.sv.cls_info + PN_CI_CLAIM + a.cls, *claim_w = reinterpret_cast<int *>(smem_f + FL_CLAIM);
+    int *claim_ctr = a.sv.cls_info + PN_CI_CLAIM, *claim_w = reinterpret_cast<int *>(smem_f + FL_CLAIM);
     int nclaim = 0;
 
-    long long tile = t0;
     int si0, si1, si2, p0, p1;
     FGather G;
     {
-        const int row = tid0 / PN_TPR, q = tid0 % PN_TPR, k = row - pn_row_div(row, kinv) * K;
-        si0 = f_sample_of(a, tile, row, Ns, kinv); si1 = t1 < tile_last ? f_sample_of(a, t1, row, Ns, kinv) : -1;
-        si2 = t2 < tile_last ? f_sample_of(a, t2, row, Ns, kinv) : -1;
-        p0 = si0 >= 0 ? a.pidx[(long long)si0 * a.Kstride + k] : -1;
-        p1 = si1 >= 0 ? a.pidx[(long long)si1 * a.Kstride + k] : -1;
+        const int row = tid0 / PN_TPR, q = tid0 % PN_TPR;
+        const PnTileCls c0 = pn_tile_cls(ctab, a.cr, t0), c1 = pn_tile_cls(ctab, a.cr, t1);
+        si0 = f_sample_of(a, c0, row); si1 = t1 < tile_last ? f_sample_of(a, c1, row) : -1;
+        si2 = t2 < tile_last ? f_sample_of(a, pn_tile_cls(ctab, a.cr, t2), row) : -1;
+        p0 = si0 >= 0 ? a.pidx[(long long)si0 * a.Kstride + f_slot_of(c0, row)] : -1;
+        p1 = si1 >= 0 ? a.pidx[(long long)si1 * a.Kstride + f_slot_of(c1, row)] : -1;
         f_gather<PERS, FRAMES>(a, G, si0, p0, q, frames);
     }
 
@@ -757,14 +747,18 @@
     PN_TR_ITER_DECL;
     for (bool first = true; t0 < tile_last; first = false) {
         PN_TR_ITER_NEXT;
-        tile = t0;
+        const PnTileCls c0 = pn_tile_cls(ctab, a.cr, t0);
+        const int K = c0.K, TS = c0.TS, Ns = c0.Ns;
+        const unsigned kinv = c0.kinv;
+        const long long tile = c0.tile;
+        float *fs = a.sv.fs + (long long)c0.vb * PN_H;
         int tid = threadIdx.x;
         asm volatile("" : "+v"(tid));
         const int lane = tid & 63, wave = __builtin_amdgcn_readfirstlane(tid >> 6);
         const int row = tid / PN_TPR, q = tid % PN_TPR, k = row - pn_row_div(row, kinv) * K;
-        const long long gtile = tb + tile;
-        PN_LDS_BARRIER();
-        PN_TR(pn_trace_fwd, 0); PN_TR_HWID(pn_trace_fwd); PN_TR_SPAN(pn_span_fwd, a.cls, 0);
+        const long long gtile = c0.tb + tile;
+        PN_LDS_BARRIER();
+        PN_TR(pn_trace_fwd, 0); PN_TR_HWID(pn_trace_fwd); PN_TR_SPAN(pn_span_fwd, 0, 0);
         f_build<PERS, MIX, FRAMES>(a, G, X, exb, wraw, sidx, si0, p0, row, q);
         f_acc_bias(P + PO_B1, wave, lane, acc);
         PnTileW<MIX, 2, 8, NP> W1;
@@ -854,21 +848,21 @@
         if (tid == 0 && claims) claimed = atomicAdd(claim_ctr, 1);
         const int si_next = si1, p_next = p1;
         if (t1 < tile_last) f_gather<PERS, FRAMES>(a, G, si1, p1, q, frames);
-        const int p2 = si2 >= 0 ? a.pidx[(long long)si2 * a.Kstride + k] : -1;
-        const int si3 = t3 < tile_last ? f_sample_of(a, t3, row, Ns, kinv) : -1;
+        const int p2 = si2 >= 0 ? a.pidx[(long long)si2 * a.Kstride + f_slot_of(pn_tile_cls(ctab, a.cr, t2), row)] : -1;
+        const int si3 = t3 < tile_last ? f_sample_of(a, pn_tile_cls(ctab, a.cr, t3), row) : -1;
         PN_LDS_BARRIER();
         PN_TR(pn_trace_fwd, 13);
         f_epilogue<false>(acc, X, wave, lane, mask);
         PN_LDS_BARRIER();
         PN_TR(pn_trace_fwd, 14);
         if (K == 8 || K == 4 || K == 2 || K == 1) {
-            if (K == 8) f_tail<8, TRAIN>(a, X, w5s, wrow, sidx, b5, tile, gtile, tid);
-            else if (K == 4) f_tail<4, TRAIN>(a, X, w5s, wrow, sidx, b5, tile, gtile, tid);
-            else if (K == 2) f_tail<2, TRAIN>(a, X, w5s, wrow, sidx, b5, tile, gtile, tid);
-            else f_tail<1, TRAIN>(a, X, w5s, wrow, sidx, b5, tile, gtile, tid);
+            if (K == 8) f_tail<8, TRAIN>(a, fs, Ns, X, w5s, wrow, sidx, b5, tile, gtile, tid);
+            else if (K == 4) f_tail<4, TRAIN>(a, fs, Ns, X, w5s, wrow, sidx, b5, tile, gtile, tid);
+            else if (K == 2) f_tail<2, TRAIN>(a, fs, Ns, X, w5s, wrow, sidx, b5, tile, gtile, tid);
+            else f_tail<1, TRAIN>(a, fs, Ns, X, w5s, wrow, sidx, b5, tile, gtile, tid);
             PN_TR(pn_trace_fwd, 15);
         } else {
-        f_tail<0, TRAIN>(a, X, w5s, wrow, sidx, b5, tile, gtile, tid, wraw);
+        f_tail<0, TRAIN>(a, fs, Ns, X, w5s, wrow, sidx, b5, tile, gtile, tid, wraw);
         PN_LDS_BARRIER();
         PN_TR(pn_trace_fwd, 15);
         for (int e = tid; e < TS * 32; e += PN_NTHR) {
@@ -883,9 +877,9 @@
                 f1.x = pn_fma2_lo(h.z, m.z, w, f1.x); f1.y = pn_fma2_hi(h.z, m.z, w, f1.y); f1.z = pn_fma2_lo(h.w, m.w, w, f1.z); f1.w = pn_fma2_hi(h.w, m.w, w, f1.w);
             }
             const long long vs = tile * TS + ls;
-            if (vs < a.cap_samples) {
-                *reinterpret_cast<float4 *>(a.sv.fs + vs * PN_H + 8 * cg) = f0;
-                *reinterpret_cast<float4 *>(a.sv.fs + vs * PN_H + 8 * cg + 4) = f1;
+            if (vs < Ns) {
+                *reinterpret_cast<float4 *>(fs + vs * PN_H + 8 * cg) = f0;
+                *reinterpret_cast<float4 *>(fs + vs * PN_H + 8 * cg + 4) = f1;
             }
         }
         if (tid < TS) {
@@ -900,7 +894,7 @@
         si0 = si_next; p0 = p_next; si1 = si2; p1 = p2; si2 = si3;
         if (tid == 0 && claims) *claim_w = claimed;
         t0 = t1; t1 = t2; t2 = t3; ++nclaim;
-        PN_TR(pn_trace_fwd, 16); PN_TR_SPAN(pn_span_fwd, a.cls, 1);
+        PN_TR(pn_trace_fwd, 16); PN_TR_SPAN(pn_span_fwd, 0, 1);
     }
 }
 
@@ -1121,16 +1115,14 @@
     a.cls_list = sv.cls_list; a.cls_info = sv.cls_info; a.Kstride = K;
     int kc[PN_NCLS];
     const int ncls = pn_class_slots(K, kc);
+    pn_class_records(kc, a.cr);
     {
         PnProfScope prof(PNK_AGG_FWD, s);
-        for (int j = 0; j < ncls; ++j) {
-            a.cls = j; a.K = kc[j]; a.TS = pn_tile_samples(kc[j]);
-            const int grid_a = pn_tile_grid((cap_samples + a.TS - 1) / a.TS, 2LL * ncu);
-            if (frames) { FwdArgsF af; static_cast<FwdArgs &>(af) = a; af.frames = pts->frames; hipLaunchKernelGGL(kfnf, dim3(grid_a), dim3(PN_NTHR), lds_a, s, af); }
-            else hipLaunchKernelGGL(kfn, dim3(grid_a), dim3(PN_NTHR), lds_a, s, a);
-        }
-    }
-    a.K = K; a.TS = pn_tile_samples(K); a.valid_list = sv.cls_list;
+        const int grid_a = pn_tile_grid(cap_samples / a.TS + ncls, 2LL * ncu);
+        if (frames) { FwdArgsF af; static_cast<FwdArgs &>(af) = a; af.frames = pts->frames; hipLaunchKernelGGL(kfnf, dim3(grid_a), dim3(PN_NTHR), lds_a, s, af); }
+        else hipLaunchKernelGGL(kfn, dim3(grid_a), dim3(PN_NTHR), lds_a, s, a);
+    }
+    a.valid_list = sv.cls_list;
     {
         PnProfScope prof(PNK_COLOR_FWD, s);
         if (frames) { FwdArgsF af; static_cast<FwdArgs &>(af) = a; af.frames = pts->frames; hipLaunchKernelGGL(cfnf, dim3(grid_c), dim3(256), lds_c, s, af); }
diff --git a/pointnerf_amd/csrc/backward.hip b/pointnerf_amd/csrc/backward.hip
--- a/pointnerf_amd/csrc/backward.hip
+++ b/pointnerf_amd/csrc/backward.hip
@@ -11,6 +11,7 @@
     const float *raydir;
     const int *pidx, *valid_list, *counters;
     const int *cls_list, *cls_info;
+    PnClsRec cr[PN_NCLS];
     int cls;
     int SR, K, TS;
     long long cap_samples;
@@ -486,12 +487,21 @@
     float *dx = reinterpret_cast<float *>(smem_b);
     float *gwf = XYZG ? reinterpret_cast<float *>(smem_b + BL_GW) : nullptr;
     const int tid0 = threadIdx.x;
-    const int K = a.K, TS = a.TS;
-    const unsigned kinv = pn_kinv(K);
-    const int Ns = a.cls_info[PN_CI_COUNT + a.cls];
-    const long long vb = a.cls_info[PN_CI_VBASE + a.cls], tb = a.cls_info[PN_CI_TBASE + a.cls];
-    a.sv.dfs += vb * PN_H;
-    const long long ntiles = ((long long)Ns + TS - 1) / TS;
+    constexpr bool CLAIM = !(XYZG && !MIX);
+    int K = a.K, TS = a.TS;
+    unsigned kinv = pn_kinv(K);
+    long long tb = 0;
+    const float *dfs = a.sv.dfs;
+    long long ntiles;
+    [[maybe_unused]] PnClsTab ctab;
+    if constexpr (CLAIM) { ctab = pn_tile_cls_init(a.cls_info, a.cr); ntiles = ctab.total; }
+    else {
+        const int Ns = a.cls_info[PN_CI_COUNT + a.cls];
+        const long long vb = a.cls_info[PN_CI_VBASE + a.cls];
+        tb = a.cls_info[PN_CI_TBASE + a.cls];
+        dfs += vb * PN_H;
+        ntiles = ((long long)Ns + TS - 1) / TS;
+    }
     const float *P = a.params;
     const char *img = reinterpret_cast<const char *>(a.packed);
     float S, invS;
@@ -500,30 +510,43 @@
     float gw5[8] = {0.f, 0.f, 0.f, 0.f, 0.f, 0.f, 0.f, 0.f};
     float gb5t = 0.f;
     f32x16 acc[PN_NFB][2];
-    constexpr bool CLAIM = !(XYZG && !MIX);
     using tile_t = std::conditional_t<CLAIM, int, long long>;
     const tile_t tile_first = blockIdx.x, tile_last = (tile_t)ntiles, grid = gridDim.x;
     tile_t t_cur = tile_first;
     [[maybe_unused]] tile_t t_nxt = t_cur + grid;
     int nclaim = 0;
-    int *claim_ctr = reinterpret_cast<int *>(a.sv.gscale) + PN_GS_CLAIM + a.cls, *claim_w = reinterpret_cast<int *>(smem_b + BL_CLAIM);
+    int *claim_ctr = reinterpret_cast<int *>(a.sv.gscale) + PN_GS_CLAIM + (CLAIM ? 0 : a.cls), *claim_w = reinterpret_cast<int *>(smem_b + BL_CLAIM);
     int4 rm_cur = make_int4(-1, -1, 0, 0);
     float ar_cur = 0.f;
+    if constexpr (CLAIM) {
+        if (tile_first >= tile_last) return;
+        if (tid0 < PN_TILE) {
+            const PnTileCls c = pn_tile_cls(ctab, a.cr, tile_first);
+            rm_cur = a.sv.rmeta[((long long)c.tb + c.tile) * PN_TILE + tid0];
+            ar_cur = a.sv.arow[((long long)c.tb + c.tile) * PN_TILE + tid0];
+        }
+    } else {
     if (tid0 < PN_TILE && tile_first < tile_last) {
         rm_cur = a.sv.rmeta[(tb + tile_first) * PN_TILE + tid0];
         ar_cur = a.sv.arow[(tb + tile_first) * PN_TILE + tid0];
     }
+    }
     PN_TR_ITER_DECL;
     for (; t_cur < tile_last; ++nclaim) {
         PN_TR_ITER_NEXT;
-        const long long tile = t_cur;
+        long long tile = t_cur;
+        if constexpr (CLAIM) {
+            const PnTileCls c = pn_tile_cls(ctab, a.cr, t_cur);
+            K = c.K; TS = c.TS; kinv = c.kinv; tb = c.tb; tile = c.tile;
+            dfs = a.sv.dfs + (long long)c.vb * PN_H;
+        }
         int tid = threadIdx.x;
         asm volatile("" : "+v"(tid));
         const int lane = tid & 63, wave = __builtin_amdgcn_readfirstlane(tid >> 6);
         const int row = tid / PN_TPR, q = tid % PN_TPR;
         const long long gtile = tb + tile;
         PN_LDS_BARRIER();
-        PN_TR(pn_trace_bwd, 0); PN_TR_HWID(pn_trace_bwd); PN_TR_SPAN(pn_span_bwd, a.cls, 0);
+        PN_TR(pn_trace_bwd, 0); PN_TR_HWID(pn_trace_bwd); PN_TR_SPAN(pn_span_bwd, CLAIM ? 0 : a.cls, 0);
         unsigned m1[PN_NFB], m2[PN_NFB], m3[PN_NFB];
 #pragma unroll
         for (int fb = 0; fb < PN_NFB; ++fb) {
@@ -547,8 +570,9 @@
         float ar_nxt = 0.f;
         if constexpr (CLAIM) {
             if (tid < PN_TILE && t_nxt < tile_last) {
-                rm_nxt = a.sv.rmeta[(tb + t_nxt) * PN_TILE + tid];
-                ar_nxt = a.sv.arow[(tb + t_nxt) * PN_TILE + tid];
+                const PnTileCls cn = pn_tile_cls(ctab, a.cr, t_nxt);
+                rm_nxt = a.sv.rmeta[((long long)cn.tb + cn.tile) * PN_TILE + tid];
+                ar_nxt = a.sv.arow[((long long)cn.tb + cn.tile) * PN_TILE + tid];
             }
         } else {
             if (tid < PN_TILE && tile + grid < tile_last) {
@@ -574,7 +598,7 @@
         }
         __builtin_amdgcn_sched_barrier(0);
         float4 dfr[4];
-        const float *dfb0 = a.sv.dfs + (tile * TS + pn_row_div(8 * ((tid >> 5) & 7), kinv)) * PN_H + 8 * (tid & 31);
+        const float *dfb0 = dfs + (tile * TS + pn_row_div(8 * ((tid >> 5) & 7), kinv)) * PN_H + 8 * (tid & 31);
         if (K == 8 || K == 4) {
             dfr[0] = *reinterpret_cast<const float4 *>(dfb0); dfr[1] = *reinterpret_cast<const float4 *>(dfb0 + 4);
             if (K == 4) { dfr[2] = *reinterpret_cast<const float4 *>(dfb0 + PN_H); dfr[3] = *reinterpret_cast<const float4 *>(dfb0 + PN_H + 4); }
@@ -772,7 +796,7 @@
         }
         if constexpr (XYZG) b_xyz_row(a, dx + row * LDX, gwf, wrow, wnrm, sidx, rp, row, q, K, kinv, rs.inv(row));
         if constexpr (!CLAIM) t_cur += grid;
-        PN_TR(pn_trace_bwd, 16); PN_TR_SPAN(pn_span_bwd, a.cls, 1);
+        PN_TR(pn_trace_bwd, 16); PN_TR_SPAN(pn_span_bwd, CLAIM ? 0 : a.cls, 1);
     }
     if (tile_first >= tile_last) return;
     {
@@ -1274,11 +1298,16 @@
     int kc[PN_NCLS];
     const int ncls = pn_class_slots(K, kc);
     { PnProfScope prof(PNK_AGG_BWD, s);
-      for (int j = 0; j < ncls; ++j) {
+      pn_class_records(kc, a.cr);
+      if (!xg || mix) {
+          a.cls = 0;
+          const int grid_a = pn_tile_grid(n_valid / a.TS + ncls, 2LL * ncu);
+          if (xg) { static_cast<BwdArgs &>(ax) = a; hipLaunchKernelGGL(kax, dim3(grid_a), dim3(PN_NTHR), lds_a, s, ax); }
+          else hipLaunchKernelGGL(kab, dim3(grid_a), dim3(PN_NTHR), lds_a, s, a);
+      } else for (int j = 0; j < ncls; ++j) {
           a.cls = j; a.K = kc[j]; a.TS = pn_tile_samples(kc[j]);
           const int grid_a = pn_tile_grid((n_valid + a.TS - 1) / a.TS, 2LL * ncu);
-          if (xg) { static_cast<BwdArgs &>(ax) = a; hipLaunchKernelGGL(kax, dim3(grid_a), dim3(PN_NTHR), lds_a, s, ax); }
-          else hipLaunchKernelGGL(kab, dim3(grid_a), dim3(PN_NTHR), lds_a, s, a);
+          static_cast<BwdArgs &>(ax) = a; hipLaunchKernelGGL(kax, dim3(grid_a), dim3(PN_NTHR), lds_a, s, ax);
       } }
     PN_CHECK_LAUNCH();
     if (pg->ready_event && hipEventRecord((hipEvent_t)pg->ready_event, s) != hipSuccess) return PNERF_E_LAUNCH;
diff --git a/pointnerf_amd/csrc/mlp_common.h b/pointnerf_amd/csrc/mlp_common.h
--- a/pointnerf_amd/csrc/mlp_common.h
+++ b/pointnerf_amd/csrc/mlp_common.h
@@ -120,10 +120,44 @@
 };
 PnArith pn_arith();
 
-__host__ __device__ inline int pn_tile_samples(int K) { return PN_TILE / K; }
-__device__ __forceinline__ unsigned pn_kinv(int K) { return (65536u + (unsigned)K - 1u) / (unsigned)K; }
+__host__ __device__ inline int pn_tile_samples(int K) { return K > 0 ? PN_TILE / K : 1; }
+__host__ __device__ __forceinline__ unsigned pn_kinv(int K) { return K > 0 ? (65536u + (unsigned)K - 1u) / (unsigned)K : 0u; }
 __device__ __forceinline__ int pn_row_div(int row, unsigned kinv) { return (int)(((unsigned)row * kinv) >> 16); }
 
+struct PnClsRec { int K, TS; unsigned kinv; };
+static inline void pn_class_records(const int kc[3], PnClsRec (&cr)[3]) {
+    for (int c = 0; c < 3; ++c) { cr[c].K = kc[c]; cr[c].TS = pn_tile_samples(kc[c]); cr[c].kinv = pn_kinv(kc[c]); }
+}
+struct PnClsTab { int first[PN_NCLS], Ns[PN_NCLS], vb[PN_NCLS], tb[PN_NCLS]; int total; };
+struct PnTileCls {
+    int tile;
+    int K, TS;
+    unsigned kinv;
+    int Ns, vb, tb;
+};
+__device__ __forceinline__ PnClsTab pn_tile_cls_init(const int *__restrict__ cls_info, const PnClsRec (&cr)[PN_NCLS]) {
+    PnClsTab t;
+    int first = 0;
+#pragma unroll
+    for (int j = 0; j < PN_NCLS; ++j) {
+        const int c = PN_NCLS - 1 - j;
+        t.first[j] = first;
+        t.Ns[j] = __builtin_amdgcn_readfirstlane(cls_info[PN_CI_COUNT + c]); t.vb[j] = __builtin_amdgcn_readfirstlane(cls_info[PN_CI_VBASE + c]);
+        t.tb[j] = __builtin_amdgcn_readfirstlane(cls_info[PN_CI_TBASE + c]);
+        first += cr[c].K > 0 ? (t.Ns[j] + cr[c].TS - 1) / cr[c].TS : 0;
+    }
+    t.total = first;
+    return t;
+}
+__device__ __forceinline__ PnTileCls pn_tile_cls(const PnClsTab &tab, const PnClsRec (&cr)[PN_NCLS], int t) {
+    const bool b1 = t >= tab.first[1], b2 = t >= tab.first[2];
+    auto sel = [&](int v0, int v1, int v2) { return b2 ? v2 : (b1 ? v1 : v0); };
+    PnTileCls c;
+    c.tile = t - sel(tab.first[0], tab.first[1], tab.first[2]);
+    c.K = sel(cr[2].K, cr[1].K, cr[0].K); c.TS = sel(cr[2].TS, cr[1].TS, cr[0].TS); c.kinv = (unsigned)sel((int)cr[2].kinv, (int)cr[1].kinv, (int)cr[0].kinv);
+    c.Ns = sel(tab.Ns[0], tab.Ns[1], tab.Ns[2]); c.vb = sel(tab.vb[0], tab.vb[1], tab.vb[2]); c.tb = sel(tab.tb[0], tab.tb[1], tab.tb[2]);
+    return c;
+}
 
 #ifdef PN_PHASE_TRACE
 #define PN_TR_WGS   512
```

New measurement: 2.152 million, median of 6. Within noise of the previous version (+0.3%).
